# CVPR23/Depth-guided-Texture-Diffusion-for-Image-Semantic-Segmentation

Hardware: NVIDIA B200
Metric: rgbd_images_per_sec_384 (higher is better)
Workload: dtype bf16

## Files before the change

depth-guided-texture-diffusion-for-image-semantic-segmentation_b200/csrc/common.cuh:

```cuda
#pragma once
#include <cuda_bf16.h>
#include <cuda_runtime.h>
#include <stdint.h>
#include <stdio.h>

#include "../../include/dgtd_ops.h"

#if defined(__CUDA_ARCH__) && (__CUDA_ARCH__ < 1000)
#error "libdgtd_ops targets sm_100a only"
#endif

namespace dgtd {

void set_error(const char* fmt, ...);
void count_launch(int n = 1);

#define DGTD_CHECK_ARG(cond, ...)        \
  do {                                   \
    if (!(cond)) {                       \
      ::dgtd::set_error(__VA_ARGS__);    \
      return -1;                         \
    }                                    \
  } while (0)

#define DGTD_LAUNCH_CHECK(name)                                                  \
  do {                                                                           \
    cudaError_t e__ = cudaGetLastError();                                        \
    if (e__ != cudaSuccess) {                                                    \
      ::dgtd::set_error("%s: launch failed: %s", name, cudaGetErrorString(e__)); \
      return -2;                                                                 \
    }                                                                            \
    ::dgtd::count_launch();                                                      \
  } while (0)

static inline int cdiv(int64_t a, int64_t b) { return (int)((a + b - 1) / b); }

__device__ __forceinline__ float warp_sum(float v) {
#pragma unroll
  for (int o = 16; o > 0; o >>= 1) v += __shfl_xor_sync(0xffffffffu, v, o);
  return v;
}

__device__ __forceinline__ float gelu_erf(float x) {
  return 0.5f * x * (1.0f + erff(x * 0.70710678118654752440f));
}

__device__ __forceinline__ float sigmoidf_acc(float x) { return 1.0f / (1.0f + expf(-x)); }

template <int ACT>
__device__ __forceinline__ float apply_act(float x) {
  if (ACT == DGTD_ACT_GELU) return gelu_erf(x);
  if (ACT == DGTD_ACT_RELU) return fmaxf(x, 0.0f);
  return x;
}

__device__ __forceinline__ float to_float(float v) { return v; }
__device__ __forceinline__ float to_float(__nv_bfloat16 v) { return __bfloat162float(v); }

template <typename T>
__device__ __forceinline__ T from_float(float v);
template <>
__device__ __forceinline__ float from_float<float>(float v) { return v; }
template <>
__device__ __forceinline__ __nv_bfloat16 from_float<__nv_bfloat16>(float v) {
  return __float2bfloat16_rn(v);
}

__device__ __forceinline__ void store1(float* p, float v) { *p = v; }
__device__ __forceinline__ void store1(__nv_bfloat16* p, float v) { *p = __float2bfloat16_rn(v); }
__device__ __forceinline__ void store4(float* p, float a, float b, float c, float d) {
  *reinterpret_cast<float4*>(p) = make_float4(a, b, c, d);
}
__device__ __forceinline__ void store4(__nv_bfloat16* p, float a, float b, float c, float d) {
  __nv_bfloat162 lo = __floats2bfloat162_rn(a, b), hi = __floats2bfloat162_rn(c, d);
  uint2 u;
  u.x = *reinterpret_cast<uint32_t*>(&lo);
  u.y = *reinterpret_cast<uint32_t*>(&hi);
  *reinterpret_cast<uint2*>(p) = u;
}
__device__ __forceinline__ float4 load4(const float* p) {
  return *reinterpret_cast<const float4*>(p);
}
__device__ __forceinline__ float4 load4(const __nv_bfloat16* p) {
  uint2 u = *reinterpret_cast<const uint2*>(p);
  __nv_bfloat162 lo = *reinterpret_cast<__nv_bfloat162*>(&u.x);
  __nv_bfloat162 hi = *reinterpret_cast<__nv_bfloat162*>(&u.y);
  float2 a = __bfloat1622float2(lo), b = __bfloat1622float2(hi);
  return make_float4(a.x, a.y, b.x, b.y);
}

__device__ __forceinline__ uint64_t pk2(float a, float b) {
  uint64_t r;
  asm("mov.b64 %0, {%1, %2};" : "=l"(r) : "f"(a), "f"(b));
  return r;
}
__device__ __forceinline__ void up2(uint64_t r, float& a, float& b) {
  asm("mov.b64 {%0, %1}, %2;" : "=f"(a), "=f"(b) : "l"(r));
}
__device__ __forceinline__ uint64_t fma2(uint64_t a, uint64_t b, uint64_t c) {
  uint64_t d;
  asm("fma.rn.f32x2 %0, %1, %2, %3;" : "=l"(d) : "l"(a), "l"(b), "l"(c));
  return d;
}
__device__ __forceinline__ uint64_t mul2(uint64_t a, uint64_t b) {
  uint64_t d;
  asm("mul.rn.f32x2 %0, %1, %2;" : "=l"(d) : "l"(a), "l"(b));
  return d;
}
__device__ __forceinline__ uint64_t add2(uint64_t a, uint64_t b) {
  uint64_t d;
  asm("add.rn.f32x2 %0, %1, %2;" : "=l"(d) : "l"(a), "l"(b));
  return d;
}
__device__ __forceinline__ void bilinear_src(int dst, float scale, int in_size, int& i0, int& i1,
                                             float& l1) {
  float s = (dst + 0.5f) * scale - 0.5f;
  s = s < 0.f ? 0.f : s;
  i0 = (int)s;
  if (i0 > in_size - 1) i0 = in_size - 1;
  i1 = i0 + (i0 < in_size - 1 ? 1 : 0);
  l1 = s - (float)i0;
}

}
```

depth-guided-texture-diffusion-for-image-semantic-segmentation_b200/csrc/convnext_ops.cu:

```cuda
#include "common.cuh"

namespace dgtd {

constexpr int STEM_PX = 16;

constexpr int STEM_TILES_PER_CTA = 12;

__global__ void __launch_bounds__(256)
stem_kernel(const float* __restrict__ image, const float* __restrict__ grid, int G,
            const float* __restrict__ w, const float* __restrict__ bias,
            const float* __restrict__ ln_w, const float* __restrict__ ln_b, float* __restrict__ out,
            int H, int W, int oh, int ow, int Cout, float eps, int total_tiles) {
  extern __shared__ float sm[];
  float* in = sm;
  float* ys = sm + STEM_PX * 48;
  const int tiles_x = (ow + STEM_PX - 1) / STEM_PX;
  const int c = threadIdx.x;
  float wr[48];
#pragma unroll
  for (int k = 0; k < 48; ++k) wr[k] = w[(int64_t)c * 48 + k];
  const float bc = bias[c];
  const int lane = threadIdx.x & 31, wid = threadIdx.x >> 5, nw = blockDim.x >> 5;

  for (int it = 0; it < STEM_TILES_PER_CTA; ++it) {
    int tile = blockIdx.x * STEM_TILES_PER_CTA + it;
    if (tile >= total_tiles) break;
    const int tx = tile % tiles_x;
    tile /= tiles_x;
    const int oy = tile % oh, b = tile / oh;
    const int ox0 = tx * STEM_PX;
    for (int e = threadIdx.x; e < 3 * 4 * 4 * STEM_PX; e += blockDim.x) {
      int ci = e / (16 * STEM_PX), r = e - ci * 16 * STEM_PX;
      int ky = r / (4 * STEM_PX), j = r - ky * 4 * STEM_PX;
      int px = j >> 2, kx = j & 3;
      int iy = oy * 4 + ky, ix = ox0 * 4 + j;
      float v = 0.f;
      if (ox0 + px < ow) {
        v = image[(((int64_t)b * 3 + ci) * H + iy) * W + ix];
        if (grid) {
          int y0, y1, x0, x1;
          float ly, lx;
          bilinear_src(iy, (float)G / H, G, y0, y1, ly);
          bilinear_src(ix, (float)G / W, G, x0, x1, lx);
          const float* g = grid + ((int64_t)b * 3 + ci) * G * G;
          v += (1.f - ly) * ((1.f - lx) * g[y0 * G + x0] + lx * g[y0 * G + x1]) +
               ly * ((1.f - lx) * g[y1 * G + x0] + lx * g[y1 * G + x1]);
        }
      }
      in[px * 48 + ci * 16 + ky * 4 + kx] = v;
    }
    __syncthreads();
#pragma unroll 4
    for (int px = 0; px < STEM_PX; ++px) {
      float acc = bc;
#pragma unroll
      for (int k4 = 0; k4 < 12; ++k4) {
        float4 v = *reinterpret_cast<const float4*>(&in[px * 48 + k4 * 4]);
        acc = fmaf(wr[k4 * 4 + 0], v.x, acc);
        acc = fmaf(wr[k4 * 4 + 1], v.y, acc);
        acc = fmaf(wr[k4 * 4 + 2], v.z, acc);
        acc = fmaf(wr[k4 * 4 + 3], v.w, acc);
      }
      ys[px * Cout + c] = acc;
    }
    __syncthreads();
    for (int px = wid; px < STEM_PX; px += nw) {
      if (ox0 + px >= ow) continue;
      float s = 0.f;
      for (int cc = lane; cc < Cout; cc += 32) s += ys[px * Cout + cc];
      float mean = warp_sum(s) / Cout;
      float q = 0.f;
      for (int cc = lane; cc < Cout; cc += 32) {
        float d = ys[px * Cout + cc] - mean;
        q = fmaf(d, d, q);
      }
      float rstd = 1.0f / sqrtf(warp_sum(q) / Cout + eps);
      float* o = out + (((int64_t)b * oh + oy) * ow + ox0 + px) * Cout;
      for (int cc = lane; cc < Cout; cc += 32)
        o[cc] = (ys[px * Cout + cc] - mean) * rstd * ln_w[cc] + ln_b[cc];
    }
    __syncthreads();
  }
}

template <typename OT, int VPL>
__global__ void __launch_bounds__(256)
ln_patchify_kernel(const float* __restrict__ x, const float* __restrict__ ln_w,
                   const float* __restrict__ ln_b, OT* __restrict__ out, int B, int h, int w, int C,
                   float eps) {
  const int h2 = h >> 1, w2 = w >> 1;
  int64_t pix = (int64_t)blockIdx.x * 8 + (threadIdx.x >> 5);
  int64_t total = (int64_t)B * h2 * 2 * w2 * 2;
  if (pix >= total) return;
  const int lane = threadIdx.x & 31;
  int xx = (int)(pix % (w2 * 2));
  int64_t t = pix / (w2 * 2);
  int yy = (int)(t % (h2 * 2));
  int b = (int)(t / (h2 * 2));
  const float* p = x + (((int64_t)b * h + yy) * w + xx) * C;
  float v[VPL];
  float s = 0.f;
#pragma unroll
  for (int j = 0; j < VPL; ++j) {
    v[j] = p[lane + 32 * j];
    s += v[j];
  }
  float mean = warp_sum(s) / C;
  float q = 0.f;
#pragma unroll
  for (int j = 0; j < VPL; ++j) {
    float d = v[j] - mean;
    q = fmaf(d, d, q);
  }
  float rstd = 1.0f / sqrtf(warp_sum(q) / C + eps);
  OT* o = out + (((int64_t)b * h2 + (yy >> 1)) * w2 + (xx >> 1)) * (4 * (int64_t)C) +
          (int64_t)((yy & 1) * 2 + (xx & 1)) * C;
#pragma unroll
  for (int j = 0; j < VPL; ++j) {
    int cc = lane + 32 * j;
    o[cc] = from_float<OT>((v[j] - mean) * rstd * ln_w[cc] + ln_b[cc]);
  }
}

template <typename OT, int V4, int R>
__global__ void __launch_bounds__(256)
ln_patchify_v4_kernel(const float* __restrict__ x, const float* __restrict__ ln_w, const float* __restrict__ ln_b,
                      OT* __restrict__ out, int B, int h, int w, int C, float eps) {
  const int h2 = h >> 1, w2 = w >> 1;
  const int64_t total = (int64_t)B * h2 * w2 * 4;
  const int64_t pix0 = ((int64_t)blockIdx.x * 8 + (threadIdx.x >> 5)) * R;
  if (pix0 >= total) return;
  const int lane = threadIdx.x & 31;
  float4 v[R][V4];
#pragma unroll
  for (int r = 0; r < R; ++r) {
    const int64_t pix = pix0 + r;
    const int r4 = (int)(pix & 3);
    int64_t t = pix >> 2;
    const int x2 = (int)(t % w2);
    t /= w2;
    const int y2 = (int)(t % h2), b = (int)(t / h2);
    const float* p = x + (((int64_t)b * h + 2 * y2 + (r4 >> 1)) * w + 2 * x2 + (r4 & 1)) * C;
#pragma unroll
    for (int j = 0; j < V4; ++j)
      v[r][j] = pix < total ? __ldg(reinterpret_cast<const float4*>(p + (j * 32 + lane) * 4)) : make_float4(0.f, 0.f, 0.f, 0.f);
  }
  float4 g[V4], be[V4];
#pragma unroll
  for (int j = 0; j < V4; ++j) {
    g[j] = __ldg(reinterpret_cast<const float4*>(ln_w + (j * 32 + lane) * 4));
    be[j] = __ldg(reinterpret_cast<const float4*>(ln_b + (j * 32 + lane) * 4));
  }
  const float inv_c = 1.0f / C;
#pragma unroll
  for (int r = 0; r < R; ++r) {
    float s = 0.f;
#pragma unroll
    for (int j = 0; j < V4; ++j) s += (v[r][j].x + v[r][j].y) + (v[r][j].z + v[r][j].w);
    const float mean = warp_sum(s) * inv_c;
    float q = 0.f;
#pragma unroll
    for (int j = 0; j < V4; ++j) {
      const float a = v[r][j].x - mean, bb = v[r][j].y - mean, c = v[r][j].z - mean, d = v[r][j].w - mean;
      q += (a * a + bb * bb) + (c * c + d * d);
    }
    const float rstd = 1.0f / sqrtf(warp_sum(q) * inv_c + eps);
    if (pix0 + r < total) {
      OT* o = out + (pix0 + r) * C;
#pragma unroll
      for (int j = 0; j < V4; ++j)
        store4(o + (j * 32 + lane) * 4, (v[r][j].x - mean) * rstd * g[j].x + be[j].x, (v[r][j].y - mean) * rstd * g[j].y + be[j].y,
               (v[r][j].z - mean) * rstd * g[j].z + be[j].z, (v[r][j].w - mean) * rstd * g[j].w + be[j].w);
    }
  }
}

template <typename OT, int TH>
__global__ void __launch_bounds__(256, 2)
dwconv7_ln_kernel(const float* __restrict__ x, const float* __restrict__ dw_w,
                  const float* __restrict__ dw_b, const float* __restrict__ ln_w,
                  const float* __restrict__ ln_b, OT* __restrict__ out, int h, int w, int C,
                  float eps) {
  constexpr int TW = 8, NPX = TH * TW;
  extern __shared__ float ys[];
  const int tiles_x = (w + TW - 1) / TW, tiles_y = (h + TH - 1) / TH;
  int bid = blockIdx.x;
  const int tx = bid % tiles_x;
  bid /= tiles_x;
  const int ty = bid % tiles_y, b = bid / tiles_y;
  const int x0 = tx * TW, y0 = ty * TH;
  const float* xb = x + (int64_t)b * h * w * C;

  for (int c = threadIdx.x; c < C; c += blockDim.x) {
    float wr[49];
#pragma unroll
    for (int k = 0; k < 49; ++k) wr[k] = dw_w[(int64_t)c * 49 + k];
    float acc[TH][TW];
    const float bc = dw_b[c];
#pragma unroll
    for (int i = 0; i < TH; ++i)
#pragma unroll
      for (int j = 0; j < TW; ++j) acc[i][j] = bc;
#pragma unroll
    for (int iy = 0; iy < TH + 6; ++iy) {
      const int gy = y0 + iy - 3;
      if (gy < 0 || gy >= h) continue;
      float in[TW + 6];
      const float* row = xb + (int64_t)gy * w * C + c;
#pragma unroll
      for (int j = 0; j < TW + 6; ++j) {
        int gx = x0 + j - 3;
        in[j] = (gx >= 0 && gx < w) ? row[(int64_t)gx * C] : 0.f;
      }
#pragma unroll
      for (int oy = 0; oy < TH; ++oy) {
        const int ky = iy - oy;
        if (ky < 0 || ky >= 7) continue;
#pragma unroll
        for (int ox = 0; ox < TW; ++ox)
#pragma unroll
          for (int kx = 0; kx < 7; ++kx) acc[oy][ox] = fmaf(wr[ky * 7 + kx], in[ox + kx], acc[oy][ox]);
      }
      asm volatile("" ::: "memory");
    }
#pragma unroll
    for (int i = 0; i < TH; ++i)
#pragma unroll
      for (int j = 0; j < TW; ++j) ys[(i * TW + j) * C + c] = acc[i][j];
  }
  __syncthreads();
  const int lane = threadIdx.x & 31, wid = threadIdx.x >> 5, nw = blockDim.x >> 5;
  for (int px = wid; px < NPX; px += nw) {
    const int oy = y0 + px / TW, ox = x0 + px % TW;
    if (oy >= h || ox >= w) continue;
    const float* yp = ys + px * C;
    float s = 0.f;
    for (int c = lane; c < C; c += 32) s += yp[c];
    const float mean = warp_sum(s) / C;
    float q = 0.f;
    for (int c = lane; c < C; c += 32) {
      float d = yp[c] - mean;
      q = fmaf(d, d, q);
    }
    const float rstd = 1.0f / sqrtf(warp_sum(q) / C + eps);
    OT* o = out + (((int64_t)b * h + oy) * w + ox) * C;
    for (int c = lane; c < C; c += 32)
      o[c] = from_float<OT>((yp[c] - mean) * rstd * ln_w[c] + ln_b[c]);
  }
}

__global__ void __launch_bounds__(256)
fusion_sum_kernel(const float* __restrict__ z0, const float* __restrict__ z1, const float* __restrict__ z2,
                  const float* __restrict__ z3, int h0, int w0, int h1, int w1, int h2, int w2, int h3, int w3,
                  const float* __restrict__ bias, float* __restrict__ out_nhwc, float* __restrict__ out_nchw,
                  __nv_bfloat16* __restrict__ out_pad, int C, int Cpad, int quads, int64_t total) {
  const int64_t i = (int64_t)blockIdx.x * blockDim.x + threadIdx.x;
  if (i >= total) return;
  const int cq = (int)(i % quads);
  const int64_t p = i / quads;
  const int c = cq * 4;
  if (c >= C) {
    if (out_pad && c < Cpad) store4(out_pad + p * Cpad + c, 0.f, 0.f, 0.f, 0.f);
    return;
  }
  const int ox = (int)(p % w0);
  const int64_t t = p / w0;
  const int oy = (int)(t % h0), b = (int)(t / h0);
  float4 acc = load4(bias + c);
  {
    const float4 v = load4(z0 + p * C + c);
    acc.x += v.x; acc.y += v.y; acc.z += v.z; acc.w += v.w;
  }
#pragma unroll
  for (int lv = 1; lv < 4; ++lv) {
    const float* src = lv == 1 ? z1 : lv == 2 ? z2 : z3;
    const int hh = lv == 1 ? h1 : lv == 2 ? h2 : h3;
    const int ww = lv == 1 ? w1 : lv == 2 ? w2 : w3;
    int y0, y1, x0, x1;
    float ly, lx;
    bilinear_src(oy, (float)hh / h0, hh, y0, y1, ly);
    bilinear_src(ox, (float)ww / w0, ww, x0, x1, lx);
    const float* sb = src + (int64_t)b * hh * ww * C + c;
    const float4 a = load4(sb + ((int64_t)y0 * ww + x0) * C), bq = load4(sb + ((int64_t)y0 * ww + x1) * C);
    const float4 cc = load4(sb + ((int64_t)y1 * ww + x0) * C), d = load4(sb + ((int64_t)y1 * ww + x1) * C);
    const float w00 = (1.f - ly) * (1.f - lx), w01 = (1.f - ly) * lx, w10 = ly * (1.f - lx), w11 = ly * lx;
    acc.x += w00 * a.x + w01 * bq.x + w10 * cc.x + w11 * d.x;
    acc.y += w00 * a.y + w01 * bq.y + w10 * cc.y + w11 * d.y;
    acc.z += w00 * a.z + w01 * bq.z + w10 * cc.z + w11 * d.z;
    acc.w += w00 * a.w + w01 * bq.w + w10 * cc.w + w11 * d.w;
  }
  if (out_nhwc) store4(out_nhwc + p * C + c, acc.x, acc.y, acc.z, acc.w);
  if (out_pad) store4(out_pad + p * Cpad + c, acc.x, acc.y, acc.z, acc.w);
  if (out_nchw) {
    const int64_t hw = (int64_t)h0 * w0, r = p - (int64_t)b * hw;
    float* o = out_nchw + ((int64_t)b * C + c) * hw + r;
    o[0] = acc.x; o[hw] = acc.y; o[2 * hw] = acc.z; o[3 * hw] = acc.w;
  }
}

template <typename IT, typename OT>
__global__ void resize_nhwc_kernel(const IT* __restrict__ x, OT* __restrict__ out, int h, int w, int C,
                                   int oh, int ow, int64_t total) {
  int64_t i = (int64_t)blockIdx.x * blockDim.x + threadIdx.x;
  if (i >= total) return;
  const int c4 = C >> 2;
  int cq = (int)(i % c4);
  int64_t t = i / c4;
  int ox = (int)(t % ow);
  t /= ow;
  int oy = (int)(t % oh), b = (int)(t / oh);
  int y0, y1, x0, x1;
  float ly, lx;
  bilinear_src(oy, (float)h / oh, h, y0, y1, ly);
  bilinear_src(ox, (float)w / ow, w, x0, x1, lx);
  const IT* xb = x + (int64_t)b * h * w * C + cq * 4;
  float4 a = load4(xb + ((int64_t)y0 * w + x0) * C), bq = load4(xb + ((int64_t)y0 * w + x1) * C);
  float4 cc = load4(xb + ((int64_t)y1 * w + x0) * C), d = load4(xb + ((int64_t)y1 * w + x1) * C);
  float w00 = (1.f - ly) * (1.f - lx), w01 = (1.f - ly) * lx, w10 = ly * (1.f - lx), w11 = ly * lx;
  store4(out + (((int64_t)b * oh + oy) * ow + ox) * C + cq * 4,
         w00 * a.x + w01 * bq.x + w10 * cc.x + w11 * d.x, w00 * a.y + w01 * bq.y + w10 * cc.y + w11 * d.y,
         w00 * a.z + w01 * bq.z + w10 * cc.z + w11 * d.z, w00 * a.w + w01 * bq.w + w10 * cc.w + w11 * d.w);
}

}

namespace dgtd {
int ln_rows_any(const float* y, const float* ln_w, const float* ln_b, void* out, int out_dtype, int64_t rows, int C,
                float eps, cudaStream_t s);
int dwconv7_ln_tma(const float* x, const float* wT, const float* dw_b, const float* ln_w, const float* ln_b,
                   float* ws, void* out, int out_dtype, int B, int h, int w, int C, float eps, cudaStream_t s);
int dwconv7_stats_tma(const float* x, const float* wT, const float* dw_b, __nv_bfloat16* y, float2* stats, int B, int h,
                      int w, int C, float eps, cudaStream_t s);
}
using namespace dgtd;

extern "C" {

int dgtd_stem_fwd(const float* image, const float* grid, int G, const float* w, const float* b,
                  const float* ln_w, const float* ln_b, float* out, int B, int H, int W, int Cout,
                  float eps, dgtd_stream_t stream) {
  DGTD_CHECK_ARG(image && w && b && ln_w && ln_b && out, "stem: null pointer");
  DGTD_CHECK_ARG(B > 0 && H >= 4 && W >= 4 && Cout >= 32 && Cout <= 256 && Cout % 32 == 0,
                 "stem: bad shape B=%d H=%d W=%d Cout=%d", B, H, W, Cout);
  DGTD_CHECK_ARG(!grid || G > 0, "stem: bad grid size");
  const int oh = H / 4, ow = W / 4;
  size_t smem = (size_t)(STEM_PX * 48 + STEM_PX * Cout) * sizeof(float);
  const int total_tiles = cdiv(ow, STEM_PX) * oh * B;
  stem_kernel<<<cdiv(total_tiles, STEM_TILES_PER_CTA), Cout, smem, (cudaStream_t)stream>>>(
      image, grid, G, w, b, ln_w, ln_b, out, H, W, oh, ow, Cout, eps, total_tiles);
  DGTD_LAUNCH_CHECK("stem");
  return 0;
}

}

template <typename OT>
static int ln_patchify_dispatch(const float* x, const float* ln_w, const float* ln_b, OT* out, int B,
                                int h, int w, int C, float eps, cudaStream_t s) {
  int64_t pix = (int64_t)B * (h / 2) * 2 * (w / 2) * 2;
  if (C % 128 == 0 && (reinterpret_cast<uintptr_t>(x) & 15) == 0 && (reinterpret_cast<uintptr_t>(out) & 15) == 0 &&
      (reinterpret_cast<uintptr_t>(ln_w) & 15) == 0 && (reinterpret_cast<uintptr_t>(ln_b) & 15) == 0) {
    switch (C / 128) {
      case 1: ln_patchify_v4_kernel<OT, 1, 4><<<cdiv(pix, 32), 256, 0, s>>>(x, ln_w, ln_b, out, B, h, w, C, eps); return 0;
      case 2: ln_patchify_v4_kernel<OT, 2, 2><<<cdiv(pix, 16), 256, 0, s>>>(x, ln_w, ln_b, out, B, h, w, C, eps); return 0;
      case 4: ln_patchify_v4_kernel<OT, 4, 1><<<cdiv(pix, 8), 256, 0, s>>>(x, ln_w, ln_b, out, B, h, w, C, eps); return 0;
      case 8: ln_patchify_v4_kernel<OT, 8, 1><<<cdiv(pix, 8), 256, 0, s>>>(x, ln_w, ln_b, out, B, h, w, C, eps); return 0;
      default: break;
    }
  }
  int blocks = cdiv(pix, 8);
  switch (C / 32) {
    case 1: ln_patchify_kernel<OT, 1><<<blocks, 256, 0, s>>>(x, ln_w, ln_b, out, B, h, w, C, eps); break;
    case 2: ln_patchify_kernel<OT, 2><<<blocks, 256, 0, s>>>(x, ln_w, ln_b, out, B, h, w, C, eps); break;
    case 4: ln_patchify_kernel<OT, 4><<<blocks, 256, 0, s>>>(x, ln_w, ln_b, out, B, h, w, C, eps); break;
    case 8: ln_patchify_kernel<OT, 8><<<blocks, 256, 0, s>>>(x, ln_w, ln_b, out, B, h, w, C, eps); break;
    case 16: ln_patchify_kernel<OT, 16><<<blocks, 256, 0, s>>>(x, ln_w, ln_b, out, B, h, w, C, eps); break;
    case 32: ln_patchify_kernel<OT, 32><<<blocks, 256, 0, s>>>(x, ln_w, ln_b, out, B, h, w, C, eps); break;
    default:
      set_error("ln_patchify: C=%d must be 32*{1,2,4,8,16,32}", C);
      return -1;
  }
  return 0;
}

extern "C" int dgtd_ln_patchify_fwd(const float* x, const float* ln_w, const float* ln_b, void* out,
                         int out_dtype, int B, int h, int w, int C, float eps,
                         dgtd_stream_t stream) {
  DGTD_CHECK_ARG(x && ln_w && ln_b && out && B > 0 && h >= 2 && w >= 2 && C % 32 == 0,
                 "ln_patchify: bad args");
  int rc = out_dtype == DGTD_BF16
               ? ln_patchify_dispatch(x, ln_w, ln_b, (__nv_bfloat16*)out, B, h, w, C, eps, (cudaStream_t)stream)
               : ln_patchify_dispatch(x, ln_w, ln_b, (float*)out, B, h, w, C, eps, (cudaStream_t)stream);
  if (rc) return rc;
  DGTD_LAUNCH_CHECK("ln_patchify");
  return 0;
}

template <typename OT>
static int dwconv_launch(const float* x, const float* dw_w, const float* dw_b, const float* ln_w,
                         const float* ln_b, OT* out, int B, int h, int w, int C, float eps,
                         cudaStream_t s) {
  constexpr int TH = 4;
  size_t smem = (size_t)TH * 8 * C * sizeof(float);
  if (smem > 48 * 1024) {
    cudaError_t e = cudaFuncSetAttribute(dwconv7_ln_kernel<OT, TH>,
                                         cudaFuncAttributeMaxDynamicSharedMemorySize, (int)smem);
    if (e != cudaSuccess) {
      set_error("dwconv7_ln: cannot opt in to %zu B smem: %s", smem, cudaGetErrorString(e));
      return -2;
    }
  }
  int threads = C < 256 ? C : 256;
  int64_t blocks = (int64_t)B * cdiv(h, TH) * cdiv(w, 8);
  dwconv7_ln_kernel<OT, TH><<<(unsigned)blocks, threads, smem, s>>>(x, dw_w, dw_b, ln_w, ln_b, out, h,
                                                                    w, C, eps);
  return 0;
}

extern "C" {

int dgtd_dwconv7_ln_fwd(const float* x, const float* dw_w, const float* dw_b, const float* ln_w,
                        const float* ln_b, void* out, int out_dtype, int B, int h, int w, int C,
                        float eps, dgtd_stream_t stream) {
  DGTD_CHECK_ARG(x && dw_w && dw_b && ln_w && ln_b && out, "dwconv7_ln: null pointer");
  DGTD_CHECK_ARG(B > 0 && h > 0 && w > 0 && C >= 32 && C % 32 == 0 && C <= 1024,
                 "dwconv7_ln: bad shape B=%d h=%d w=%d C=%d", B, h, w, C);
  int rc = out_dtype == DGTD_BF16
               ? dwconv_launch(x, dw_w, dw_b, ln_w, ln_b, (__nv_bfloat16*)out, B, h, w, C, eps, (cudaStream_t)stream)
               : dwconv_launch(x, dw_w, dw_b, ln_w, ln_b, (float*)out, B, h, w, C, eps, (cudaStream_t)stream);
  if (rc) return rc;
  DGTD_LAUNCH_CHECK("dwconv7_ln");
  return 0;
}

int dgtd_dwconv7_ln_tma_fwd(const float* x, const float* dw_wT, const float* dw_b, const float* ln_w,
                            const float* ln_b, float* ws, void* out, int out_dtype, int B, int h, int w,
                            int C, float eps, dgtd_stream_t stream) {
  DGTD_CHECK_ARG(x && dw_wT && dw_b && ln_w && ln_b && ws && out, "dwconv7_ln_tma: null pointer");
  DGTD_CHECK_ARG(B > 0 && h > 0 && w > 0 && C >= 128 && C % 128 == 0 && C <= 1024,
                 "dwconv7_ln_tma: bad shape B=%d h=%d w=%d C=%d (C must be a multiple of 128)", B, h, w, C);
  int rc = dwconv7_ln_tma(x, dw_wT, dw_b, ln_w, ln_b, ws, out, out_dtype, B, h, w, C, eps, (cudaStream_t)stream);
  if (rc > 0) {
    set_error("dwconv7_ln_tma: shape not supported by the TMA variant");
    return -1;
  }
  if (rc) return rc;
  DGTD_LAUNCH_CHECK("dwconv7_ln_tma.ln");
  return 0;
}

int dgtd_dwconv7_stats_tma_fwd(const float* x, const float* dw_wT, const float* dw_b, void* y, float* stats, int B, int h,
                               int w, int C, float eps, dgtd_stream_t stream) {
  DGTD_CHECK_ARG(x && dw_wT && dw_b && y && stats, "dwconv7_stats_tma: null pointer");
  DGTD_CHECK_ARG(B > 0 && h > 0 && w > 0 && C >= 128 && C % 128 == 0 && C <= 1024,
                 "dwconv7_stats_tma: bad shape B=%d h=%d w=%d C=%d (C must be a multiple of 128)", B, h, w, C);
  DGTD_CHECK_ARG((reinterpret_cast<uintptr_t>(stats) & 7) == 0 && (reinterpret_cast<uintptr_t>(y) & 15) == 0,
                 "dwconv7_stats_tma: y must be 16-byte, stats 8-byte aligned");
  int rc = dwconv7_stats_tma(x, dw_wT, dw_b, (__nv_bfloat16*)y, (float2*)stats, B, h, w, C, eps, (cudaStream_t)stream);
  if (rc > 0) {
    set_error("dwconv7_stats_tma: shape not supported by the TMA variant");
    return -1;
  }
  return rc;
}

int dgtd_ln_rows_fwd(const float* y, const float* ln_w, const float* ln_b, void* out, int out_dtype, int64_t rows,
                     int C, float eps, dgtd_stream_t stream) {
  DGTD_CHECK_ARG(y && ln_w && ln_b && out && rows > 0 && C % 128 == 0 && C <= 1024, "ln_rows: bad args");
  int rc = ln_rows_any(y, ln_w, ln_b, out, out_dtype, rows, C, eps, (cudaStream_t)stream);
  if (rc) return rc;
  DGTD_LAUNCH_CHECK("ln_rows");
  return 0;
}

int dgtd_fusion_sum_fwd(const float* z0, const float* z1, const float* z2, const float* z3, const int* hw,
                        const float* bias, float* out_nhwc, float* out_nchw, void* out_pad, int Cpad, int B, int C,
                        dgtd_stream_t stream) {
  DGTD_CHECK_ARG(z0 && z1 && z2 && z3 && hw && bias, "fusion_sum: null pointer");
  DGTD_CHECK_ARG(C > 0 && C % 4 == 0, "fusion_sum: C must be a multiple of 4");
  DGTD_CHECK_ARG(out_nhwc || out_nchw || out_pad, "fusion_sum: no output requested");
  DGTD_CHECK_ARG(!out_pad || (Cpad >= C && Cpad % 4 == 0), "fusion_sum: Cpad must be a multiple of 4 and >= C");
  const int quads = (out_pad && Cpad > C ? Cpad : C) / 4;
  const int64_t total = (int64_t)B * hw[0] * hw[1] * quads;
  fusion_sum_kernel<<<(unsigned)cdiv(total, (int64_t)256), 256, 0, (cudaStream_t)stream>>>(
      z0, z1, z2, z3, hw[0], hw[1], hw[2], hw[3], hw[4], hw[5], hw[6], hw[7], bias, out_nhwc, out_nchw,
      (__nv_bfloat16*)out_pad, C, Cpad, quads, total);
  DGTD_LAUNCH_CHECK("fusion_sum");
  return 0;
}

int dgtd_resize_nhwc_fwd(const void* x, void* out, int B, int h, int w, int C, int oh, int ow,
                         int dtype_in, int dtype_out, dgtd_stream_t stream) {
  DGTD_CHECK_ARG(x && out && B > 0 && h > 0 && w > 0 && oh > 0 && ow > 0 && C % 4 == 0,
                 "resize_nhwc: bad args (C must be a multiple of 4)");
  int64_t total = (int64_t)B * oh * ow * (C / 4);
  cudaStream_t s = (cudaStream_t)stream;
  int blocks = cdiv(total, 256);
  if (dtype_in == DGTD_F32 && dtype_out == DGTD_F32)
    resize_nhwc_kernel<<<blocks, 256, 0, s>>>((const float*)x, (float*)out, h, w, C, oh, ow, total);
  else if (dtype_in == DGTD_BF16 && dtype_out == DGTD_BF16)
    resize_nhwc_kernel<<<blocks, 256, 0, s>>>((const __nv_bfloat16*)x, (__nv_bfloat16*)out, h, w, C, oh, ow, total);
  else if (dtype_in == DGTD_BF16 && dtype_out == DGTD_F32)
    resize_nhwc_kernel<<<blocks, 256, 0, s>>>((const __nv_bfloat16*)x, (float*)out, h, w, C, oh, ow, total);
  else
    resize_nhwc_kernel<<<blocks, 256, 0, s>>>((const float*)x, (__nv_bfloat16*)out, h, w, C, oh, ow, total);
  DGTD_LAUNCH_CHECK("resize_nhwc");
  return 0;
}

}
```

depth-guided-texture-diffusion-for-image-semantic-segmentation_b200/csrc/dwconv_tma.cu:

```cuda
#include "blackwell.cuh"
#include "common.cuh"

namespace dgtd {

int sm_count();
static inline int sm_count_dw() { return sm_count(); }

template <int SY, int SX, bool ADD, typename OT = float>
__global__ void __launch_bounds__(SY * SX * 32, 2)
dwconv7_tma_kernel(const __grid_constant__ CUtensorMap tmX, const float* __restrict__ wT,
                   const float* __restrict__ bias, const float* __restrict__ add, OT* __restrict__ y, int h,
                   int w, int C, int tiles_x, int tiles_y) {
  constexpr int TH = 4 * SY, TW = 8 * SX, PH = TH + 6, PW = TW + 6, NCH = 4;
  constexpr int TILE_FLOATS = PH * PW * 32;
  constexpr uint32_t TILE_BYTES = TILE_FLOATS * 4;
  extern __shared__ __align__(128) float xs[];
  __shared__ uint64_t bar[2];

  int bid = blockIdx.x;
  const int cgs = C >> 7;
  const int cg = bid % cgs; bid /= cgs;
  const int tx = bid % tiles_x; bid /= tiles_x;
  const int ty = bid % tiles_y;
  const int b = bid / tiles_y;
  const int warp = threadIdx.x >> 5, lane = threadIdx.x & 31;
  const int sy = warp / SX, sx = warp - sy * SX;
  const int x0 = tx * TW, y0 = ty * TH;

  if (threadIdx.x == 0) {
    bw::prefetch_tmap(&tmX);
    bw::mbar_init(&bar[0], 1);
    bw::mbar_init(&bar[1], 1);
    bw::fence_mbar_init();
  }
  __syncthreads();
  if (threadIdx.x == 0) {
    bw::mbar_arrive_expect_tx(&bar[0], TILE_BYTES);
    bw::tma_load_4d(&tmX, &bar[0], xs, cg * 128, x0 - 3, y0 - 3, b);
  }

#pragma unroll 1
  for (int i = 0; i < NCH; ++i) {
    const int c = cg * 128 + i * 32 + lane;
    if (threadIdx.x == 0 && i + 1 < NCH) {
      bw::fence_proxy_async_smem();
      bw::mbar_arrive_expect_tx(&bar[(i + 1) & 1], TILE_BYTES);
      bw::tma_load_4d(&tmX, &bar[(i + 1) & 1], xs + ((i + 1) & 1) * TILE_FLOATS, cg * 128 + (i + 1) * 32, x0 - 3,
                      y0 - 3, b);
    }
    uint64_t w2[49];
#pragma unroll
    for (int k = 0; k < 49; ++k) {
      const float t = __ldg(wT + (int64_t)k * C + c);
      w2[k] = pk2(t, t);
    }
    const float bc = bias ? __ldg(bias + c) : 0.f;
    uint64_t acc[2][8];
#pragma unroll
    for (int q = 0; q < 2; ++q)
#pragma unroll
      for (int j = 0; j < 8; ++j) acc[q][j] = pk2(bc, bc);

    bw::mbar_wait(&bar[i & 1], (i >> 1) & 1);
    const float* base = xs + (i & 1) * TILE_FLOATS + ((4 * sy) * PW + 8 * sx) * 32 + lane;
#pragma unroll
    for (int iy = 0; iy < 9; ++iy) {
      uint64_t pr[14];
#pragma unroll
      for (int j = 0; j < 14; ++j) {
        const volatile float* p0 = base + (iy * PW + j) * 32;
        pr[j] = pk2(p0[0], p0[PW * 32]);
      }
#pragma unroll
      for (int q = 0; q < 2; ++q) {
        const int ky = iy - 2 * q;
        if (ky < 0 || ky >= 7) continue;
#pragma unroll
        for (int kx = 0; kx < 7; ++kx)
#pragma unroll
          for (int j = 0; j < 8; ++j) acc[q][j] = fma2(w2[ky * 7 + kx], pr[j + kx], acc[q][j]);
      }
    }
    if (ADD) {
      float av[4][8];
#pragma unroll
      for (int a = 0; a < 4; ++a)
#pragma unroll
        for (int j = 0; j < 8; ++j) {
          const int oy = y0 + 4 * sy + a, ox = x0 + 8 * sx + j;
          av[a][j] = (oy < h && ox < w) ? __ldg(add + (((int64_t)b * h + oy) * w + ox) * C + c) : 0.f;
        }
#pragma unroll
      for (int q = 0; q < 2; ++q)
#pragma unroll
        for (int j = 0; j < 8; ++j) acc[q][j] = add2(acc[q][j], pk2(av[2 * q][j], av[2 * q + 1][j]));
    }
    {
      const int oy0 = y0 + 4 * sy, ox0 = x0 + 8 * sx;
      OT* yp = y + (((int64_t)b * h + oy0) * w + ox0) * C + c;
      const int rs = w * C;
      if (oy0 + 4 <= h && ox0 + 8 <= w) {
#pragma unroll
        for (int q = 0; q < 2; ++q)
#pragma unroll
          for (int j = 0; j < 8; ++j) {
            float v0, v1;
            up2(acc[q][j], v0, v1);
            store1(yp + (2 * q) * rs + j * C, v0);
            store1(yp + (2 * q + 1) * rs + j * C, v1);
          }
      } else {
#pragma unroll
        for (int q = 0; q < 2; ++q)
#pragma unroll
          for (int j = 0; j < 8; ++j) {
            float v0, v1;
            up2(acc[q][j], v0, v1);
            if (ox0 + j < w) {
              if (oy0 + 2 * q < h) store1(yp + (2 * q) * rs + j * C, v0);
              if (oy0 + 2 * q + 1 < h) store1(yp + (2 * q + 1) * rs + j * C, v1);
            }
          }
      }
    }
    __syncthreads();
  }
}


template <int SY, int SX, bool ADD, typename OT>
__global__ void __launch_bounds__(SY * SX * 32, 2)
dwconv7_tma_persist_kernel(const __grid_constant__ CUtensorMap tmX, const __grid_constant__ CUtensorMap tmW,
                           const float* __restrict__ bias, const float* __restrict__ add, OT* __restrict__ y, int h,
                           int w, int C, int tiles_x, int tiles_y, int num_items) {
  constexpr int TH = 4 * SY, TW = 8 * SX, PH = TH + 6, PW = TW + 6;
  constexpr int TILE_FLOATS = PH * PW * 32;
  constexpr uint32_t TILE_BYTES = TILE_FLOATS * 4, W_BYTES = 49 * 32 * 4;
  extern __shared__ __align__(128) float xs[];
  float* wbuf = xs + 2 * TILE_FLOATS;
  __shared__ uint64_t bar[3];

  const int warp = threadIdx.x >> 5, lane = threadIdx.x & 31;
  const int sy = warp / SX, sx = warp - sy * SX;
  const int nch = C >> 5;
  auto issue_tile = [&](int item, int buf) {
    const int chunk = item % nch;
    int t = item / nch;
    const int tx = t % tiles_x; t /= tiles_x;
    const int ty = t % tiles_y;
    const int b = t / tiles_y;
    bw::mbar_arrive_expect_tx(&bar[buf], TILE_BYTES);
    bw::tma_load_4d(&tmX, &bar[buf], xs + buf * TILE_FLOATS, chunk * 32, tx * TW - 3, ty * TH - 3, b);
  };
  auto issue_weights = [&](int item) {
    bw::mbar_arrive_expect_tx(&bar[2], W_BYTES);
    bw::tma_load_2d(&tmW, &bar[2], wbuf, (item % nch) * 32, 0);
  };
  if (threadIdx.x == 0) {
    bw::prefetch_tmap(&tmX);
    bw::prefetch_tmap(&tmW);
    bw::mbar_init(&bar[0], 1);
    bw::mbar_init(&bar[1], 1);
    bw::mbar_init(&bar[2], 1);
    bw::fence_mbar_init();
  }
  __syncthreads();
  if (threadIdx.x == 0 && (int)blockIdx.x < num_items) {
    issue_tile(blockIdx.x, 0);
    issue_weights(blockIdx.x);
  }
  int it = 0;
#pragma unroll 1
  for (int item = blockIdx.x; item < num_items; item += gridDim.x, ++it) {
    const int next = item + gridDim.x;
    if (threadIdx.x == 0 && next < num_items) {
      bw::fence_proxy_async_smem();
      issue_tile(next, (it + 1) & 1);
    }
    const int chunk = item % nch;
    int t = item / nch;
    const int tx = t % tiles_x; t /= tiles_x;
    const int ty = t % tiles_y;
    const int b = t / tiles_y;
    const int x0 = tx * TW, y0 = ty * TH;
    const int c = chunk * 32 + lane;
    bw::mbar_wait(&bar[2], it & 1);
    uint64_t w2[49];
#pragma unroll
    for (int k = 0; k < 49; ++k) {
      const float tv = wbuf[k * 32 + lane];
      w2[k] = pk2(tv, tv);
    }
    __syncthreads();
    if (threadIdx.x == 0 && next < num_items) {
      bw::fence_proxy_async_smem();
      issue_weights(next);
    }
    const float bc = bias ? __ldg(bias + c) : 0.f;
    uint64_t acc[2][8];
#pragma unroll
    for (int q = 0; q < 2; ++q)
#pragma unroll
      for (int j = 0; j < 8; ++j) acc[q][j] = pk2(bc, bc);

    bw::mbar_wait(&bar[it & 1], (it >> 1) & 1);
    const float* base = xs + (it & 1) * TILE_FLOATS + ((4 * sy) * PW + 8 * sx) * 32 + lane;
#pragma unroll
    for (int iy = 0; iy < 9; ++iy) {
      uint64_t pr[14];
#pragma unroll
      for (int j = 0; j < 14; ++j) {
        const volatile float* p0 = base + (iy * PW + j) * 32;
        pr[j] = pk2(p0[0], p0[PW * 32]);
      }
#pragma unroll
      for (int q = 0; q < 2; ++q) {
        const int ky = iy - 2 * q;
        if (ky < 0 || ky >= 7) continue;
#pragma unroll
        for (int kx = 0; kx < 7; ++kx)
#pragma unroll
          for (int j = 0; j < 8; ++j) acc[q][j] = fma2(w2[ky * 7 + kx], pr[j + kx], acc[q][j]);
      }
    }
    if (ADD) {
      float av[4][8];
#pragma unroll
      for (int a = 0; a < 4; ++a)
#pragma unroll
        for (int j = 0; j < 8; ++j) {
          const int oy = y0 + 4 * sy + a, ox = x0 + 8 * sx + j;
          av[a][j] = (oy < h && ox < w) ? __ldg(add + (((int64_t)b * h + oy) * w + ox) * C + c) : 0.f;
        }
#pragma unroll
      for (int q = 0; q < 2; ++q)
#pragma unroll
        for (int j = 0; j < 8; ++j) acc[q][j] = add2(acc[q][j], pk2(av[2 * q][j], av[2 * q + 1][j]));
    }
    {
      const int oy0 = y0 + 4 * sy, ox0 = x0 + 8 * sx;
      OT* yp = y + (((int64_t)b * h + oy0) * w + ox0) * C + c;
      const int rs = w * C;
      if (oy0 + 4 <= h && ox0 + 8 <= w) {
#pragma unroll
        for (int q = 0; q < 2; ++q)
#pragma unroll
          for (int j = 0; j < 8; ++j) {
            float v0, v1;
            up2(acc[q][j], v0, v1);
            store1(yp + (2 * q) * rs + j * C, v0);
            store1(yp + (2 * q + 1) * rs + j * C, v1);
          }
      } else {
#pragma unroll
        for (int q = 0; q < 2; ++q)
#pragma unroll
          for (int j = 0; j < 8; ++j) {
            float v0, v1;
            up2(acc[q][j], v0, v1);
            if (ox0 + j < w) {
              if (oy0 + 2 * q < h) store1(yp + (2 * q) * rs + j * C, v0);
              if (oy0 + 2 * q + 1 < h) store1(yp + (2 * q + 1) * rs + j * C, v1);
            }
          }
      }
    }
    __syncthreads();
  }
}

template <int SY, int SX>
__global__ void __launch_bounds__(SY * SX * 32, 2)
dwconv7_wgrad_tma_kernel(const __grid_constant__ CUtensorMap tmX, const float* __restrict__ dy,
                         float* __restrict__ part, int h, int w, int C, int tiles_x, int tiles_y, int ntiles) {
  constexpr int TH = 4 * SY, TW = 8 * SX, PH = TH + 6, PW = TW + 6, NW = SY * SX;
  constexpr int TILE_FLOATS = PH * PW * 32;
  constexpr uint32_t TILE_BYTES = TILE_FLOATS * 4;
  static_assert(NW * 50 * 32 <= 2 * TILE_FLOATS, "reduction scratch must fit in the tile buffers");
  extern __shared__ __align__(128) float xs[];
  __shared__ uint64_t bar[2];

  const int chunk = blockIdx.x, P = gridDim.y;
  const int warp = threadIdx.x >> 5, lane = threadIdx.x & 31;
  const int sy = warp / SX, sx = warp - sy * SX;
  const int c = chunk * 32 + lane;

  auto issue = [&](int t, int buf) {
    const int tx = t % tiles_x;
    const int r = t / tiles_x;
    const int ty = r % tiles_y, b = r / tiles_y;
    bw::mbar_arrive_expect_tx(&bar[buf], TILE_BYTES);
    bw::tma_load_4d(&tmX, &bar[buf], xs + buf * TILE_FLOATS, chunk * 32, tx * TW - 3, ty * TH - 3, b);
  };
  if (threadIdx.x == 0) {
    bw::prefetch_tmap(&tmX);
    bw::mbar_init(&bar[0], 1);
    bw::mbar_init(&bar[1], 1);
    bw::fence_mbar_init();
  }
  __syncthreads();
  if (threadIdx.x == 0) issue(blockIdx.y, 0);

  float acc[50];
#pragma unroll
  for (int k = 0; k < 50; ++k) acc[k] = 0.f;

  int it = 0;
#pragma unroll 1
  for (int t = blockIdx.y; t < ntiles; t += P, ++it) {
    if (threadIdx.x == 0 && t + P < ntiles) {
      bw::fence_proxy_async_smem();
      issue(t + P, (it + 1) & 1);
    }
    const int tx = t % tiles_x;
    const int r = t / tiles_x;
    const int ty = r % tiles_y, b = r / tiles_y;
    const int oy0 = ty * TH + 4 * sy, ox0 = tx * TW + 8 * sx;
    float g[4][8];
#pragma unroll
    for (int a = 0; a < 4; ++a)
#pragma unroll
      for (int j = 0; j < 8; ++j) {
        const int oy = oy0 + a, ox = ox0 + j;
        g[a][j] = (oy < h && ox < w) ? __ldg(dy + (((int64_t)b * h + oy) * w + ox) * C + c) : 0.f;
        acc[49] += g[a][j];
      }
    bw::mbar_wait(&bar[it & 1], (it >> 1) & 1);
    const float* base = xs + (it & 1) * TILE_FLOATS + ((4 * sy) * PW + 8 * sx) * 32 + lane;
#pragma unroll
    for (int iy = 0; iy < 10; ++iy) {
      float in[14];
#pragma unroll
      for (int j = 0; j < 14; ++j) in[j] = base[(iy * PW + j) * 32];
#pragma unroll
      for (int a = 0; a < 4; ++a) {
        const int ky = iy - a;
        if (ky < 0 || ky >= 7) continue;
#pragma unroll
        for (int kx = 0; kx < 7; ++kx)
#pragma unroll
          for (int j = 0; j < 8; ++j) acc[ky * 7 + kx] = fmaf(g[a][j], in[j + kx], acc[ky * 7 + kx]);
      }
    }
    __syncthreads();
  }
  float* red = xs;
#pragma unroll
  for (int k = 0; k < 50; ++k) red[(warp * 50 + k) * 32 + lane] = acc[k];
  __syncthreads();
  for (int i = threadIdx.x; i < 50 * 32; i += NW * 32) {
    float v = 0.f;
#pragma unroll
    for (int q = 0; q < NW; ++q) v += red[q * 50 * 32 + i];
    part[((int64_t)blockIdx.y * 50 + (i >> 5)) * C + chunk * 32 + (i & 31)] = v;
  }
}

template <typename OT, int VPL>
__global__ void __launch_bounds__(256)
ln_rows_kernel(const float* __restrict__ y, const float* __restrict__ ln_w, const float* __restrict__ ln_b,
               OT* __restrict__ out, int64_t rows, int C, float eps) {
  const int64_t row = (int64_t)blockIdx.x * 8 + (threadIdx.x >> 5);
  if (row >= rows) return;
  const int lane = threadIdx.x & 31;
  const float* p = y + row * C;
  float4 v[VPL];
  float s = 0.f;
#pragma unroll
  for (int j = 0; j < VPL; ++j) {
    v[j] = *reinterpret_cast<const float4*>(p + (j * 32 + lane) * 4);
    s += (v[j].x + v[j].y) + (v[j].z + v[j].w);
  }
  const float mean = warp_sum(s) / C;
  float q = 0.f;
#pragma unroll
  for (int j = 0; j < VPL; ++j) {
    float a = v[j].x - mean, b = v[j].y - mean, c = v[j].z - mean, d = v[j].w - mean;
    q += (a * a + b * b) + (c * c + d * d);
  }
  const float rstd = 1.0f / sqrtf(warp_sum(q) / C + eps);
  OT* o = out + row * C;
#pragma unroll
  for (int j = 0; j < VPL; ++j) {
    const int c0 = (j * 32 + lane) * 4;
    float4 g = *reinterpret_cast<const float4*>(ln_w + c0), be = *reinterpret_cast<const float4*>(ln_b + c0);
    store4(o + c0, (v[j].x - mean) * rstd * g.x + be.x, (v[j].y - mean) * rstd * g.y + be.y,
           (v[j].z - mean) * rstd * g.z + be.z, (v[j].w - mean) * rstd * g.w + be.w);
  }
}

template <int LPR, int V, int U>
__global__ void __launch_bounds__(256)
row_stats_bf16_kernel(const __nv_bfloat16* __restrict__ y, float2* __restrict__ stats, int64_t rows, int C, float eps) {
  constexpr int RPP = 32 / LPR;
  constexpr int RPW = RPP * U;
  const int lane = threadIdx.x & 31, sub = lane / LPR, l = lane % LPR;
  const int64_t row0 = ((int64_t)blockIdx.x * 8 + (threadIdx.x >> 5)) * RPW + sub;
  uint4 raw[U][V];
#pragma unroll
  for (int u = 0; u < U; ++u) {
    const int64_t row = row0 + u * RPP;
#pragma unroll
    for (int j = 0; j < V; ++j) {
      raw[u][j] = make_uint4(0u, 0u, 0u, 0u);
      if (row < rows) raw[u][j] = __ldg(reinterpret_cast<const uint4*>(y + row * C + (j * LPR + l) * 8));
    }
  }
  const float inv_c = 1.0f / C;
#pragma unroll
  for (int u = 0; u < U; ++u) {
    float f[V][8];
    float s = 0.f;
#pragma unroll
    for (int j = 0; j < V; ++j) {
      const uint32_t w4[4] = {raw[u][j].x, raw[u][j].y, raw[u][j].z, raw[u][j].w};
#pragma unroll
      for (int e = 0; e < 4; ++e) {
        f[j][2 * e] = __uint_as_float(w4[e] << 16);
        f[j][2 * e + 1] = __uint_as_float(w4[e] & 0xffff0000u);
      }
      s += ((f[j][0] + f[j][1]) + (f[j][2] + f[j][3])) + ((f[j][4] + f[j][5]) + (f[j][6] + f[j][7]));
    }
#pragma unroll
    for (int o = LPR / 2; o > 0; o >>= 1) s += __shfl_xor_sync(0xffffffffu, s, o);
    const float mean = s * inv_c;
    float q = 0.f;
#pragma unroll
    for (int j = 0; j < V; ++j) {
#pragma unroll
      for (int e = 0; e < 8; e += 2) {
        const float a = f[j][e] - mean, b = f[j][e + 1] - mean;
        q += a * a + b * b;
      }
    }
#pragma unroll
    for (int o = LPR / 2; o > 0; o >>= 1) q += __shfl_xor_sync(0xffffffffu, q, o);
    const int64_t row = row0 + u * RPP;
    if (l == 0 && row < rows) stats[row] = make_float2(mean, 1.0f / sqrtf(q * inv_c + eps));
  }
}

static int row_stats_grid(int64_t rows, int rows_per_block) { return (int)cdiv(rows, rows_per_block); }

int row_stats_bf16(const __nv_bfloat16* y, float2* stats, int64_t rows, int C, float eps, cudaStream_t s) {
  if (reinterpret_cast<uintptr_t>(y) & 15) {
    set_error("row_stats: the matrix must be 16-byte aligned");
    return -1;
  }
  switch (C / 128) {
    case 1: row_stats_bf16_kernel<16, 1, 4><<<row_stats_grid(rows, 64), 256, 0, s>>>(y, stats, rows, C, eps); break;
    case 2: row_stats_bf16_kernel<32, 1, 4><<<row_stats_grid(rows, 32), 256, 0, s>>>(y, stats, rows, C, eps); break;
    case 4: row_stats_bf16_kernel<32, 2, 2><<<row_stats_grid(rows, 16), 256, 0, s>>>(y, stats, rows, C, eps); break;
    case 8: row_stats_bf16_kernel<32, 4, 1><<<row_stats_grid(rows, 8), 256, 0, s>>>(y, stats, rows, C, eps); break;
    default:
      set_error("row_stats: C=%d must be 128*{1,2,4,8}", C);
      return -1;
  }
  return 0;
}

template <int SY, int SX, bool ADD, typename OT>
static int dw_launch_persist(const CUtensorMap& tm, const float* wT, const float* bias, const float* add, OT* y, int B, int h,
                             int w, int C, cudaStream_t s) {
  constexpr int PH = 4 * SY + 6, PW = 8 * SX + 6;
  constexpr int SMEM = 2 * PH * PW * 128 + 49 * 32 * 4 + 128;
  auto kern = dwconv7_tma_persist_kernel<SY, SX, ADD, OT>;
  static bool configured = false;
  if (!configured) {
    cudaError_t e = cudaFuncSetAttribute(kern, cudaFuncAttributeMaxDynamicSharedMemorySize, SMEM);
    if (e != cudaSuccess) {
      set_error("dwconv7_tma(persistent): cannot opt in to %d B smem: %s", SMEM, cudaGetErrorString(e));
      return -2;
    }
    configured = true;
  }
  CUtensorMap tmW;
  {
    const uint64_t dims[2] = {(uint64_t)C, 49}, strides[1] = {(uint64_t)C * 4};
    const uint32_t box[2] = {32, 49};
    int rc = make_tmap(&tmW, wT, CU_TENSOR_MAP_DATA_TYPE_FLOAT32, 2, dims, strides, box, CU_TENSOR_MAP_SWIZZLE_NONE);
    if (rc) return rc;
  }
  const int tiles_x = cdiv(w, 8 * SX), tiles_y = cdiv(h, 4 * SY);
  const int64_t items = (int64_t)B * tiles_x * tiles_y * (C / 32);
  if (items > 0x7fffffff) {
    set_error("dwconv7_tma(persistent): too many items");
    return -1;
  }
  const int slots = 2 * sm_count_dw();
  const int grid = items < slots ? (int)items : slots;
  kern<<<grid, SY * SX * 32, SMEM, s>>>(tm, tmW, bias, add, y, h, w, C, tiles_x, tiles_y, (int)items);
  return 0;
}

template <int SY, int SX>
static int dw_launch_bf16(const CUtensorMap& tm, const float* wT, const float* bias, __nv_bfloat16* y, int B, int h, int w,
                          int C, cudaStream_t s) {
  if ((reinterpret_cast<uintptr_t>(wT) & 15) == 0)
    return dw_launch_persist<SY, SX, false, __nv_bfloat16>(tm, wT, bias, nullptr, y, B, h, w, C, s);
  constexpr int PH = 4 * SY + 6, PW = 8 * SX + 6;
  constexpr int SMEM = 2 * PH * PW * 128 + 128;
  auto kern = dwconv7_tma_kernel<SY, SX, false, __nv_bfloat16>;
  static bool configured = false;
  if (!configured) {
    cudaError_t e = cudaFuncSetAttribute(kern, cudaFuncAttributeMaxDynamicSharedMemorySize, SMEM);
    if (e != cudaSuccess) {
      set_error("dwconv7_tma(bf16): cannot opt in to %d B smem: %s", SMEM, cudaGetErrorString(e));
      return -2;
    }
    configured = true;
  }
  const int tiles_x = cdiv(w, 8 * SX), tiles_y = cdiv(h, 4 * SY);
  const int64_t blocks = (int64_t)B * tiles_x * tiles_y * (C / 128);
  kern<<<(unsigned)blocks, SY * SX * 32, SMEM, s>>>(tm, wT, bias, nullptr, y, h, w, C, tiles_x, tiles_y);
  return 0;
}

template <int SY, int SX>
static int dw_launch(const CUtensorMap& tm, const float* wT, const float* bias, const float* add, float* y, int B,
                     int h, int w, int C, cudaStream_t s) {
  if ((reinterpret_cast<uintptr_t>(wT) & 15) == 0) {
    if (add) return dw_launch_persist<SY, SX, true, float>(tm, wT, bias, add, y, B, h, w, C, s);
    return dw_launch_persist<SY, SX, false, float>(tm, wT, bias, nullptr, y, B, h, w, C, s);
  }
  constexpr int PH = 4 * SY + 6, PW = 8 * SX + 6;
  constexpr int SMEM = 2 * PH * PW * 128 + 128;
  static bool configured = false;
  if (!configured) {
    cudaError_t e = cudaFuncSetAttribute(dwconv7_tma_kernel<SY, SX, false>, cudaFuncAttributeMaxDynamicSharedMemorySize, SMEM);
    if (e == cudaSuccess)
      e = cudaFuncSetAttribute(dwconv7_tma_kernel<SY, SX, true>, cudaFuncAttributeMaxDynamicSharedMemorySize, SMEM);
    if (e != cudaSuccess) {
      set_error("dwconv7_tma: cannot opt in to %d B smem: %s", SMEM, cudaGetErrorString(e));
      return -2;
    }
    configured = true;
  }
  const int tiles_x = cdiv(w, 8 * SX), tiles_y = cdiv(h, 4 * SY);
  const int64_t blocks = (int64_t)B * tiles_x * tiles_y * (C / 128);
  if (add)
    dwconv7_tma_kernel<SY, SX, true><<<(unsigned)blocks, SY * SX * 32, SMEM, s>>>(tm, wT, bias, add, y, h, w, C, tiles_x, tiles_y);
  else
    dwconv7_tma_kernel<SY, SX, false><<<(unsigned)blocks, SY * SX * 32, SMEM, s>>>(tm, wT, bias, add, y, h, w, C, tiles_x, tiles_y);
  return 0;
}

template <typename OT>
static int ln_rows_launch(const float* y, const float* ln_w, const float* ln_b, OT* out, int64_t rows, int C,
                          float eps, cudaStream_t s) {
  const int blocks = cdiv(rows, 8);
  switch (C / 128) {
    case 1: ln_rows_kernel<OT, 1><<<blocks, 256, 0, s>>>(y, ln_w, ln_b, out, rows, C, eps); break;
    case 2: ln_rows_kernel<OT, 2><<<blocks, 256, 0, s>>>(y, ln_w, ln_b, out, rows, C, eps); break;
    case 4: ln_rows_kernel<OT, 4><<<blocks, 256, 0, s>>>(y, ln_w, ln_b, out, rows, C, eps); break;
    case 8: ln_rows_kernel<OT, 8><<<blocks, 256, 0, s>>>(y, ln_w, ln_b, out, rows, C, eps); break;
    default:
      set_error("dwconv7_ln(tma): C=%d must be 128*{1,2,4,8}", C);
      return -1;
  }
  return 0;
}

int dwconv7_tma(const float* x, const float* wT, const float* dw_b, const float* add, float* y, int B, int h, int w,
                int C, cudaStream_t s) {
  if (C % 128 || C > 1024 || (reinterpret_cast<uintptr_t>(x) & 15)) return 1;
  const int SX = (w % 24 == 0 && w % 16 != 0) ? 3 : 2;
  const int SY = (h % 8 == 0 || h > 12) ? 2 : 3;
  CUtensorMap tm;
  {
    PFN_tmapEncodeTiled enc = get_tmap_encoder();
    if (!enc) return -3;
    cuuint64_t gd[4] = {(cuuint64_t)C, (cuuint64_t)w, (cuuint64_t)h, (cuuint64_t)B};
    cuuint64_t gs[3] = {(cuuint64_t)C * 4, (cuuint64_t)w * C * 4, (cuuint64_t)h * w * C * 4};
    cuuint32_t bx[4] = {32, (cuuint32_t)(8 * SX + 6), (cuuint32_t)(4 * SY + 6), 1};
    cuuint32_t es[4] = {1, 1, 1, 1};
    CUresult r = enc(&tm, CU_TENSOR_MAP_DATA_TYPE_FLOAT32, 4, const_cast<float*>(x), gd, gs, bx, es,
                     CU_TENSOR_MAP_INTERLEAVE_NONE, CU_TENSOR_MAP_SWIZZLE_NONE, CU_TENSOR_MAP_L2_PROMOTION_L2_128B,
                     CU_TENSOR_MAP_FLOAT_OOB_FILL_NONE);
    if (r != CUDA_SUCCESS) {
      set_error("dwconv7(tma): cuTensorMapEncodeTiled failed (%d) for x (%d,%d,%d,%d)", (int)r, B, h, w, C);
      return -3;
    }
  }
  int rc;
  if (SY == 2 && SX == 2) rc = dw_launch<2, 2>(tm, wT, dw_b, add, y, B, h, w, C, s);
  else if (SY == 2 && SX == 3) rc = dw_launch<2, 3>(tm, wT, dw_b, add, y, B, h, w, C, s);
  else if (SY == 3 && SX == 2) rc = dw_launch<3, 2>(tm, wT, dw_b, add, y, B, h, w, C, s);
  else rc = dw_launch<3, 3>(tm, wT, dw_b, add, y, B, h, w, C, s);
  if (rc) return rc;
  cudaError_t e = cudaGetLastError();
  if (e != cudaSuccess) {
    set_error("dwconv7_tma: launch failed: %s", cudaGetErrorString(e));
    return -2;
  }
  count_launch();
  return 0;
}


template <int SY, int SX>
static int dwg_launch(const CUtensorMap& tm, const float* dy, float* part, int P, int B, int h, int w, int C,
                      cudaStream_t s) {
  constexpr int PH = 4 * SY + 6, PW = 8 * SX + 6;
  constexpr int SMEM = 2 * PH * PW * 128 + 128;
  auto kern = dwconv7_wgrad_tma_kernel<SY, SX>;
  static bool configured = false;
  if (!configured) {
    cudaError_t e = cudaFuncSetAttribute(kern, cudaFuncAttributeMaxDynamicSharedMemorySize, SMEM);
    if (e != cudaSuccess) {
      set_error("dwconv7_wgrad_tma: cannot opt in to %d B smem: %s", SMEM, cudaGetErrorString(e));
      return -2;
    }
    configured = true;
  }
  const int tiles_x = cdiv(w, 8 * SX), tiles_y = cdiv(h, 4 * SY);
  kern<<<dim3(C / 32, P), SY * SX * 32, SMEM, s>>>(tm, dy, part, h, w, C, tiles_x, tiles_y, B * tiles_x * tiles_y);
  return 0;
}

static int dw_tile_shape(int h, int w, int* SY, int* SX) {
  *SX = (w % 24 == 0 && w % 16 != 0) ? 3 : 2;
  *SY = (h % 8 == 0 || h > 12) ? 2 : 3;
  return 0;
}

static int dw_make_tmap(CUtensorMap* tm, const float* x, int B, int h, int w, int C, int SY, int SX) {
  PFN_tmapEncodeTiled enc = get_tmap_encoder();
  if (!enc) return -3;
  cuuint64_t gd[4] = {(cuuint64_t)C, (cuuint64_t)w, (cuuint64_t)h, (cuuint64_t)B};
  cuuint64_t gs[3] = {(cuuint64_t)C * 4, (cuuint64_t)w * C * 4, (cuuint64_t)h * w * C * 4};
  cuuint32_t bx[4] = {32, (cuuint32_t)(8 * SX + 6), (cuuint32_t)(4 * SY + 6), 1};
  cuuint32_t es[4] = {1, 1, 1, 1};
  CUresult r = enc(tm, CU_TENSOR_MAP_DATA_TYPE_FLOAT32, 4, const_cast<float*>(x), gd, gs, bx, es,
                   CU_TENSOR_MAP_INTERLEAVE_NONE, CU_TENSOR_MAP_SWIZZLE_NONE, CU_TENSOR_MAP_L2_PROMOTION_L2_128B,
                   CU_TENSOR_MAP_FLOAT_OOB_FILL_NONE);
  if (r != CUDA_SUCCESS) {
    set_error("dwconv7(tma): cuTensorMapEncodeTiled failed (%d) for x (%d,%d,%d,%d)", (int)r, B, h, w, C);
    return -3;
  }
  return 0;
}

int dwconv7_wgrad_tma(const float* x, const float* dy, float* part, int max_parts, int* parts, int B, int h, int w,
                      int C, cudaStream_t s) {
  if (C % 128 || (reinterpret_cast<uintptr_t>(x) & 15) || (int64_t)B * h * w < 2048) return 1;
  int SY, SX;
  dw_tile_shape(h, w, &SY, &SX);
  const int ntiles = B * cdiv(w, 8 * SX) * cdiv(h, 4 * SY);
  int P = cdiv(2 * 148, C / 32);
  if (P > ntiles) P = ntiles;
  if (P > max_parts) P = max_parts;
  if (P < 1) return 1;
  CUtensorMap tm;
  int rc = dw_make_tmap(&tm, x, B, h, w, C, SY, SX);
  if (rc) return rc;
  if (SY == 2 && SX == 2) rc = dwg_launch<2, 2>(tm, dy, part, P, B, h, w, C, s);
  else if (SY == 2 && SX == 3) rc = dwg_launch<2, 3>(tm, dy, part, P, B, h, w, C, s);
  else if (SY == 3 && SX == 2) rc = dwg_launch<3, 2>(tm, dy, part, P, B, h, w, C, s);
  else rc = dwg_launch<3, 3>(tm, dy, part, P, B, h, w, C, s);
  if (rc) return rc;
  cudaError_t e = cudaGetLastError();
  if (e != cudaSuccess) {
    set_error("dwconv7_wgrad_tma: launch failed: %s", cudaGetErrorString(e));
    return -2;
  }
  count_launch();
  *parts = P;
  return 0;
}

int dwconv7_stats_tma(const float* x, const float* wT, const float* dw_b, __nv_bfloat16* y, float2* stats, int B, int h,
                      int w, int C, float eps, cudaStream_t s) {
  if (C % 128 || C > 1024 || (reinterpret_cast<uintptr_t>(x) & 15)) return 1;
  int SY, SX;
  dw_tile_shape(h, w, &SY, &SX);
  CUtensorMap tm;
  int rc = dw_make_tmap(&tm, x, B, h, w, C, SY, SX);
  if (rc) return rc;
  if (SY == 2 && SX == 2) rc = dw_launch_bf16<2, 2>(tm, wT, dw_b, y, B, h, w, C, s);
  else if (SY == 2 && SX == 3) rc = dw_launch_bf16<2, 3>(tm, wT, dw_b, y, B, h, w, C, s);
  else if (SY == 3 && SX == 2) rc = dw_launch_bf16<3, 2>(tm, wT, dw_b, y, B, h, w, C, s);
  else rc = dw_launch_bf16<3, 3>(tm, wT, dw_b, y, B, h, w, C, s);
  if (rc) return rc;
  cudaError_t e = cudaGetLastError();
  if (e != cudaSuccess) {
    set_error("dwconv7_stats_tma: launch failed: %s", cudaGetErrorString(e));
    return -2;
  }
  count_launch();
  rc = row_stats_bf16(y, stats, (int64_t)B * h * w, C, eps, s);
  if (rc) return rc;
  e = cudaGetLastError();
  if (e != cudaSuccess) {
    set_error("row_stats: launch failed: %s", cudaGetErrorString(e));
    return -2;
  }
  count_launch();
  return 0;
}

int dwconv7_ln_tma(const float* x, const float* wT, const float* dw_b, const float* ln_w, const float* ln_b,
                   float* ws, void* out, int out_dtype, int B, int h, int w, int C, float eps, cudaStream_t s) {
  int rc = dwconv7_tma(x, wT, dw_b, nullptr, ws, B, h, w, C, s);
  if (rc) return rc;
  const int64_t rows = (int64_t)B * h * w;
  return out_dtype == DGTD_BF16 ? ln_rows_launch(ws, ln_w, ln_b, (__nv_bfloat16*)out, rows, C, eps, s)
                                : ln_rows_launch(ws, ln_w, ln_b, (float*)out, rows, C, eps, s);
}

int ln_rows_any(const float* y, const float* ln_w, const float* ln_b, void* out, int out_dtype, int64_t rows, int C,
                float eps, cudaStream_t s) {
  return out_dtype == DGTD_BF16 ? ln_rows_launch(y, ln_w, ln_b, (__nv_bfloat16*)out, rows, C, eps, s)
                                : ln_rows_launch(y, ln_w, ln_b, (float*)out, rows, C, eps, s);
}

}
```

depth-guided-texture-diffusion-for-image-semantic-segmentation_b200/csrc/mlp_fused.cu:

```cuda
#include "tc_common.cuh"

namespace dgtd {

namespace mlpf {

constexpr int C = 128, HID = 4 * C, HC = 128, NCH = HID / HC;
constexpr int BLK = 128 * 64 * 2;
constexpr int KB1 = C / 64, KB2 = HC / 64;
constexpr int A_BYTES = KB1 * BLK, H_BYTES = KB2 * BLK;
constexpr int WST = 4;
constexpr int NEPI = 16;
constexpr int STG_BYTES = NEPI * 4096;
constexpr int OFF_A = 0, OFF_H = A_BYTES, OFF_W = OFF_H + 2 * H_BYTES, OFF_STG = OFF_W + WST * BLK, OFF_BAR = OFF_STG + STG_BYTES;
constexpr int NBARS = 2 + 2 * WST + 4 + 4 + 4 + NEPI;
constexpr int SMEM = OFF_BAR + NBARS * 8 + 16;
constexpr int THREADS = 128 + NEPI * 32;
static_assert(SMEM <= 232448, "shared memory budget");

struct Params {
  const float* row_stats;
  const float* col_s;
  const float* cbias;
  const float* b2;
  const float* gamma;
  const float* res;
  float* out;
  int M, tiles;
};

__device__ __forceinline__ uint32_t swz_l(int lane) { return (uint32_t)(lane & 7); }

__global__ void __launch_bounds__(THREADS, 1)
mlp_fused_kernel(const __grid_constant__ CUtensorMap tmY, const __grid_constant__ CUtensorMap tmW1,
                 const __grid_constant__ CUtensorMap tmW2, const __grid_constant__ CUtensorMap tmRes,
                 const __grid_constant__ CUtensorMap tmOut, const Params p) {
  extern __shared__ __align__(1024) uint8_t smem[];
  uint8_t* sA = smem + OFF_A;
  uint8_t* sH = smem + OFF_H;
  uint8_t* sW = smem + OFF_W;
  uint64_t* bars = reinterpret_cast<uint64_t*>(smem + OFF_BAR);
  uint8_t* sStg = smem + OFF_STG;
  uint64_t* a_full = bars;
  uint64_t* a_empty = a_full + 1;
  uint64_t* w_full = a_empty + 1;
  uint64_t* w_empty = w_full + WST;
  uint64_t* c1_full = w_empty + WST;
  uint64_t* c1_empty = c1_full + 2;
  uint64_t* h_full = c1_empty + 2;
  uint64_t* h_empty = h_full + 2;
  uint64_t* c2_full = h_empty + 2;
  uint64_t* c2_empty = c2_full + 2;
  uint64_t* r_full = c2_empty + 2;
  uint32_t* tmem_slot = reinterpret_cast<uint32_t*>(r_full + NEPI);

  const int warp = threadIdx.x >> 5, lane = threadIdx.x & 31;
  if (warp == 0 && lane == 0) {
    bw::prefetch_tmap(&tmY);
    bw::prefetch_tmap(&tmW1);
    bw::prefetch_tmap(&tmW2);
    bw::prefetch_tmap(&tmRes);
    bw::prefetch_tmap(&tmOut);
  }
  if (warp == 1 && lane == 0) {
    bw::mbar_init(a_full, 1);
    bw::mbar_init(a_empty, 1);
    for (int i = 0; i < 2; ++i) {
      bw::mbar_init(&c1_full[i], 1);
      bw::mbar_init(&c1_empty[i], NEPI);
      bw::mbar_init(&h_full[i], NEPI);
      bw::mbar_init(&h_empty[i], 1);
      bw::mbar_init(&c2_full[i], 1);
      bw::mbar_init(&c2_empty[i], NEPI);
    }
    for (int i = 0; i < NEPI; ++i) bw::mbar_init(&r_full[i], 1);
    for (int i = 0; i < WST; ++i) {
      bw::mbar_init(&w_full[i], 1);
      bw::mbar_init(&w_empty[i], 1);
    }
    bw::fence_mbar_init();
  }
  if (warp == 2) bw::tmem_alloc(tmem_slot, 512);
  bw::tc_fence_before();
  __syncthreads();
  bw::tc_fence_after();
  const uint32_t tmem_base = *tmem_slot;

  if (warp == 0) {
    if (lane == 0) {
      int ws = 0;
      uint32_t wph = 0;
      auto load_w = [&](const CUtensorMap* tm, int k0, int r0) {
        bw::mbar_wait(&w_empty[ws], wph ^ 1);
        bw::mbar_arrive_expect_tx(&w_full[ws], BLK);
        bw::tma_load_2d(tm, &w_full[ws], sW + ws * BLK, k0, r0);
        if (++ws == WST) { ws = 0; wph ^= 1; }
      };
      int it = 0;
      for (int tile = blockIdx.x; tile < p.tiles; tile += gridDim.x, ++it) {
        bw::mbar_wait(a_empty, (it & 1) ^ 1);
        bw::mbar_arrive_expect_tx(a_full, A_BYTES);
        for (int kb = 0; kb < KB1; ++kb) bw::tma_load_2d(&tmY, a_full, sA + kb * BLK, kb * 64, tile * 128);
        for (int s = 0; s <= NCH; ++s) {
          if (s < NCH)
            for (int kb = 0; kb < KB1; ++kb) load_w(&tmW1, kb * 64, s * HC);
          if (s >= 1)
            for (int kb = 0; kb < KB2; ++kb) load_w(&tmW2, (s - 1) * HC + kb * 64, 0);
        }
      }
    }
  } else if (warp == 1) {
    if (lane == 0) {
      constexpr uint32_t idesc = bw::umma_idesc_bf16(128, 128);
      int ws = 0;
      uint32_t wph = 0;
      uint32_t q1 = 0, q2 = 0;
      int it = 0;
      for (int tile = blockIdx.x; tile < p.tiles; tile += gridDim.x, ++it) {
        const int ab = it & 1;
        bw::mbar_wait(a_full, it & 1);
        for (int s = 0; s <= NCH; ++s) {
          if (s < NCH) {
            const uint32_t b = q1 & 1;
            bw::mbar_wait(&c1_empty[b], ((q1 >> 1) & 1) ^ 1);
            bw::tc_fence_after();
            const uint32_t d = tmem_base + b * HC;
            for (int kb = 0; kb < KB1; ++kb) {
              bw::mbar_wait(&w_full[ws], wph);
              bw::tc_fence_after();
              const uint64_t da = bw::umma_smem_desc_kmajor(bw::smem_u32(sA + kb * BLK), 128);
              const uint64_t db = bw::umma_smem_desc_kmajor(bw::smem_u32(sW + ws * BLK), 128);
#pragma unroll
              for (int k = 0; k < 4; ++k) bw::umma_bf16(d, da + 2 * k, db + 2 * k, idesc, (kb | k) != 0);
              bw::umma_commit(&w_empty[ws]);
              if (++ws == WST) { ws = 0; wph ^= 1; }
            }
            bw::umma_commit(&c1_full[b]);
            if (s == NCH - 1) bw::umma_commit(a_empty);
            ++q1;
          }
          if (s >= 1) {
            const int c = s - 1;
            const uint32_t b = q2 & 1;
            if (c == 0) {
              bw::mbar_wait(&c2_empty[ab], ((it >> 1) & 1) ^ 1);
              bw::tc_fence_after();
            }
            bw::mbar_wait(&h_full[b], (q2 >> 1) & 1);
            bw::tc_fence_after();
            const uint32_t d = tmem_base + 2 * HC + ab * C;
            for (int kb = 0; kb < KB2; ++kb) {
              bw::mbar_wait(&w_full[ws], wph);
              bw::tc_fence_after();
              const uint64_t da = bw::umma_smem_desc_kmajor(bw::smem_u32(sH + b * H_BYTES + kb * BLK), 128);
              const uint64_t db = bw::umma_smem_desc_kmajor(bw::smem_u32(sW + ws * BLK), 128);
#pragma unroll
              for (int k = 0; k < 4; ++k) bw::umma_bf16(d, da + 2 * k, db + 2 * k, idesc, (c | kb | k) != 0);
              bw::umma_commit(&w_empty[ws]);
              if (++ws == WST) { ws = 0; wph ^= 1; }
            }
            bw::umma_commit(&h_empty[b]);
            if (c == NCH - 1) bw::umma_commit(&c2_full[ab]);
            ++q2;
          }
        }
      }
    }
  } else if (warp >= 4) {
    const int quad = warp & 3, part = (warp - 4) >> 2, ew = warp - 4;
    const int r = quad * 32 + lane;
    const uint32_t lane_addr = (uint32_t)(quad * 32) << 16;
    uint8_t* hrow_p = sH + (part >> 1) * BLK + r * 128;
    const uint32_t swz = (uint32_t)(r & 7);
    uint8_t* stg = sStg + ew * 4096;
    uint8_t* srow_p = stg + lane * 128;
    uint64_t* rbar = &r_full[ew];
    uint32_t q = 0;
    int it = 0;
    for (int tile = blockIdx.x; tile < p.tiles; tile += gridDim.x, ++it) {
      const int ab = it & 1;
      const int row0 = tile * 128 + quad * 32;
      if (lane == 0) {
        bw::tma_store_wait_read<0>();
        bw::mbar_arrive_expect_tx(rbar, 4096);
        bw::tma_load_2d(&tmRes, rbar, stg, part * 32, row0);
      }
      const float2 rs = __ldg(reinterpret_cast<const float2*>(p.row_stats) + row0 + lane);
      const uint64_t nm = pk2(-rs.x, -rs.x), rr = pk2(rs.y, rs.y);
      for (int c = 0; c < NCH; ++c, ++q) {
        const uint32_t b = q & 1;
        bw::mbar_wait(&c1_full[b], (q >> 1) & 1);
        bw::tc_fence_after();
        uint32_t v[32];
        bw::tmem_ld_32x32(tmem_base + lane_addr + b * HC + part * 32, v);
        bw::tmem_ld_wait();
        bw::tc_fence_before();
        __syncwarp();
        if (lane == 0) bw::mbar_arrive(&c1_empty[b]);
        bw::mbar_wait(&h_empty[b], ((q >> 1) & 1) ^ 1);
        const int n0 = c * HC + part * 32;
#pragma unroll
        for (int j = 0; j < 32; j += 8) {
          const float4 s0 = __ldg(reinterpret_cast<const float4*>(p.col_s + n0 + j));
          const float4 s1 = __ldg(reinterpret_cast<const float4*>(p.col_s + n0 + j + 4));
          const float4 b0 = __ldg(reinterpret_cast<const float4*>(p.cbias + n0 + j));
          const float4 b1 = __ldg(reinterpret_cast<const float4*>(p.cbias + n0 + j + 4));
          float f[8];
#pragma unroll
          for (int e = 0; e < 8; ++e) f[e] = __uint_as_float(v[j + e]);
          uint64_t x0 = fma2(nm, pk2(s0.x, s0.y), pk2(f[0], f[1])), x1 = fma2(nm, pk2(s0.z, s0.w), pk2(f[2], f[3]));
          uint64_t x2 = fma2(nm, pk2(s1.x, s1.y), pk2(f[4], f[5])), x3 = fma2(nm, pk2(s1.z, s1.w), pk2(f[6], f[7]));
          up2(fma2(rr, x0, pk2(b0.x, b0.y)), f[0], f[1]);
          up2(fma2(rr, x1, pk2(b0.z, b0.w)), f[2], f[3]);
          up2(fma2(rr, x2, pk2(b1.x, b1.y)), f[4], f[5]);
          up2(fma2(rr, x3, pk2(b1.z, b1.w)), f[6], f[7]);
#pragma unroll
          for (int e = 0; e < 8; e += 2) DGTD_GELU2(f[e], f[e + 1]);
          const __nv_bfloat162 a0 = __floats2bfloat162_rn(f[0], f[1]), a1 = __floats2bfloat162_rn(f[2], f[3]);
          const __nv_bfloat162 a2 = __floats2bfloat162_rn(f[4], f[5]), a3 = __floats2bfloat162_rn(f[6], f[7]);
          const uint32_t ch = (uint32_t)((part & 1) * 4 + (j >> 3));
          *reinterpret_cast<uint4*>(hrow_p + b * H_BYTES + ((ch ^ swz) << 4)) =
              make_uint4(*reinterpret_cast<const uint32_t*>(&a0), *reinterpret_cast<const uint32_t*>(&a1),
                         *reinterpret_cast<const uint32_t*>(&a2), *reinterpret_cast<const uint32_t*>(&a3));
        }
        bw::fence_proxy_async_smem();
        __syncwarp();
        if (lane == 0) bw::mbar_arrive(&h_full[b]);
      }
      bw::mbar_wait(&c2_full[ab], (it >> 1) & 1);
      bw::tc_fence_after();
      uint32_t v[32];
      bw::tmem_ld_32x32(tmem_base + lane_addr + 2 * HC + ab * C + part * 32, v);
      bw::tmem_ld_wait();
      bw::tc_fence_before();
      __syncwarp();
      if (lane == 0) bw::mbar_arrive(&c2_empty[ab]);
      bw::mbar_wait(rbar, it & 1);
#pragma unroll
      for (int j = 0; j < 32; j += 4) {
        float4* sp = reinterpret_cast<float4*>(srow_p + ((((uint32_t)(j >> 2)) ^ swz_l(lane)) << 4));
        float4 x = *sp;
        const float4 bb = __ldg(reinterpret_cast<const float4*>(p.b2 + part * 32 + j));
        float4 g = make_float4(1.f, 1.f, 1.f, 1.f);
        if (p.gamma) g = __ldg(reinterpret_cast<const float4*>(p.gamma + part * 32 + j));
        x.x += g.x * (__uint_as_float(v[j]) + bb.x);
        x.y += g.y * (__uint_as_float(v[j + 1]) + bb.y);
        x.z += g.z * (__uint_as_float(v[j + 2]) + bb.z);
        x.w += g.w * (__uint_as_float(v[j + 3]) + bb.w);
        *sp = x;
      }
      bw::fence_proxy_async_smem();
      __syncwarp();
      if (lane == 0) {
        bw::tma_store_2d(&tmOut, stg, part * 32, row0);
        bw::tma_store_commit();
      }
    }
    if (lane == 0) bw::tma_store_wait_all<0>();
  }

  bw::tc_fence_before();
  __syncthreads();
  if (warp == 2) {
    bw::tc_fence_after();
    bw::tmem_dealloc(tmem_base, 512);
  }
}

}
}

using namespace dgtd;

extern "C" int dgtd_convnext_mlp_fused_fwd(const void* y, const float* row_stats, const void* w1, const float* col_s,
                                           const float* cbias, const void* w2, const float* b2, const float* gamma,
                                           const float* residual, float* out, int64_t M, int C, dgtd_stream_t stream) {
  using namespace mlpf;
  DGTD_CHECK_ARG(y && row_stats && w1 && col_s && cbias && w2 && b2 && residual && out, "convnext_mlp_fused: null pointer");
  DGTD_CHECK_ARG(C == mlpf::C, "convnext_mlp_fused: C = %d is not built (stage 0, C = 128, only)", C);
  DGTD_CHECK_ARG(M > 0 && M % 128 == 0 && M < ((int64_t)1 << 31), "convnext_mlp_fused: M = %lld must be a positive multiple of 128",
                 (long long)M);
  cudaStream_t s = (cudaStream_t)stream;
  CUtensorMap tmY, tmW1, tmW2;
  {
    uint64_t dims[2] = {(uint64_t)C, (uint64_t)M}, str[1] = {(uint64_t)C * 2};
    uint32_t box[2] = {64, 128};
    if (make_tmap(&tmY, y, CU_TENSOR_MAP_DATA_TYPE_BFLOAT16, 2, dims, str, box, CU_TENSOR_MAP_SWIZZLE_128B)) return -3;
  }
  {
    uint64_t dims[2] = {(uint64_t)C, (uint64_t)HID}, str[1] = {(uint64_t)C * 2};
    uint32_t box[2] = {64, 128};
    if (make_tmap(&tmW1, w1, CU_TENSOR_MAP_DATA_TYPE_BFLOAT16, 2, dims, str, box, CU_TENSOR_MAP_SWIZZLE_128B)) return -3;
  }
  {
    uint64_t dims[2] = {(uint64_t)HID, (uint64_t)C}, str[1] = {(uint64_t)HID * 2};
    uint32_t box[2] = {64, 128};
    if (make_tmap(&tmW2, w2, CU_TENSOR_MAP_DATA_TYPE_BFLOAT16, 2, dims, str, box, CU_TENSOR_MAP_SWIZZLE_128B)) return -3;
  }
  CUtensorMap tmRes, tmOut;
  {
    uint64_t dims[2] = {(uint64_t)C, (uint64_t)M}, str[1] = {(uint64_t)C * 4};
    uint32_t box[2] = {32, 32};
    if (make_tmap(&tmRes, residual, CU_TENSOR_MAP_DATA_TYPE_FLOAT32, 2, dims, str, box, CU_TENSOR_MAP_SWIZZLE_128B)) return -3;
    if (make_tmap(&tmOut, out, CU_TENSOR_MAP_DATA_TYPE_FLOAT32, 2, dims, str, box, CU_TENSOR_MAP_SWIZZLE_128B)) return -3;
  }
  static bool configured = false;
  if (!configured) {
    cudaError_t e = cudaFuncSetAttribute(mlp_fused_kernel, cudaFuncAttributeMaxDynamicSharedMemorySize, SMEM);
    if (e != cudaSuccess) {
      set_error("convnext_mlp_fused: cannot opt in to %d B of shared memory: %s", SMEM, cudaGetErrorString(e));
      return -2;
    }
    configured = true;
  }
  Params p;
  p.row_stats = row_stats; p.col_s = col_s; p.cbias = cbias; p.b2 = b2; p.gamma = gamma; p.res = residual; p.out = out;
  p.M = (int)M; p.tiles = (int)(M / 128);
  const int grid = p.tiles < sm_count() ? p.tiles : sm_count();
  mlp_fused_kernel<<<grid, THREADS, SMEM, s>>>(tmY, tmW1, tmW2, tmRes, tmOut, p);
  DGTD_LAUNCH_CHECK("convnext_mlp_fused");
  return 0;
}
```

depth-guided-texture-diffusion-for-image-semantic-segmentation_b200/twig/model/texture_diffuser.py:

```python
from __future__ import annotations

import os

import math
from typing import Dict, List, Optional, Sequence, Tuple

import torch
import torch.nn as nn

from ..ops.capi import ACT_GELU, ACT_NONE, ACT_RELU, BF16, F32
from ..ops.functions import texture_diffusion_func as OP
from ..ops.functions import train_func as TF
from ..ops.functions import decoder_bank as DB

__all__ = [
    "LayerNorm", "ShapePropWeightRegressor", "convnext_Block", "ShapePropEncoder", "MessagePassing",
    "ShapePropDecoder", "prompt_encoder", "prompt_decoder", "DropPath", "init_weights_", "set_precision",
    "build_texture_diffuser", "pvt_token_grids", "texture_prompts", "texture_prompts_train", "PVT_EMBED_DIMS",
    "PVT_DEPTHS",
]

LN_FOLD = os.environ.get("DGTD_LN_FOLD", "1") != "0"

PVT_EMBED_DIMS = (64, 128, 320, 512)
PVT_DEPTHS = (3, 4, 6, 3)


def _mode(module: nn.Module) -> int:
    p = getattr(module, "_dgtd_precision", None)
    if p is None:
        p = "bf16" if torch.is_autocast_enabled() else "fp32"
    return BF16 if p == "bf16" else F32


def set_precision(module: nn.Module, precision: Optional[str]) -> nn.Module:
    assert precision in ("fp32", "bf16", None)
    for m in module.modules():
        m._dgtd_precision = precision
    return module


class _Packed:

    def __init__(self):
        self._store: Dict[str, Tuple[tuple, torch.Tensor]] = {}

    def get(self, key: str, srcs: Sequence[torch.Tensor], fn):
        sig = tuple((t.data_ptr(), t._version, t.device) for t in srcs)
        hit = self._store.get(key)
        if hit is not None and hit[0] == sig:
            return hit[1]
        with torch.no_grad():
            val = fn()
            if hit is not None and _refresh_in_place(hit[1], val):
                val = hit[1]
        self._store[key] = (sig, val)
        return val


def _refresh_in_place(old, new) -> bool:
    if isinstance(old, torch.Tensor) and isinstance(new, torch.Tensor):
        if old.shape != new.shape or old.dtype != new.dtype or old.device != new.device:
            return False
        if old.data_ptr() != new.data_ptr():
            old.copy_(new)
        return True
    if isinstance(old, (tuple, list)) and isinstance(new, (tuple, list)) and len(old) == len(new):
        ok = all(isinstance(a, torch.Tensor) and isinstance(b, torch.Tensor) and a.shape == b.shape and a.dtype == b.dtype
                 and a.device == b.device for a, b in zip(old, new))
        if not ok:
            return False
        for a, b in zip(old, new):
            if a.data_ptr() != b.data_ptr():
                a.copy_(b)
        return True
    return False


def _packed(module: nn.Module) -> _Packed:
    pk = module.__dict__.get("_dgtd_packed")
    if pk is None:
        pk = module.__dict__["_dgtd_packed"] = _Packed()
    return pk


_SCRATCH: Dict[tuple, torch.Tensor] = {}


def scratch_buffer(name: str, device: torch.device, numel: int, dtype: torch.dtype) -> torch.Tensor:
    if torch.cuda.is_current_stream_capturing():
        return torch.empty(numel, device=device, dtype=dtype)
    key = (name, device, torch.cuda.current_stream(device).cuda_stream, dtype)
    buf = _SCRATCH.get(key)
    if buf is None or buf.numel() < numel:
        buf = _SCRATCH[key] = torch.empty(numel, device=device, dtype=dtype)
    return buf


def _scratch(device: torch.device, numel: int) -> torch.Tensor:
    return scratch_buffer("block", device, numel, torch.float32)


def _as(t: torch.Tensor, mode: int) -> torch.Tensor:
    return t.detach().to(torch.bfloat16).contiguous() if mode == BF16 else t.detach().float().contiguous()


def _wants_grad(module: nn.Module, *inputs) -> bool:
    if not torch.is_grad_enabled():
        return False
    return any(p.requires_grad for p in module.parameters()) or any(
        isinstance(t, torch.Tensor) and t.requires_grad for t in inputs)


class DropPath(nn.Module):

    def __init__(self, drop_prob: float = 0.0, scale_by_keep: bool = True):
        super().__init__()
        self.drop_prob = drop_prob
        self.scale_by_keep = scale_by_keep

    def keep_scale(self, batch: int, device, dtype=torch.float32) -> Optional[torch.Tensor]:
        if self.drop_prob == 0.0 or not self.training:
            return None
        keep = 1.0 - self.drop_prob
        mask = torch.empty(batch, device=device, dtype=dtype).bernoulli_(keep)
        if keep > 0.0 and self.scale_by_keep:
            mask.div_(keep)
        return mask

    def forward(self, x):
        ks = self.keep_scale(x.shape[0], x.device, x.dtype)
        return x if ks is None else x * ks.view((-1,) + (1,) * (x.dim() - 1))


class LayerNorm(nn.Module):

    def __init__(self, normalized_shape, eps=1e-6, data_format="channels_last"):
        super().__init__()
        self.weight = nn.Parameter(torch.ones(normalized_shape))
        self.bias = nn.Parameter(torch.zeros(normalized_shape))
        self.eps = eps
        self.data_format = data_format
        if self.data_format not in ["channels_last", "channels_first"]:
            raise NotImplementedError
        self.normalized_shape = (normalized_shape,)

    def forward(self, x):
        if _wants_grad(self, x):
            if self.data_format == "channels_first":
                y = TF.LayerNormRowsFn.apply(TF.LayoutFn.apply(x, True), self.weight, self.bias, self.eps)
                return TF.LayoutFn.apply(y, False)
            return TF.LayerNormRowsFn.apply(x, self.weight, self.bias, self.eps)
        return OP.layer_norm(x.contiguous().float(), self.weight.detach(), self.bias.detach(), self.eps,
                             self.data_format == "channels_first")


class ShapePropWeightRegressor(nn.Module):

    def __init__(self, in_channels, latent_dim):
        super(ShapePropWeightRegressor, self).__init__()
        self.latent_dim = latent_dim
        self.reg = nn.Conv2d(in_channels, self.latent_dim * 49, kernel_size=1)

    def forward(self, x):
        return OP.conv1x1_nchw_autograd(x, self.reg.weight, self.reg.bias, True)


class convnext_Block(nn.Module):

    def __init__(self, dim, drop_path=0., layer_scale_init_value=1e-6):
        super().__init__()
        self.dwconv = nn.Conv2d(dim, dim, kernel_size=7, padding=3, groups=dim)
        self.norm = LayerNorm(dim, eps=1e-6)
        self.pwconv1 = nn.Linear(dim, 4 * dim)
        self.act = nn.GELU()
        self.pwconv2 = nn.Linear(4 * dim, dim)
        self.gamma = nn.Parameter(layer_scale_init_value * torch.ones((dim)),
                                  requires_grad=True) if layer_scale_init_value > 0 else None
        self.drop_path = DropPath(drop_path) if drop_path > 0. else nn.Identity()

    def _forward_nhwc(self, x: torch.Tensor, mode: int) -> torch.Tensor:
        pk = _packed(self)
        B, h, w, C = x.shape
        dw_w = pk.get("dw", [self.dwconv.weight], lambda: self.dwconv.weight.detach().reshape(C, 49).float().contiguous())
        w1 = pk.get(f"w1.{mode}", [self.pwconv1.weight], lambda: _as(self.pwconv1.weight, mode))
        w2 = pk.get(f"w2.{mode}", [self.pwconv2.weight], lambda: _as(self.pwconv2.weight, mode))
        keep = self.drop_path.keep_scale(B, x.device) if isinstance(self.drop_path, DropPath) else None
        gamma = self.gamma.detach() if self.gamma is not None else None
        if mode == BF16 and LN_FOLD and C % 128 == 0 and B * h * w >= 2048:
            dw_wT = pk.get("dwT", [self.dwconv.weight],
                           lambda: self.dwconv.weight.detach().reshape(C, 49).t().float().contiguous())

            def fold():
                w1f = self.pwconv1.weight.detach().float()
                wq = (w1f * self.norm.weight.detach().float()[None, :]).to(torch.bfloat16).contiguous()
                return (wq, wq.float().sum(1).contiguous(),
                        (w1f @ self.norm.bias.detach().float() + self.pwconv1.bias.detach().float()).contiguous())
            wq, col_s, cbias = pk.get("w1.lnfold", [self.pwconv1.weight, self.pwconv1.bias, self.norm.weight, self.norm.bias], fold)
            y, stats = OP.dwconv7_stats_tma(x, dw_wT, self.dwconv.bias.detach(), self.norm.eps)
            if keep is None and C in OP.MLP_FUSED_C and (B * h * w) % 128 == 0:
                OP.convnext_mlp_fused_(y.view(-1, C), stats, wq, col_s, cbias, w2, self.pwconv2.bias.detach(), gamma, x)
                return x
            hid = OP.linear_lnfold(y.view(-1, C), wq, cbias, col_s, stats, act=ACT_GELU)
            OP.linear_residual_(hid, w2, self.pwconv2.bias.detach(), gamma, keep, h * w, x)
            return x
        if C % 128 == 0 and B * h * w >= 2048:
            dw_wT = pk.get("dwT", [self.dwconv.weight],
                           lambda: self.dwconv.weight.detach().reshape(C, 49).t().float().contiguous())
            ws = _scratch(x.device, x.numel())
            a = OP.dwconv7_ln_tma(x, dw_wT, self.dwconv.bias.detach(), self.norm.weight.detach(),
                                  self.norm.bias.detach(), mode, ws, self.norm.eps)
        else:
            a = OP.dwconv7_ln(x, dw_w, self.dwconv.bias.detach(), self.norm.weight.detach(),
                              self.norm.bias.detach(), mode, self.norm.eps)
        hid = OP.linear(a.view(-1, C), w1, self.pwconv1.bias.detach(), act=ACT_GELU)
        OP.linear_residual_(hid, w2, self.pwconv2.bias.detach(), gamma, keep, h * w, x)
        return x

    def _forward_train(self, x: torch.Tensor, mode: int = F32) -> torch.Tensor:
        keep = self.drop_path.keep_scale(x.shape[0], x.device) if isinstance(self.drop_path, DropPath) else None
        M = x.shape[0] * x.shape[1] * x.shape[2]
        fn = TF.ConvNextBlockBf16Fn if (mode == BF16 and TF.tc_rows_ok(M) and x.shape[-1] % 128 == 0) else TF.ConvNextBlockFn
        return fn.apply(x, self.dwconv.weight, self.dwconv.bias, self.norm.weight, self.norm.bias,
                                        self.pwconv1.weight, self.pwconv1.bias, self.pwconv2.weight,
                                        self.pwconv2.bias, self.gamma, keep, self.norm.eps)

    def forward(self, x):
        if _wants_grad(self, x):
            return TF.LayoutFn.apply(self._forward_train(TF.LayoutFn.apply(x, True), _mode(self)), False)
        y = OP.nchw_to_nhwc(x.contiguous().float())
        y = self._forward_nhwc(y, _mode(self))
        return y.permute(0, 3, 1, 2)


class ShapePropEncoder(nn.Module):

    def __init__(self, in_channels, out_dim):
        super(ShapePropEncoder, self).__init__()
        self.downsample_layers = nn.ModuleList()
        dims = [128, 256, 512, 1024]
        stem = nn.Sequential(
            nn.Conv2d(3, dims[0], kernel_size=4, stride=4),
            LayerNorm(dims[0], eps=1e-6, data_format="channels_first")
        )
        self.downsample_layers.append(stem)
        for i in range(3):
            downsample_layer = nn.Sequential(
                LayerNorm(dims[i], eps=1e-6, data_format="channels_first"),
                nn.Conv2d(dims[i], dims[i + 1], kernel_size=2, stride=2),
            )
            self.downsample_layers.append(downsample_layer)

        self.stages = nn.ModuleList()
        drop_path_rate = 0.4
        depths = [3, 3, 27, 3]
        layer_scale_init_value = 1.0
        dp_rates = [x.item() for x in torch.linspace(0, drop_path_rate, sum(depths))]
        cur = 0
        for i in range(4):
            stage = nn.Sequential(
                *[convnext_Block(dim=dims[i], drop_path=dp_rates[cur + j],
                                 layer_scale_init_value=layer_scale_init_value) for j in range(depths[i])]
            )
            self.stages.append(stage)
            cur += depths[i]

        self.convs = nn.ModuleList()
        for i in range(4):
            self.convs.append(nn.Conv2d(dims[i], out_dim, 1))
        self.fusion_conv = nn.Conv2d(out_dim * 4, out_dim, 1)
        self.dims = dims
        self.out_dim = out_dim

    def _pyramid(self, image: torch.Tensor, grid: Optional[torch.Tensor], mode: int) -> List[torch.Tensor]:
        pk = _packed(self)
        st_conv, st_ln = self.downsample_layers[0][0], self.downsample_layers[0][1]
        w0 = pk.get("stem", [st_conv.weight], lambda: st_conv.weight.detach().reshape(self.dims[0], 48).float().contiguous())
        if mode == BF16 and self.dims[0] % 128 == 0 and image.shape[-1] % 4 == 0:
            w0b = pk.get("stem.bf16", [st_conv.weight], lambda: w0.to(torch.bfloat16))
            B, _, H, W = image.shape
            patches = OP.stem_patches(image, grid, BF16)
            if self.dims[0] == 128 and patches.shape[0] >= 256:
                x = OP.linear_ln(patches, w0b, st_conv.bias.detach().float(), st_ln.weight.detach().float(),
                                 st_ln.bias.detach().float(), st_ln.eps).view(B, H // 4, W // 4, self.dims[0])
            else:
                x = OP.linear(patches, w0b, st_conv.bias.detach(), out_dtype=F32)
                x = OP.ln_rows_(x, st_ln.weight.detach(), st_ln.bias.detach(), st_ln.eps).view(B, H // 4, W // 4, self.dims[0])
        else:
            x = OP.stem(image, grid, w0, st_conv.bias.detach(), st_ln.weight.detach(), st_ln.bias.detach(), st_ln.eps)
        outs = []
        for i in range(4):
            if i > 0:
                ln, conv = self.downsample_layers[i][0], self.downsample_layers[i][1]
                B, h, w, C = x.shape
                wd = pk.get(f"ds{i}.{mode}", [conv.weight],
                            lambda conv=conv, C=C: _as(conv.weight.detach().permute(0, 2, 3, 1).reshape(2 * C, 4 * C), mode))
                a = OP.ln_patchify(x, ln.weight.detach(), ln.bias.detach(), mode, ln.eps)
                x = OP.linear(a, wd, conv.bias.detach(), out_dtype=F32).view(B, h // 2, w // 2, 2 * C)
            for blk in self.stages[i]:
                x = blk._forward_nhwc(x, mode)
            outs.append(x)
        return outs

    def _head(self, outs: List[torch.Tensor], want_nchw: bool, pad_to: int = 0, mode: int = F32):
        pk = _packed(self)
        B = outs[0].shape[0]
        levels, hw = [], []
        L = self.out_dim
        fw = self.fusion_conv.weight
        for i, o in enumerate(outs):
            conv = self.convs[i]
            wl = pk.get(f"headf{i}", [conv.weight, fw],
                        lambda conv=conv, i=i: (fw.detach().reshape(L, 4 * L)[:, i * L:(i + 1) * L].float()
                                                @ conv.weight.detach().reshape(L, -1).float()).contiguous())
            bl = pk.get(f"headfb{i}", [conv.bias, fw],
                        lambda conv=conv, i=i: (fw.detach().reshape(L, 4 * L)[:, i * L:(i + 1) * L].float()
                                                @ conv.bias.detach().float()).contiguous())
            a = o.view(-1, o.shape[-1])
            if mode == BF16 and L % 8 == 0 and L <= 64:
                levels.append(OP.linear_tf32(a, wl, bl))
            else:
                levels.append(OP.linear(a, wl, bl, out_dtype=F32))
            hw.append((o.shape[1], o.shape[2]))
        return OP.fusion_sum(levels, hw, self.fusion_conv.bias.detach(), B, want_nhwc=True, want_nchw=want_nchw,
                             pad_to=pad_to)

    def _forward_train(self, image: torch.Tensor, grid: Optional[torch.Tensor], mode: int = F32) -> torch.Tensor:
        st_conv, st_ln = self.downsample_layers[0][0], self.downsample_layers[0][1]
        x = TF.StemFn.apply(image, grid, st_conv.weight, st_conv.bias, st_ln.weight, st_ln.bias, st_ln.eps)
        levels = []
        for i in range(4):
            if i > 0:
                ln, conv = self.downsample_layers[i][0], self.downsample_layers[i][1]
                Mo = x.shape[0] * (x.shape[1] // 2) * (x.shape[2] // 2)
                ds = TF.DownsampleBf16Fn if (mode == BF16 and TF.tc_rows_ok(Mo)) else TF.DownsampleFn
                x = ds.apply(x, ln.weight, ln.bias, conv.weight, conv.bias, ln.eps)
            for blk in self.stages[i]:
                x = blk._forward_train(x, mode)
            levels.append(TF.LinearFn.apply(x, self.convs[i].weight, self.convs[i].bias))
        return TF.FusionFn.apply(levels[0], levels[1], levels[2], levels[3], self.fusion_conv.weight,
                                 self.fusion_conv.bias)

    def forward(self, x):
        if _wants_grad(self, x):
            return TF.LayoutFn.apply(self._forward_train(x, None, _mode(self)), False)
        outs = self._pyramid(x.contiguous().float(), None, _mode(self))
        _, nchw, _ = self._head(outs, want_nchw=True, mode=_mode(self))
        return nchw


class MessagePassing(nn.Module):

    def __init__(self, latent_dim, img_size=384, k=7, max_step=4, sym_norm=False):
        super(MessagePassing, self).__init__()
        if k != 7:
            raise NotImplementedError("MessagePassing kernels are built for k=7 (cod.py:1181)")
        if sym_norm:
            raise NotImplementedError("sym_norm branch is dead code in the reference (cod.py:1194-1198)")
        self.k = k
        self.size = k * k
        self.max_step = max_step
        self.sym_norm = sym_norm
        self.img_size = img_size
        self.conv = nn.Conv2d(latent_dim, 3, 1)

    def forward(self, input, weight):
        n, c, h, w = input.size()
        steps = max(h, w) if self.max_step < 0 else self.max_step
        x = OP.message_passing_core(input, weight, steps, 1e-5)
        x = OP.conv1x1_nchw_autograd(x, self.conv.weight, self.conv.bias, False)
        size = self.img_size if isinstance(self.img_size, (tuple, list)) else (self.img_size, self.img_size)
        return OP.resize_bilinear_nchw_autograd(x, size)


_pack_conv3 = DB.pack_conv3
_fold_conv3_bilinear = DB.fold_conv3_bilinear
_pad_taps_bf16 = DB.pad_taps_bf16
_pad_rows = DB.pad_rows
_fold_params = DB.fold_params


class ShapePropDecoder(nn.Module):

    def __init__(self, out_dim, latent_dim):
        super(ShapePropDecoder, self).__init__()
        dilation = 1
        self.decoder = nn.Sequential(
            nn.Conv2d(latent_dim, latent_dim, kernel_size=3, stride=1, padding=dilation, dilation=dilation),
            nn.ReLU(True),
            nn.Conv2d(latent_dim, latent_dim, kernel_size=3, stride=1, padding=dilation, dilation=dilation),
            nn.ReLU(True),
            nn.Conv2d(latent_dim, out_dim, kernel_size=3, stride=1, padding=dilation, dilation=dilation),
        )

    def _forward_train(self, emb_nhwc: torch.Tensor) -> torch.Tensor:
        d = self.decoder
        y = TF.Conv3x3Fn.apply(emb_nhwc, d[0].weight, d[0].bias, True)
        y = TF.Conv3x3Fn.apply(y, d[2].weight, d[2].bias, True)
        return TF.Conv3x3Fn.apply(y, d[4].weight, d[4].bias, False)

    def forward(self, embedding):
        if _wants_grad(self, embedding):
            return self._forward_train(TF.LayoutFn.apply(embedding, True)).permute(0, 3, 1, 2)
        return _decode_full([self], OP.nchw_to_nhwc(embedding.contiguous().float()))[0]


def _decoder_front(decoders: Sequence[ShapePropDecoder], emb: torch.Tensor) -> torch.Tensor:
    B, h, w, L = emb.shape
    D = len(decoders)
    host = decoders[0]
    pk = _packed(host)
    ws = [d.decoder[0].weight for d in decoders]
    key = "c1." + ".".join(str(id(d)) for d in decoders)
    w1 = pk.get(key + ".w", ws, lambda: torch.cat([_pack_conv3(t) for t in ws], 0).contiguous())
    b1 = pk.get(key + ".b", [d.decoder[0].bias for d in decoders],
                lambda: torch.cat([d.decoder[0].bias.detach().float() for d in decoders]).contiguous())
    h1 = OP.conv_nhwc(emb, w1, b1, L, (h, w), 3, 1, -1, act=ACT_RELU)
    h2 = torch.empty_like(h1)
    for i, d in enumerate(decoders):
        w2 = _packed(d).get("c2", [d.decoder[2].weight], lambda d=d: _pack_conv3(d.decoder[2].weight))
        OP.conv_nhwc(h1[..., i * L:(i + 1) * L], w2, d.decoder[2].bias.detach(), L, (h, w), 3, 1, -1,
                     act=ACT_RELU, out=h2[..., i * L:(i + 1) * L], Cout=L)
    return h2


def _decoder_front_bf16(decoders: Sequence[ShapePropDecoder], emb_pad: torch.Tensor) -> torch.Tensor:
    B, h, w, _ = emb_pad.shape
    D = len(decoders)
    L = decoders[0].decoder[0].in_channels
    pk = _packed(decoders[0])
    key = "bf16." + ".".join(str(id(d)) for d in decoders)
    w1 = pk.get(key + ".w1", [d.decoder[0].weight for d in decoders],
                lambda: torch.cat([_pad_taps_bf16(_pack_conv3(d.decoder[0].weight), L, 32) for d in decoders], 0).contiguous())
    b1 = pk.get(key + ".b1", [d.decoder[0].bias for d in decoders],
                lambda: torch.cat([_pad_rows(d.decoder[0].bias, 32) for d in decoders]).contiguous())
    w2 = pk.get(key + ".w2", [d.decoder[2].weight for d in decoders],
                lambda: torch.cat([_pad_taps_bf16(_pack_conv3(d.decoder[2].weight), L, 32) for d in decoders], 0).contiguous())
    b2 = pk.get(key + ".b2", [d.decoder[2].bias for d in decoders],
                lambda: torch.cat([_pad_rows(d.decoder[2].bias, 32) for d in decoders]).contiguous())
    gs = B * h * w * 32
    h1 = torch.empty(D, B, h, w, 32, device=emb_pad.device, dtype=torch.bfloat16)
    OP.conv_nhwc_grouped(emb_pad, w1, b1, 32, (h, w), 3, 1, -1, ACT_RELU, h1, 32 * D, 32, 1, 0, 32 * D, gs)
    h2 = torch.empty_like(h1)
    OP.conv_nhwc_grouped(h1[0], w2, b2, 32, (h, w), 3, 1, -1, ACT_RELU, h2, 32, 32, D, gs, 32, gs)
    return h2


def _decode_tokens_bf16(decoders: Sequence[ShapePropDecoder], h2: torch.Tensor, index0: int,
                        src_hw: Tuple[int, int], grid: Tuple[int, int]) -> List[torch.Tensor]:
    B = h2.shape[1]
    D = len(decoders)
    E = decoders[0].decoder[4].out_channels
    L = decoders[0].decoder[4].in_channels
    h, w = src_hw
    fold = _fold_params((h, w), grid)
    pk = _packed(decoders[0])
    key = f"bf16.c3.{grid}." + ".".join(str(id(d)) for d in decoders)
    ws = [d.decoder[4].weight for d in decoders]
    if (h, w) == tuple(grid):
        ks, stride, off = 3, 1, -1
        w3 = pk.get(key, ws, lambda: torch.cat([_pad_taps_bf16(_pack_conv3(t), L) for t in ws], 0).contiguous())
    elif fold is not None:
        ks, stride, off = 4, fold[0], fold[1]
        w3 = pk.get(key, ws, lambda: torch.cat([_pad_taps_bf16(_fold_conv3_bilinear(t), L) for t in ws], 0).contiguous())
    else:
        raise NotImplementedError(f"bf16 prompt injection needs an integer power-of-two ratio, got {(h, w)} -> {grid}")
    b3 = pk.get(key + ".b", [d.decoder[4].bias for d in decoders],
                lambda: torch.cat([d.decoder[4].bias.detach().float() for d in decoders]).contiguous())
    out = torch.empty(D, B, grid[0] * grid[1], E, device=h2.device, dtype=torch.bfloat16)
    OP.conv_nhwc_grouped(h2[index0], w3, b3, 32, grid, ks, stride, off, ACT_NONE, out, E, E, D, h2.stride(0), E,
                         B * grid[0] * grid[1] * E)
    return [out[i] for i in range(D)]


def _decode_full(decoders: Sequence[ShapePropDecoder], emb: torch.Tensor) -> List[torch.Tensor]:
    B, h, w, L = emb.shape
    h2 = _decoder_front(decoders, emb)
    outs = []
    for i, d in enumerate(decoders):
        w3 = _packed(d).get("c3", [d.decoder[4].weight], lambda d=d: _pack_conv3(d.decoder[4].weight))
        y = OP.conv_nhwc(h2[..., i * L:(i + 1) * L], w3, d.decoder[4].bias.detach(), L, (h, w), 3, 1, -1)
        outs.append(y.permute(0, 3, 1, 2))
    return outs


def _decode_tokens(decoders: Sequence[ShapePropDecoder], emb: torch.Tensor, grid: Tuple[int, int],
                   h2: Optional[torch.Tensor] = None, index0: int = 0) -> List[torch.Tensor]:
    B, h, w, L = emb.shape
    if h2 is None:
        h2 = _decoder_front(decoders, emb)
        index0 = 0
    outs = []
    fold = _fold_params((h, w), grid)
    for i, d in enumerate(decoders):
        src = h2[..., (index0 + i) * L:(index0 + i + 1) * L]
        conv = d.decoder[4]
        if (h, w) == tuple(grid):
            w3 = _packed(d).get("c3", [conv.weight], lambda conv=conv: _pack_conv3(conv.weight))
            y = OP.conv_nhwc(src, w3, conv.bias.detach(), L, grid, 3, 1, -1)
        elif fold is not None:
            w4 = _packed(d).get("c3fold", [conv.weight], lambda conv=conv: _fold_conv3_bilinear(conv.weight))
            y = OP.conv_nhwc(src, w4, conv.bias.detach(), L, grid, 4, fold[0], fold[1])
        else:
            w3 = _packed(d).get("c3", [conv.weight], lambda conv=conv: _pack_conv3(conv.weight))
            y = OP.resize_nhwc(OP.conv_nhwc(src, w3, conv.bias.detach(), L, (h, w), 3, 1, -1), grid)
        outs.append(y.view(B, grid[0] * grid[1], -1))
    return outs


class prompt_encoder(nn.Module):

    def __init__(self, latent_dim, embed_dim, depth, fusion=False):
        super(prompt_encoder, self).__init__()
        self.embed_dim = embed_dim
        self.depth = depth
        self.propagation_weight_regressor = ShapePropWeightRegressor(3, latent_dim)
        self.encoder1 = nn.Conv2d(1, latent_dim, 1)
        self.encoder2 = ShapePropEncoder(3, 24)
        self.adaptor = nn.Conv2d(6, 3, 1)
        self.message_passing = MessagePassing(latent_dim, img_size=384, sym_norm=False)
        self.freq_nums = 0.3
        self.latent_dim = latent_dim

    def fft(self, x, rate):
        return OP.fft_highpass(x.contiguous().float(), rate)

    def _forward_fused(self, image: torch.Tensor, cues: torch.Tensor, mode: int, want_nchw: bool = True,
                       pad_to: int = 0):
        H = 12
        image = image.contiguous().float()
        cues = cues.contiguous().float()
        x = OP.fft_highpass(image, self.freq_nums, tensor_cores=(mode == BF16))
        reg = self.propagation_weight_regressor.reg
        mp = self.message_passing
        pk = _packed(self)
        reg_w = pk.get("reg", [reg.weight], lambda: reg.weight.detach().reshape(reg.out_channels, 3).float().contiguous())
        enc_w = pk.get("enc1", [self.encoder1.weight], lambda: self.encoder1.weight.detach().reshape(-1).float().contiguous())
        mp_w = pk.get("mpc", [mp.conv.weight], lambda: mp.conv.weight.detach().reshape(3, -1).float().contiguous())
        steps = H if mp.max_step < 0 else mp.max_step
        grid3, _, _ = OP.diffusion_front(x, cues, reg_w, reg.bias.detach(), enc_w, self.encoder1.bias.detach(),
                                         mp_w, mp.conv.bias.detach(), grid=H, steps=steps)
        outs = self.encoder2._pyramid(image, grid3, mode)
        nhwc, nchw, pad = self.encoder2._head(outs, want_nchw=want_nchw, pad_to=pad_to, mode=mode)
        return x, nhwc, nchw, pad

    def _forward_train(self, image: torch.Tensor, cues: torch.Tensor, mode: Optional[int] = None):
        mode = _mode(self) if mode is None else mode
        H = 12
        image = image.contiguous().float()
        x = self.fft(image, self.freq_nums)
        xx = OP.resize_nchw(x, (H, H), bilinear=False)
        weights = self.propagation_weight_regressor(xx)
        c12 = OP.resize_bilinear_nchw_autograd(cues.contiguous().float(), (H, H))
        d12 = OP.conv1x1_nchw_autograd(c12, self.encoder1.weight, self.encoder1.bias, False)
        mp = self.message_passing
        steps = H if mp.max_step < 0 else mp.max_step
        core = OP.message_passing_core(d12, weights, steps, 1e-5)
        grid3 = OP.conv1x1_nchw_autograd(core, mp.conv.weight, mp.conv.bias, False)
        return x, self.encoder2._forward_train(image, grid3, mode)

    def forward(self, image, cues, cross=False):
        if _wants_grad(self, cues):
            x, emb3 = self._forward_train(image, cues)
            return x, TF.LayoutFn.apply(emb3, False)
        x, _, emb3, _ = self._forward_fused(image, cues, _mode(self), want_nchw=True)
        return x, emb3


class prompt_decoder(nn.Module):

    def __init__(self, latent_dim, embed_dim, depth, fusion=False):
        super(prompt_decoder, self).__init__()
        self.depth = depth
        self.decoder = nn.Sequential(*[ShapePropDecoder(embed_dim, 24) for i in range(depth)])

    def forward(self, embedding, cross=False):
        if _wants_grad(self, embedding):
            emb = TF.LayoutFn.apply(embedding, True)
            return [d._forward_train(emb).permute(0, 3, 1, 2) for d in self.decoder]
        emb = OP.nchw_to_nhwc(embedding.contiguous().float())
        return _decode_full(list(self.decoder), emb)


def init_weights_(module: nn.Module) -> None:
    if isinstance(module, nn.Linear):
        nn.init.trunc_normal_(module.weight, std=.02)
        if module.bias is not None:
            nn.init.constant_(module.bias, 0)
    elif isinstance(module, nn.LayerNorm):
        nn.init.constant_(module.bias, 0)
        nn.init.constant_(module.weight, 1.0)
    elif isinstance(module, nn.Conv2d):
        fan_out = module.kernel_size[0] * module.kernel_size[1] * module.out_channels
        fan_out //= module.groups
        module.weight.data.normal_(0, math.sqrt(2.0 / fan_out))
        if module.bias is not None:
            module.bias.data.zero_()


def build_texture_diffuser(seed: Optional[int] = None, embed_dims=PVT_EMBED_DIMS, depths=PVT_DEPTHS,
                           latent_dim: int = 24):
    if seed is not None:
        torch.manual_seed(seed)
    enc = prompt_encoder(latent_dim, list(embed_dims), list(depths), True)
    dec = nn.Sequential(*[prompt_decoder(latent_dim, embed_dims[i], depths[i], True) for i in range(len(depths))])
    enc.apply(init_weights_)
    dec.apply(init_weights_)
    return enc, dec


def pvt_token_grids(img_hw: Sequence[int]) -> List[Tuple[int, int]]:
    h, w = int(img_hw[0]), int(img_hw[1])
    h, w = (h + 6 - 7) // 4 + 1, (w + 6 - 7) // 4 + 1
    out = [(h, w)]
    for _ in range(3):
        h, w = (h + 2 - 3) // 2 + 1, (w + 2 - 3) // 2 + 1
        out.append((h, w))
    return out


def texture_prompts_train(enc: "prompt_encoder", dec: nn.Sequential, image: torch.Tensor, depth: torch.Tensor,
                          precision: Optional[str] = None):
    mode = _mode(enc) if precision is None else (BF16 if precision == "bf16" else F32)
    emb1, emb3 = enc._forward_train(image, depth, mode)
    grids = pvt_token_grids(image.shape[-2:])
    B = image.shape[0]
    if DB.bank_supported(tuple(emb3.shape[1:3]), grids):
        cfg = {"stages": [(len(dec[s].decoder), tuple(grids[s])) for s in range(len(dec))], "mode": mode}
        params = [t for s in range(len(dec)) for d in dec[s].decoder
                  for t in (d.decoder[0].weight, d.decoder[0].bias, d.decoder[2].weight, d.decoder[2].bias,
                            d.decoder[4].weight, d.decoder[4].bias)]
        flat = DB.DecoderBankFn.apply(emb3, cfg, *params)
        tokens, i = [], 0
        for s in range(len(dec)):
            n = len(dec[s].decoder)
            tokens.append(list(flat[i:i + n]))
            i += n
        return emb1, TF.LayoutFn.apply(emb3, False), tokens
    tokens = []
    for s in range(len(dec)):
        row = []
        for d in dec[s].decoder:
            y = d._forward_train(emb3)
            if tuple(y.shape[1:3]) != tuple(grids[s]):
                y = TF.ResizeNHWCFn.apply(y, grids[s])
            row.append(y.reshape(B, grids[s][0] * grids[s][1], -1))
        tokens.append(row)
    return emb1, TF.LayoutFn.apply(emb3, False), tokens


@torch.no_grad()
def texture_prompts(enc: "prompt_encoder", dec: nn.Sequential, image: torch.Tensor, depth: torch.Tensor,
                    precision: Optional[str] = None, want_embedding3: bool = True):
    return _texture_prompts_infer(enc, dec, image, depth, precision, want_embedding3)


def _texture_prompts_infer(enc: "prompt_encoder", dec: nn.Sequential, image: torch.Tensor, depth: torch.Tensor,
                           precision: Optional[str] = None, want_embedding3: bool = True):
    mode = _mode(enc) if precision is None else (BF16 if precision == "bf16" else F32)
    grids = pvt_token_grids(image.shape[-2:])
    all_dec = [d for s in range(len(dec)) for d in dec[s].decoder]
    src_hw = (image.shape[-2] // 4, image.shape[-1] // 4)
    tc_ok = mode == BF16 and all(tuple(g) == src_hw or _fold_params(src_hw, g) is not None for g in grids)
    emb1, nhwc, nchw, pad = enc._forward_fused(image, depth, mode, want_nchw=want_embedding3,
                                               pad_to=32 if tc_ok else 0)
    tokens, idx = [], 0
    if tc_ok:
        h2 = _decoder_front_bf16(all_dec, pad)
        for s in range(len(dec)):
            ds = list(dec[s].decoder)
            tokens.append(_decode_tokens_bf16(ds, h2, idx, src_hw, grids[s]))
            idx += len(ds)
        return emb1, nchw, tokens
    h2 = _decoder_front(all_dec, nhwc)
    for s in range(len(dec)):
        ds = list(dec[s].decoder)
        tokens.append(_decode_tokens(ds, nhwc, grids[s], h2=h2, index0=idx))
        idx += len(ds)
    return emb1, nchw, tokens
```

depth-guided-texture-diffusion-for-image-semantic-segmentation_b200/twig/ops/capi.py:

```python
from __future__ import annotations

import ctypes
import os
from ctypes import c_char_p, c_float, c_int, c_int64, c_void_p
from typing import Optional

import torch

_HERE = os.path.dirname(os.path.abspath(__file__))
LIB_PATH = os.path.join(_HERE, "libdgtd_ops.so")

F32, BF16 = 0, 1
ACT_NONE, ACT_GELU, ACT_RELU = 0, 1, 2

_P, _I, _L, _F = c_void_p, c_int, c_int64, c_float

SIGNATURES = {
    "dgtd_version": [],
    "dgtd_last_error": [],
    "dgtd_launch_count": [],
    "dgtd_surface_normals_fwd": [_P, _P, _I, _I, _I, _P],
    "dgtd_lowpass_projector": [_P, _P, _I, _I, _P],
    "dgtd_fft_highpass_fwd": [_P, _P, _P, _P, _P, _P, _P, _P, _I, _I, _I, _P],
    "dgtd_fft_highpass_tc3_fwd": [_P, _P, _P, _P, _P, _P, _P, _P, _P, _I, _I, _I, _P],
    "dgtd_diffusion_front_fwd": [_P] * 11 + [_I] * 6 + [_P],
    "dgtd_message_passing_fwd": [_P, _P, _P, _P, _I, _I, _I, _I, _I, _I, _F, _P],
    "dgtd_message_passing_tiled_fwd": [_P, _P, _P, _P, _I, _I, _I, _I, _I, _F, _I, _P],
    "dgtd_message_passing_tiled_simt_fwd": [_P, _P, _P, _P, _I, _I, _I, _I, _I, _F, _I, _P],
    "dgtd_message_passing_tc_fwd": [_P, _P, _P, _P, _I, _I, _I, _I, _I, _F, _I, _P],
    "dgtd_pack_regressor": [_P, _P, _P, _I, _P],
    "dgtd_message_passing_regress_fwd": [_P, _P, _P, _P, _P, _I, _I, _I, _I, _I, _F, _I, _I, _P],
    "dgtd_message_passing_bwd": [_P, _P, _P, _P, _P, _I, _I, _I, _I, _I, _I, _F, _P],
    "dgtd_conv1x1_nchw_fwd": [_P, _P, _P, _P, _I, _I, _I, _I, _I, _P],
    "dgtd_conv1x1_nchw_bwd": [_P, _P, _P, _P, _P, _P, _P, _I, _I, _I, _I, _P],
    "dgtd_resize_bilinear_nchw_bwd": [_P, _P, _I, _I, _I, _I, _I, _P],
    "dgtd_resize_nchw_fwd": [_P, _P, _I, _I, _I, _I, _I, _I, _P],
    "dgtd_resize_sigmoid_sized_fwd": [_P, _P, _P, _I, _I, _I, _I, _I, _P],
    "dgtd_layer_norm_fwd": [_P, _P, _P, _P, _L, _I, _L, _F, _P],
    "dgtd_stem_fwd": [_P, _P, _I, _P, _P, _P, _P, _P, _I, _I, _I, _I, _F, _P],
    "dgtd_ln_patchify_fwd": [_P, _P, _P, _P, _I, _I, _I, _I, _I, _F, _P],
    "dgtd_dwconv7_ln_fwd": [_P, _P, _P, _P, _P, _P, _I, _I, _I, _I, _I, _F, _P],
    "dgtd_dwconv7_ln_tma_fwd": [_P, _P, _P, _P, _P, _P, _P, _I, _I, _I, _I, _I, _F, _P],
    "dgtd_linear_fwd": [_P, _P, _P, _P, _I, _I, _I, _I, _I, _I, _I, _P],
    "dgtd_dwconv7_stats_tma_fwd": [_P, _P, _P, _P, _P, _I, _I, _I, _I, _F, _P],
    "dgtd_linear_ln_fwd": [_P, _P, _P, _P, _P, _F, _P, _I, _I, _I, _P],
    "dgtd_linear_tf32_fwd": [_P, _P, _P, _P, _I, _I, _I, _I, _P],
    "dgtd_linear_lnfold_fwd": [_P, _P, _P, _P, _P, _P, _I, _I, _I, _I, _I, _I, _P],
    "dgtd_linear_residual_fwd": [_P, _P, _P, _P, _P, _I, _P, _P, _I, _I, _I, _I, _P],
    "dgtd_convnext_mlp_fused_fwd": [_P, _P, _P, _P, _P, _P, _P, _P, _P, _P, _L, _I, _P],
    "dgtd_fusion_sum_fwd": [_P, _P, _P, _P, _P, _P, _P, _P, _P, _I, _I, _I, _P],
    "dgtd_conv_nhwc_fwd": [_P, _P, _P, _P] + [_I] * 15 + [_P],
    "dgtd_conv_nhwc_grouped_fwd": [_P, _P, _P, _P] + [_I] * 16 + [_L, _I, _L, _P],
    "dgtd_resize_nhwc_fwd": [_P, _P, _I, _I, _I, _I, _I, _I, _I, _I, _P],
    "dgtd_linear_dgrad": [_P, _P, _P, _P, _P, _P, _I, _I, _I, _I, _I, _P],
    "dgtd_linear_wgrad": [_P, _P, _P, _P, _P] + [_I] * 13 + [_P],
    "dgtd_linear_wgrad_ws_floats": [_I, _I, _I],
    "dgtd_colsum": [_P, _P, _I, _P, _P, _I, _I, _P],
    "dgtd_layer_scale_finalize": [_P, _P, _P, _P, _P, _P, _P, _P, _I, _I, _P],
    "dgtd_gelu_fwd": [_P, _P, _L, _P],
    "dgtd_relu_bwd": [_P, _P, _P, _L, _P],
    "dgtd_ln_rows_bwd": [_P, _P, _P, _P, _P, _P, _P, _L, _I, _F, _P],
    "dgtd_ln_rows_bwd_ws_floats": [_L, _I],
    "dgtd_dwconv7_fwd": [_P, _P, _P, _P, _P, _I, _I, _I, _I, _I, _P],
    "dgtd_dwconv7_wgrad": [_P, _P, _P, _P, _P, _I, _I, _I, _I, _P],
    "dgtd_stem_patchify": [_P, _P, _I, _P, _I, _I, _I, _I, _P],
    "dgtd_stem_unpatchify": [_P, _P, _I, _I, _I, _P],
    "dgtd_patchify2": [_P, _P, _I, _I, _I, _I, _P],
    "dgtd_unpatchify2": [_P, _P, _I, _I, _I, _I, _P],
    "dgtd_resize_nhwc_bwd": [_P, _P, _I, _I, _I, _I, _I, _I, _I, _P],
    "dgtd_transpose_op": [_P, _P, _P, _P, _P, _P, _I, _I, _I, _I, _P],
    "dgtd_colsum_bf16": [_P, _P, _P, _I, _I, _P],
    "dgtd_eltwise_colsum_ws_floats": [_I, _I],
    "dgtd_eltwise_colsum": [_P, _P, _P, _P, _I, _P, _P, _I, _I, _I, _P],
    "dgtd_wgrad_tc_ws_floats": [_I, _I, _I],
    "dgtd_wgrad_tc_mn": [_P, _I, _P, _I, _P, _P, _I, _I, _I, _I, _P],
    "dgtd_ln_rows_fwd": [_P, _P, _P, _P, _I, _L, _I, _F, _P],
    "dgtd_ln_tokens_fwd": [_P, _P, _I, _P, _P, _P, _P, _I, _L, _I, _F, _P],
    "dgtd_patchify_tokens_fwd": [_P, _P, _I, _I, _I, _I, _I, _I, _P],
    "dgtd_dwconv3_gelu_fwd": [_P, _P, _P, _P, _I, _I, _I, _I, _I, _P],
    "dgtd_dwconv3_fwd": [_P, _P, _P, _P, _I, _I, _I, _I, _I, _P],
    "dgtd_attention_fwd": [_P, _P, _P, _I, _I, _I, _I, _I, _F, _P],
    "dgtd_attention_bwd_ws_floats": [_I, _I, _I, _I],
    "dgtd_attention_bwd": [_P, _P, _P, _P, _P, _P, _P, _I, _I, _I, _I, _I, _F, _P],
    "dgtd_dwconv3_gelu_bwd_ws_floats": [],
    "dgtd_dwconv3_gelu_bwd": [_P, _P, _P, _P, _P, _P, _P, _P, _I, _I, _I, _I, _I, _P],
    "dgtd_boundary_weight_fwd": [_P, _P, _I, _I, _I, _P],
    "dgtd_structure_loss_ws_floats": [_I, _L],
    "dgtd_structure_loss_fwd": [_P, _P, _P, _P, _P, _P, _I, _L, _P],
    "dgtd_structure_loss_bwd": [_P, _P, _P, _P, _P, _P, _I, _L, _P],
    "dgtd_col2im_nhwc": [_P, _I, _I, _I, _P, _I, _P, _I, _I, _I, _I, _I, _I, _I, _I, _I, _I, _I, _P],
    "dgtd_im2col_nhwc": [_P, _I, _P, _I, _I, _I, _I, _I, _I, _I, _I, _I, _P],
    "dgtd_group_sum": [_P, _I, _P, _L, _I, _I, _I, _P],
    "dgtd_cast_fwd": [_P, _P, _L, _I, _I, _P],
    "dgtd_nhwc_to_nchw_fwd": [_P, _P, _I, _I, _I, _I, _I, _I, _P],
    "dgtd_nchw_to_nhwc_fwd": [_P, _P, _I, _I, _I, _I, _I, _I, _P],
    "dgtd_conv_nhwc_affine_fwd": [_P, _P, _P, _P, _P, _P, _I, _P] + [_I] * 12 + [_P],
    "dgtd_channel_sums_chunks": [_I],
    "dgtd_channel_sums_fwd": [_P, _I, _P, _I, _I, _I, _P],
    "dgtd_channel_gate_fwd": [_P, _I, _I, _P, _P, _P, _I, _I, _I, _I, _P],
    "dgtd_gated_sum_fwd": [_P, _I, _P, _P, _P, _I, _P, _P, _P, _I, _I, _I, _I, _P],
    "dgtd_resize_nhwc_ld_fwd": [_P, _I, _P, _I] + [_I] * 7 + [_P],
    "dgtd_copy_channels_fwd": [_P, _I, _P, _I, _L, _I, _P],
    "dgtd_head1_fwd": [_P, _I, _P, _P, _P, _L, _I, _I, _P],
    "dgtd_sigmoid_fwd": [_P, _P, _L, _P],
    "dgtd_cast_pad_act_fwd": [_P, _I, _P, _P, _L, _I, _I, _P],
    "dgtd_conv3x3_tc_fwd": [_P, _P, _P, _P, _I, _I, _I, _I, _I, _I, _P],
    "dgtd_im2col_act_fwd": [_P, _I, _P, _P] + [_I] * 9 + [_P],
    "dgtd_col_stats_ws_bytes": [_L, _I],
    "dgtd_bn_train_fwd": [_P, _I, _P, _P, _P, _P, _F, _F, _P, _I, _P, _P, _P, _L, _I, _P],
    "dgtd_bn_apply_fwd": [_P, _I, _P, _P, _P, _P, _P, _I, _L, _I, _P],
    "dgtd_bn_train_bwd": [_P, _I, _P, _I, _P, _P, _P, _P, _I, _P, _P, _P, _I, _L, _I, _P],
    "dgtd_prelu_fwd": [_P, _P, _P, _L, _P],
    "dgtd_prelu_bwd_ws_bytes": [_L],
    "dgtd_prelu_bwd": [_P, _P, _P, _P, _P, _P, _L, _P],
    "dgtd_channel_dot_fwd": [_P, _I, _P, _I, _P, _I, _I, _I, _P],
    "dgtd_gate_bwd_ws_floats": [_I, _I, _I, _I],
    "dgtd_gate_bwd": [_P, _I, _I, _P, _I, _P, _P, _P, _P, _P, _P, _P, _P, _P, _P, _I, _I, _I, _I, _I, _P],
    "dgtd_gated_bwd": [_P, _I, _P, _P, _P, _P, _I, _I, _I, _I, _P],
    "dgtd_head1_bwd": [_P, _P, _I, _P, _P, _I, _P, _P, _P, _L, _I, _P],
    "dgtd_resize_nhwc_ld_bwd": [_P, _I, _P, _I] + [_I] * 7 + [_P],
    "dgtd_ssim_loss_ws_floats": [_L],
    "dgtd_ssim_loss_fwd": [_P, _P, _P, _P, _I, _I, _I, _P],
    "dgtd_adamw_slice_bytes": [],
    "dgtd_adamw_step": [_P, _P, _P, _P, _P, _I, _F, _F, _F, _I, _F, _F, _P],
    "dgtd_sod_metrics_ws_bytes": [_I, _I, _I],
    "dgtd_sod_metrics_fwd": [_P, _P, _P, _P, _P, _I, _I, _I, _P],
    "dgtd_sod_wfm_ws_bytes": [_I, _I, _I],
    "dgtd_sod_wfm_fwd": [_P, _P, _P, _P, _I, _I, _I, _P],
    "dgtd_sod_metrics_sized_fwd": [_P, _P, _P, _P, _P, _P, _I, _I, _I, _P],
    "dgtd_sod_wfm_sized_fwd": [_P, _P, _P, _P, _P, _I, _I, _I, _P],
}
_RESTYPES = {"dgtd_last_error": c_char_p, "dgtd_launch_count": c_int64, "dgtd_sod_metrics_ws_bytes": c_int64,
             "dgtd_sod_wfm_ws_bytes": c_int64,
             "dgtd_col_stats_ws_bytes": c_int64, "dgtd_attention_bwd_ws_floats": c_int64, "dgtd_dwconv3_gelu_bwd_ws_floats": c_int64, "dgtd_gate_bwd_ws_floats": c_int64, "dgtd_prelu_bwd_ws_bytes": c_int64}

_lib: Optional[ctypes.CDLL] = None


def load() -> ctypes.CDLL:
    global _lib
    if _lib is not None:
        return _lib
    if not os.path.exists(LIB_PATH):
        raise RuntimeError(
            f"{LIB_PATH} is missing: build it with `python -m dgtd_b200.twig.ops.build` "
            "(there is no CPU or PyTorch fallback for the texture-diffusion kernels)")
    lib = ctypes.CDLL(LIB_PATH)
    for name, argtypes in SIGNATURES.items():
        fn = getattr(lib, name)
        fn.argtypes = argtypes
        fn.restype = _RESTYPES.get(name, c_int)
    if lib.dgtd_version() != 100:
        raise RuntimeError(f"libdgtd_ops.so version {lib.dgtd_version()} != 100 (stale build?)")
    _lib = lib
    return lib


def last_error() -> str:
    msg = load().dgtd_last_error()
    return msg.decode() if msg else ""


def launch_count() -> int:
    return int(load().dgtd_launch_count())


def ptr(t: Optional[torch.Tensor]) -> Optional[int]:
    if t is None:
        return None
    return t.data_ptr()


def stream() -> int:
    return torch.cuda.current_stream().cuda_stream


def dtype_code(dt: torch.dtype) -> int:
    if dt == torch.float32:
        return F32
    if dt == torch.bfloat16:
        return BF16
    raise TypeError(f"dgtd ops support float32 / bfloat16 only, got {dt}")


_PROF = {"on": False, "events": []}


def enable_profile(on: bool = True) -> None:
    _PROF["on"] = bool(on)
    _PROF["events"] = []


def profile_summary() -> dict:
    torch.cuda.synchronize()
    out = {}
    for name, a, b in _PROF["events"]:
        e = out.setdefault(name, [0, 0.0])
        e[0] += 1
        e[1] += a.elapsed_time(b)
    return out


def call(name: str, *args) -> None:
    lib = load()
    if _PROF["on"]:
        a, b = torch.cuda.Event(enable_timing=True), torch.cuda.Event(enable_timing=True)
        a.record()
        rc = getattr(lib, name)(*args)
        b.record()
        _PROF["events"].append((name, a, b))
    else:
        rc = getattr(lib, name)(*args)
    if rc != 0:
        raise RuntimeError(f"{name} failed ({rc}): {last_error()}")


def check_cuda(*tensors: Optional[torch.Tensor]) -> None:
    for t in tensors:
        if t is None:
            continue
        if not t.is_cuda:
            raise RuntimeError("dgtd ops run on CUDA tensors only (no CPU fallback); got a "
                               f"{t.device} tensor")
        if not t.is_contiguous():
            raise RuntimeError("dgtd ops need contiguous tensors")
```

depth-guided-texture-diffusion-for-image-semantic-segmentation_b200/twig/ops/functions/texture_diffusion_func.py:

```python
from __future__ import annotations

from typing import List, Optional, Sequence, Tuple

import torch
from torch.autograd import Function
from torch.autograd.function import once_differentiable

from .. import capi
from ..capi import ACT_GELU, ACT_NONE, ACT_RELU, BF16, F32, call, check_cuda, ptr, stream

__all__ = [
    "surface_normals", "HighpassPlan", "fft_highpass", "diffusion_front", "MessagePassingFunction",
    "message_passing_core", "message_passing_tiled", "conv1x1_nchw_autograd", "resize_bilinear_nchw_autograd", "conv1x1_nchw", "resize_nchw", "layer_norm",
    "stem", "stem_patches", "ln_rows_", "fusion_sum", "ln_patchify", "dwconv7_ln", "dwconv7_ln_tma", "linear", "linear_ln", "linear_tf32", "linear_residual_", "conv_nhwc", "conv_nhwc_grouped",
    "resize_nhwc", "cast", "nhwc_to_nchw", "nchw_to_nhwc", "enable_gemm_profile", "collect_gemm_profile",
]


_PROFILE = {"on": False, "events": []}


def enable_gemm_profile(on: bool = True):
    _PROFILE["on"] = bool(on)
    _PROFILE["events"] = []
    return _PROFILE


def collect_gemm_profile(min_n: int = 0, min_k: int = 0):
    torch.cuda.synchronize()
    ev = [e for e in _PROFILE["events"] if e[3] is None or (e[3][1] >= min_n and e[3][2] >= min_k)]
    flops = sum(e[0] for e in ev)
    ms = sum(e[1].elapsed_time(e[2]) for e in ev)
    return flops, ms, len(ev)


class _timed:
    def __init__(self, flops: float, active: bool, shape=None):
        self.flops, self.active, self.shape = flops, active and _PROFILE["on"], shape

    def __enter__(self):
        if self.active:
            self.a = torch.cuda.Event(enable_timing=True)
            self.b = torch.cuda.Event(enable_timing=True)
            self.a.record()

    def __exit__(self, *exc):
        if self.active:
            self.b.record()
            _PROFILE["events"].append((self.flops, self.a, self.b, self.shape))


def _tdtype(code: int) -> torch.dtype:
    return torch.float32 if code == F32 else torch.bfloat16


def surface_normals(depth: torch.Tensor) -> torch.Tensor:
    check_cuda(depth)
    B, _, H, W = depth.shape
    out = torch.empty(B, 3, H, W, device=depth.device, dtype=torch.float32)
    call("dgtd_surface_normals_fwd", ptr(depth), ptr(out), B, H, W, stream())
    return out


class HighpassPlan:

    _cache = {}

    def __init__(self, H: int, W: int, rate: float, device: torch.device):
        line = int((W * H * rate) ** 0.5 // 2)
        self.H, self.W, self.line = H, W, line
        self.Ph = torch.empty(H, H, device=device, dtype=torch.float32)
        self.sc_h = torch.empty(2 * H, device=device, dtype=torch.float32)
        call("dgtd_lowpass_projector", ptr(self.Ph), ptr(self.sc_h), H, line, stream())
        if W == H:
            self.Pw, self.sc_w = self.Ph, self.sc_h
        else:
            self.Pw = torch.empty(W, W, device=device, dtype=torch.float32)
            self.sc_w = torch.empty(2 * W, device=device, dtype=torch.float32)
            call("dgtd_lowpass_projector", ptr(self.Pw), ptr(self.sc_w), W, line, stream())

    @classmethod
    def get(cls, H: int, W: int, rate: float, device: torch.device) -> "HighpassPlan":
        key = (H, W, float(rate), device.index)
        plan = cls._cache.get(key)
        if plan is None:
            plan = cls._cache[key] = cls(H, W, rate, device)
        return plan


def _split_bf16(t: torch.Tensor):
    hi = t.to(torch.bfloat16)
    return hi.contiguous(), (t - hi.float()).to(torch.bfloat16).contiguous()


def fft_highpass(x: torch.Tensor, rate: float = 0.3, tensor_cores: bool = False) -> torch.Tensor:
    check_cuda(x)
    assert x.dtype == torch.float32 and x.dim() == 4
    B, C, H, W = x.shape
    plan = HighpassPlan.get(H, W, rate, x.device)
    if tensor_cores and H % 8 == 0 and W % 8 == 0:
        if not hasattr(plan, "tc3"):
            def cat(t):
                hi, lo = _split_bf16(t)
                return torch.cat([hi, hi, lo], 1).contiguous()
            ph = cat(plan.Ph)
            plan.tc3 = (ph, ph if plan.Pw is plan.Ph else cat(plan.Pw))
        ph_cat, pw_cat = plan.tc3
        n = x.numel()
        ws_a = torch.empty(3 * n, device=x.device, dtype=torch.bfloat16)
        ws_f = torch.empty(n, device=x.device, dtype=torch.float32)
        coef = torch.empty(B * C * 4, device=x.device, dtype=torch.float32)
        out = torch.empty_like(x)
        call("dgtd_fft_highpass_tc3_fwd", ptr(x), ptr(ph_cat), ptr(pw_cat), ptr(plan.sc_h), ptr(plan.sc_w), ptr(ws_a),
             ptr(ws_f), ptr(coef), ptr(out), B * C, H, W, stream())
        return out
    tmp = torch.empty_like(x)
    coef = torch.empty(B * C * 4, device=x.device, dtype=torch.float32)
    out = torch.empty_like(x)
    call("dgtd_fft_highpass_fwd", ptr(x), ptr(plan.Ph), ptr(plan.Pw), ptr(plan.sc_h), ptr(plan.sc_w),
         ptr(tmp), ptr(coef), ptr(out), B * C, H, W, stream())
    return out


def diffusion_front(emb1: torch.Tensor, depth: torch.Tensor, reg_w, reg_b, enc_w, enc_b, conv_w, conv_b,
                    grid: int = 12, steps: int = 4, save_wn: bool = False):
    check_cuda(emb1, depth, reg_w, reg_b, enc_w, enc_b, conv_w, conv_b)
    B, _, H, W = emb1.shape
    C = enc_w.shape[0]
    out = torch.empty(B, 3, grid, grid, device=emb1.device, dtype=torch.float32)
    states = torch.empty(B, steps + 1, C, grid, grid, device=emb1.device, dtype=torch.float32)
    wn = torch.empty(B, C, 49, grid * grid, device=emb1.device, dtype=torch.float32) if save_wn else None
    call("dgtd_diffusion_front_fwd", ptr(emb1), ptr(depth), ptr(reg_w), ptr(reg_b), ptr(enc_w), ptr(enc_b),
         ptr(conv_w), ptr(conv_b), ptr(out), ptr(states), ptr(wn), B, H, W, grid, C, steps, stream())
    return out, states, wn


class MessagePassingFunction(Function):

    @staticmethod
    def forward(ctx, x: torch.Tensor, weight: torch.Tensor, steps: int, eps: float):
        x = x.contiguous().float()
        weight = weight.contiguous().float()
        check_cuda(x, weight)
        n, c, h, w = x.shape
        wc = weight.shape[1] // 49
        out = torch.empty_like(x)
        need_grad = x.requires_grad or weight.requires_grad
        states = torch.empty(n, steps + 1, c, h, w, device=x.device, dtype=torch.float32) if need_grad else None
        call("dgtd_message_passing_fwd", ptr(x), ptr(weight), ptr(out), ptr(states), n, c, h, w, wc, steps,
             float(eps), stream())
        if need_grad:
            ctx.save_for_backward(weight, states)
        ctx.cfg = (n, c, h, w, wc, steps, float(eps))
        return out

    @staticmethod
    @once_differentiable
    def backward(ctx, grad_out):
        weight, states = ctx.saved_tensors
        n, c, h, w, wc, steps, eps = ctx.cfg
        grad_out = grad_out.contiguous().float()
        gx = torch.empty(n, c, h, w, device=grad_out.device, dtype=torch.float32)
        gw = torch.empty_like(weight)
        call("dgtd_message_passing_bwd", ptr(grad_out), ptr(weight), ptr(states), ptr(gx), ptr(gw), n, c, h,
             w, wc, steps, eps, stream())
        return gx, gw, None, None


def message_passing_core(x: torch.Tensor, weight: torch.Tensor, steps: int = 4, eps: float = 1e-5):
    return MessagePassingFunction.apply(x, weight, steps, eps)


class Conv1x1NCHWFunction(Function):

    @staticmethod
    def forward(ctx, x, weight, bias, sigmoid: bool):
        x = x.contiguous().float()
        w2 = weight.reshape(weight.shape[0], -1).contiguous().float()
        out = conv1x1_nchw(x, w2, None if bias is None else bias.contiguous().float(), sigmoid)
        ctx.sigmoid = bool(sigmoid)
        ctx.wshape = tuple(weight.shape)
        ctx.has_bias = bias is not None
        ctx.save_for_backward(x, w2, out if sigmoid else None)
        return out

    @staticmethod
    @once_differentiable
    def backward(ctx, g):
        x, w2, y = ctx.saved_tensors
        g = g.contiguous().float()
        B, Cin = x.shape[0], x.shape[1]
        HW = x.numel() // (B * Cin)
        Cout = w2.shape[0]
        gx = torch.empty_like(x) if ctx.needs_input_grad[0] else None
        gw = torch.empty_like(w2) if (ctx.needs_input_grad[1] or ctx.needs_input_grad[2]) else None
        gb = torch.empty(Cout, device=x.device, dtype=torch.float32) if gw is not None else None
        call("dgtd_conv1x1_nchw_bwd", ptr(g), ptr(y), ptr(x), ptr(w2), ptr(gx), ptr(gw), ptr(gb), B, Cin, Cout, HW,
             stream())
        return (gx, gw.reshape(ctx.wshape) if gw is not None and ctx.needs_input_grad[1] else None,
                gb if ctx.has_bias and ctx.needs_input_grad[2] else None, None)


class ResizeBilinearNCHWFunction(Function):

    @staticmethod
    def forward(ctx, x, size):
        x = x.contiguous().float()
        ctx.in_hw = (x.shape[2], x.shape[3])
        ctx.out_hw = (int(size[0]), int(size[1]))
        return resize_nchw(x, ctx.out_hw, bilinear=True)

    @staticmethod
    @once_differentiable
    def backward(ctx, g):
        g = g.contiguous().float()
        B, C = g.shape[0], g.shape[1]
        gx = torch.empty(B, C, ctx.in_hw[0], ctx.in_hw[1], device=g.device, dtype=torch.float32)
        call("dgtd_resize_bilinear_nchw_bwd", ptr(g), ptr(gx), B * C, ctx.in_hw[0], ctx.in_hw[1], ctx.out_hw[0],
             ctx.out_hw[1], stream())
        return gx, None


def conv1x1_nchw_autograd(x, weight, bias, sigmoid: bool = False):
    return Conv1x1NCHWFunction.apply(x, weight, bias, sigmoid)


def resize_bilinear_nchw_autograd(x, size):
    return ResizeBilinearNCHWFunction.apply(x, size)


def message_passing_tiled(x: torch.Tensor, weight: torch.Tensor, steps: int, eps: float = 1e-5, impl: str = "auto"):
    check_cuda(x, weight)
    n, h, w, c = x.shape
    out = torch.empty_like(x)
    tmp = torch.empty_like(x) if steps > 1 else None
    if impl == "tc":
        call("dgtd_message_passing_tc_fwd", ptr(x), ptr(weight), ptr(out), ptr(tmp), n, h, w, c, steps,
             float(eps), capi.dtype_code(x.dtype), stream())
        return out
    assert impl in ("auto", "simt")
    call("dgtd_message_passing_tiled_fwd" if impl == "auto" else "dgtd_message_passing_tiled_simt_fwd", ptr(x),
         ptr(weight), ptr(out), ptr(tmp), n, h, w, c, steps, float(eps), capi.dtype_code(x.dtype), stream())
    return out


def message_passing_regress(x: torch.Tensor, guide: torch.Tensor, reg_w: torch.Tensor, reg_b: torch.Tensor,
                            steps: int, eps: float = 1e-5, fast_sigmoid: bool = False) -> torch.Tensor:
    check_cuda(x, guide, reg_w, reg_b)
    n, h, w, c = x.shape
    assert guide.shape == (n, 3, h, w) and reg_w.numel() == c * 49 * 3 and reg_b.numel() == c * 49
    packed = torch.empty(c * 49, 4, device=x.device, dtype=torch.float32)
    call("dgtd_pack_regressor", ptr(reg_w.detach().reshape(c * 49, 3).float().contiguous()),
         ptr(reg_b.detach().float().contiguous()), ptr(packed), c, stream())
    out = torch.empty_like(x)
    tmp = torch.empty_like(x) if steps > 1 else None
    call("dgtd_message_passing_regress_fwd", ptr(x), ptr(guide.contiguous().float()), ptr(packed), ptr(out), ptr(tmp),
         n, h, w, c, steps, float(eps), capi.dtype_code(x.dtype), int(fast_sigmoid), stream())
    return out


def conv1x1_nchw(x: torch.Tensor, w: torch.Tensor, b: Optional[torch.Tensor], sigmoid: bool = False):
    check_cuda(x, w, b)
    B, Cin = x.shape[0], x.shape[1]
    HW = x.numel() // (B * Cin)
    Cout = w.shape[0]
    out = torch.empty((B, Cout) + tuple(x.shape[2:]), device=x.device, dtype=torch.float32)
    call("dgtd_conv1x1_nchw_fwd", ptr(x), ptr(w), ptr(b), ptr(out), B, Cin, Cout, HW, int(sigmoid), stream())
    return out


def resize_nchw(x: torch.Tensor, size: Sequence[int], bilinear: bool = True) -> torch.Tensor:
    check_cuda(x)
    B, C, h, w = x.shape
    oh, ow = int(size[0]), int(size[1])
    out = torch.empty(B, C, oh, ow, device=x.device, dtype=torch.float32)
    call("dgtd_resize_nchw_fwd", ptr(x), ptr(out), B * C, h, w, oh, ow, int(bilinear), stream())
    return out


def layer_norm(x: torch.Tensor, w: torch.Tensor, b: torch.Tensor, eps: float, channels_first: bool):
    check_cuda(x, w, b)
    out = torch.empty_like(x)
    if channels_first:
        outer, C = x.shape[0], x.shape[1]
        inner = x.numel() // (outer * C)
    else:
        C = x.shape[-1]
        outer, inner = x.numel() // C, 1
    call("dgtd_layer_norm_fwd", ptr(x), ptr(w), ptr(b), ptr(out), outer, C, inner, float(eps), stream())
    return out


def stem(image: torch.Tensor, grid: Optional[torch.Tensor], w, b, ln_w, ln_b, eps: float = 1e-6):
    check_cuda(image, grid, w, b, ln_w, ln_b)
    B, _, H, W = image.shape
    Cout = w.shape[0]
    out = torch.empty(B, H // 4, W // 4, Cout, device=image.device, dtype=torch.float32)
    G = grid.shape[-1] if grid is not None else 0
    call("dgtd_stem_fwd", ptr(image), ptr(grid), G, ptr(w), ptr(b), ptr(ln_w), ptr(ln_b), ptr(out), B, H, W,
         Cout, float(eps), stream())
    return out


def ln_patchify(x: torch.Tensor, ln_w, ln_b, out_dtype: int, eps: float = 1e-6) -> torch.Tensor:
    check_cuda(x, ln_w, ln_b)
    B, h, w, C = x.shape
    out = torch.empty(B * (h // 2) * (w // 2), 4 * C, device=x.device, dtype=_tdtype(out_dtype))
    call("dgtd_ln_patchify_fwd", ptr(x), ptr(ln_w), ptr(ln_b), ptr(out), out_dtype, B, h, w, C, float(eps),
         stream())
    return out


def dwconv7_ln(x: torch.Tensor, dw_w, dw_b, ln_w, ln_b, out_dtype: int, eps: float = 1e-6) -> torch.Tensor:
    check_cuda(x, dw_w, dw_b, ln_w, ln_b)
    B, h, w, C = x.shape
    out = torch.empty(B, h, w, C, device=x.device, dtype=_tdtype(out_dtype))
    call("dgtd_dwconv7_ln_fwd", ptr(x), ptr(dw_w), ptr(dw_b), ptr(ln_w), ptr(ln_b), ptr(out), out_dtype, B, h,
         w, C, float(eps), stream())
    return out


def dwconv7_ln_tma(x: torch.Tensor, dw_wT, dw_b, ln_w, ln_b, out_dtype: int, ws: torch.Tensor,
                   eps: float = 1e-6) -> torch.Tensor:
    check_cuda(x, dw_wT, dw_b, ln_w, ln_b, ws)
    B, h, w, C = x.shape
    assert ws.numel() >= x.numel() and ws.dtype == torch.float32
    out = torch.empty(B, h, w, C, device=x.device, dtype=_tdtype(out_dtype))
    call("dgtd_dwconv7_ln_tma_fwd", ptr(x), ptr(dw_wT), ptr(dw_b), ptr(ln_w), ptr(ln_b), ptr(ws), ptr(out),
         out_dtype, B, h, w, C, float(eps), stream())
    return out


def dwconv7_stats_tma(x: torch.Tensor, dw_wT, dw_b, eps: float = 1e-6):
    check_cuda(x, dw_wT, dw_b)
    B, h, w, C = x.shape
    y = torch.empty(B, h, w, C, device=x.device, dtype=torch.bfloat16)
    stats = torch.empty(B * h * w, 2, device=x.device, dtype=torch.float32)
    call("dgtd_dwconv7_stats_tma_fwd", ptr(x), ptr(dw_wT), ptr(dw_b), ptr(y), ptr(stats), B, h, w, C, float(eps), stream())
    return y, stats


def linear_lnfold(a: torch.Tensor, w: torch.Tensor, bias: torch.Tensor, col_s: torch.Tensor, row_stats: torch.Tensor,
                  act: int = ACT_NONE, out_dtype: int = BF16) -> torch.Tensor:
    check_cuda(a, w, bias, col_s, row_stats)
    K = a.shape[-1]
    M = a.numel() // K
    N = w.shape[0]
    assert w.shape[1] == K and a.dtype == torch.bfloat16 and w.dtype == torch.bfloat16 and row_stats.shape == (M, 2)
    out = torch.empty(tuple(a.shape[:-1]) + (N,), device=a.device, dtype=_tdtype(out_dtype))
    with _timed(2.0 * M * N * K, True, (M, N, K)):
        call("dgtd_linear_lnfold_fwd", ptr(a), ptr(w), ptr(bias), ptr(col_s), ptr(row_stats), ptr(out), M, N, K, N,
             out_dtype, act, stream())
    return out


def linear(a: torch.Tensor, w: torch.Tensor, bias: Optional[torch.Tensor], act: int = ACT_NONE,
           out_dtype: Optional[int] = None, out: Optional[torch.Tensor] = None) -> torch.Tensor:
    check_cuda(a, w, bias)
    K = a.shape[-1]
    M = a.numel() // K
    N = w.shape[0]
    assert w.shape[1] == K and a.dtype == w.dtype
    din = capi.dtype_code(a.dtype)
    dout = din if out_dtype is None else out_dtype
    if out is None:
        out = torch.empty(tuple(a.shape[:-1]) + (N,), device=a.device, dtype=_tdtype(dout))
    ldo = out.shape[-1]
    with _timed(2.0 * M * N * K, din == BF16, (M, N, K)):
        call("dgtd_linear_fwd", ptr(a), ptr(w), ptr(bias), ptr(out), M, N, K, ldo, din, dout, act, stream())
    return out


def linear_ln(a: torch.Tensor, w: torch.Tensor, bias, ln_w: torch.Tensor, ln_b: torch.Tensor, eps: float) -> torch.Tensor:
    check_cuda(a, w, bias, ln_w, ln_b)
    K = a.shape[-1]
    M = a.numel() // K
    N = w.shape[0]
    assert w.shape[1] == K and a.dtype == torch.bfloat16 and w.dtype == torch.bfloat16 and a.is_contiguous()
    out = torch.empty(tuple(a.shape[:-1]) + (N,), device=a.device, dtype=torch.float32)
    call("dgtd_linear_ln_fwd", ptr(a), ptr(w), ptr(bias), ptr(ln_w), ptr(ln_b), float(eps), ptr(out), M, N, K, stream())
    return out


def linear_tf32(a: torch.Tensor, w: torch.Tensor, bias: Optional[torch.Tensor]) -> torch.Tensor:
    check_cuda(a, w, bias)
    K = a.shape[-1]
    M = a.numel() // K
    N = w.shape[0]
    assert w.shape[1] == K and a.dtype == torch.float32 and w.dtype == torch.float32 and a.is_contiguous()
    out = torch.empty(tuple(a.shape[:-1]) + (N,), device=a.device, dtype=torch.float32)
    call("dgtd_linear_tf32_fwd", ptr(a), ptr(w), ptr(bias), ptr(out), M, N, K, N, stream())
    return out


def linear_residual_(a: torch.Tensor, w: torch.Tensor, bias, gamma, keep: Optional[torch.Tensor],
                     rows_per_sample: int, residual: torch.Tensor, out: Optional[torch.Tensor] = None):
    check_cuda(a, w, bias, gamma, keep, residual)
    K = a.shape[-1]
    M = a.numel() // K
    N = w.shape[0]
    assert residual.dtype == torch.float32 and residual.numel() == M * N
    out = residual if out is None else out
    with _timed(2.0 * M * N * K, a.dtype == torch.bfloat16, (M, N, K)):
        call("dgtd_linear_residual_fwd", ptr(a), ptr(w), ptr(bias), ptr(gamma), ptr(keep), rows_per_sample,
             ptr(residual), ptr(out), M, N, K, capi.dtype_code(a.dtype), stream())
    return out


MLP_FUSED_C = (128,)


def convnext_mlp_fused_(y: torch.Tensor, row_stats: torch.Tensor, w1: torch.Tensor, col_s: torch.Tensor,
                        cbias: torch.Tensor, w2: torch.Tensor, b2: torch.Tensor, gamma: Optional[torch.Tensor],
                        residual: torch.Tensor, out: Optional[torch.Tensor] = None) -> torch.Tensor:
    check_cuda(y, row_stats, w1, col_s, cbias, w2, b2, gamma, residual)
    C = y.shape[-1]
    M = y.numel() // C
    assert y.dtype == torch.bfloat16 and w1.dtype == torch.bfloat16 and w2.dtype == torch.bfloat16
    assert w1.shape == (4 * C, C) and w2.shape == (C, 4 * C) and row_stats.shape == (M, 2)
    assert residual.dtype == torch.float32 and residual.numel() == M * C
    out = residual if out is None else out
    with _timed(4.0 * M * C * 4 * C, True, (M, 4 * C, C)):
        call("dgtd_convnext_mlp_fused_fwd", ptr(y), ptr(row_stats), ptr(w1), ptr(col_s), ptr(cbias), ptr(w2), ptr(b2),
             ptr(gamma), ptr(residual), ptr(out), M, C, stream())
    return out


def fusion_sum(levels: List[torch.Tensor], hw: List[Tuple[int, int]], bias, B: int, want_nhwc=True,
               want_nchw=False, pad_to: int = 0):
    check_cuda(*levels, bias)
    C = levels[0].shape[-1]
    dev = levels[0].device
    h0, w0 = hw[0]
    nhwc = torch.empty(B, h0, w0, C, device=dev, dtype=torch.float32) if want_nhwc else None
    nchw = torch.empty(B, C, h0, w0, device=dev, dtype=torch.float32) if want_nchw else None
    pad = torch.empty(B, h0, w0, pad_to, device=dev, dtype=torch.bfloat16) if pad_to else None
    hw_arr = (capi.c_int * 8)(*[v for pair in hw for v in pair])
    call("dgtd_fusion_sum_fwd", ptr(levels[0]), ptr(levels[1]), ptr(levels[2]), ptr(levels[3]), hw_arr,
         ptr(bias), ptr(nhwc), ptr(nchw), ptr(pad), pad_to, B, C, stream())
    return nhwc, nchw, pad


def stem_patches(image: torch.Tensor, grid: Optional[torch.Tensor], out_dtype: int) -> torch.Tensor:
    check_cuda(image, grid)
    B, _, H, W = image.shape
    out = torch.empty(B * (H // 4) * (W // 4), 48, device=image.device, dtype=_tdtype(out_dtype))
    call("dgtd_stem_patchify", ptr(image), ptr(grid), grid.shape[-1] if grid is not None else 0, ptr(out), out_dtype,
         B, H, W, stream())
    return out


def ln_rows_(y: torch.Tensor, ln_w, ln_b, eps: float = 1e-6) -> torch.Tensor:
    check_cuda(y, ln_w, ln_b)
    C = y.shape[-1]
    call("dgtd_ln_rows_fwd", ptr(y), ptr(ln_w), ptr(ln_b), ptr(y), F32, y.numel() // C, C, float(eps), stream())
    return y


def conv_nhwc(x: torch.Tensor, w: torch.Tensor, bias, Cin: int, out_hw: Tuple[int, int], ks: int,
              stride: int, off: int, act: int = ACT_NONE, out: Optional[torch.Tensor] = None,
              out_dtype: Optional[int] = None, Cout: Optional[int] = None) -> torch.Tensor:
    B, h, wd = x.shape[0], x.shape[1], x.shape[2]
    ldx = x.stride(2)
    assert x.stride(3) == 1 and x.stride(1) == wd * ldx and x.stride(0) == h * wd * ldx
    Cout = w.shape[0] if Cout is None else Cout
    oh, ow = out_hw
    din = capi.dtype_code(x.dtype)
    dout = din if out_dtype is None else out_dtype
    if out is None:
        out = torch.empty(B, oh, ow, Cout, device=x.device, dtype=_tdtype(dout))
    ldo = out.stride(2)
    call("dgtd_conv_nhwc_fwd", x.data_ptr(), ptr(w), ptr(bias), out.data_ptr(), B, h, wd, Cin, ldx, oh, ow,
         Cout, ldo, ks, stride, off, act, din, dout, stream())
    return out


def conv_nhwc_grouped(x: torch.Tensor, w: torch.Tensor, bias, Cin: int, out_hw: Tuple[int, int], ks: int,
                      stride: int, off: int, act: int, out: torch.Tensor, Cout: int, ldo: int, groups: int,
                      x_group_stride: int, w_group_rows: int, out_group_stride: int) -> torch.Tensor:
    B, h, wd = x.shape[0], x.shape[1], x.shape[2]
    ldx = x.stride(2)
    assert x.stride(3) == 1 and x.stride(1) == wd * ldx and x.stride(0) == h * wd * ldx
    oh, ow = out_hw
    call("dgtd_conv_nhwc_grouped_fwd", x.data_ptr(), ptr(w), ptr(bias), out.data_ptr(), B, h, wd, Cin, ldx,
         oh, ow, Cout, ldo, ks, stride, off, act, capi.dtype_code(x.dtype), capi.dtype_code(out.dtype), groups,
         x_group_stride, w_group_rows, out_group_stride, stream())
    return out


def resize_nhwc(x: torch.Tensor, size: Tuple[int, int], out_dtype: Optional[int] = None) -> torch.Tensor:
    check_cuda(x)
    B, h, w, C = x.shape
    din = capi.dtype_code(x.dtype)
    dout = din if out_dtype is None else out_dtype
    out = torch.empty(B, size[0], size[1], C, device=x.device, dtype=_tdtype(dout))
    call("dgtd_resize_nhwc_fwd", ptr(x), ptr(out), B, h, w, C, size[0], size[1], din, dout, stream())
    return out


def cast(x: torch.Tensor, dtype: torch.dtype) -> torch.Tensor:
    check_cuda(x)
    out = torch.empty(x.shape, device=x.device, dtype=dtype)
    call("dgtd_cast_fwd", ptr(x), ptr(out), x.numel(), capi.dtype_code(x.dtype), capi.dtype_code(dtype),
         stream())
    return out


def nhwc_to_nchw(x: torch.Tensor, C: Optional[int] = None) -> torch.Tensor:
    check_cuda(x)
    B, h, w, ld = x.shape
    C = ld if C is None else C
    out = torch.empty(B, C, h, w, device=x.device, dtype=torch.float32)
    call("dgtd_nhwc_to_nchw_fwd", ptr(x), ptr(out), B, h, w, C, ld, capi.dtype_code(x.dtype), stream())
    return out


def nchw_to_nhwc(x: torch.Tensor, dtype: torch.dtype = torch.float32, ld: Optional[int] = None):
    check_cuda(x)
    B, C, h, w = x.shape
    ld = C if ld is None else ld
    out = torch.empty(B, h, w, ld, device=x.device, dtype=dtype)
    call("dgtd_nchw_to_nhwc_fwd", ptr(x), ptr(out), B, h, w, C, ld, capi.dtype_code(dtype), stream())
    return out
```

include/dgtd_ops.h:

```cpp
#ifndef DGTD_OPS_H_
#define DGTD_OPS_H_

#include <stddef.h>
#include <stdint.h>

#ifdef __cplusplus
extern "C" {
#endif

#define DGTD_VERSION 100
#define DGTD_F32 0
#define DGTD_BF16 1

#define DGTD_ACT_NONE 0
#define DGTD_ACT_GELU 1
#define DGTD_ACT_RELU 2

typedef void* dgtd_stream_t;

int dgtd_version(void);
const char* dgtd_last_error(void);
int64_t dgtd_launch_count(void);

int dgtd_surface_normals_fwd(const float* depth, float* normals, int B, int H, int W,
                             dgtd_stream_t stream);

int dgtd_lowpass_projector(float* P, float* sc, int n, int line, dgtd_stream_t stream);
int dgtd_fft_highpass_fwd(const float* x, const float* Ph, const float* Pw, const float* sc_h,
                          const float* sc_w, float* tmp, float* coef, float* out, int planes,
                          int H, int W, dgtd_stream_t stream);
int dgtd_fft_highpass_tc3_fwd(const float* x, const void* Ph_cat, const void* Pw_cat, const float* sc_h, const float* sc_w,
                              void* ws_a, float* ws_f32, float* coef, float* out, int planes, int H, int W,
                              dgtd_stream_t stream);

int dgtd_diffusion_front_fwd(const float* emb1, const float* depth, const float* reg_w,
                             const float* reg_b, const float* enc_w, const float* enc_b,
                             const float* conv_w, const float* conv_b, float* out_grid,
                             float* save_states, float* save_wn, int B, int H, int W, int G, int C,
                             int T, dgtd_stream_t stream);

int dgtd_message_passing_fwd(const float* x, const float* weight, float* out, float* save_states,
                             int n, int c, int h, int w, int wc, int T, float eps,
                             dgtd_stream_t stream);
int dgtd_message_passing_tiled_fwd(const void* x, const float* weight, void* out, void* tmp,
                                   int n, int h, int w, int c, int T, float eps, int dtype,
                                   dgtd_stream_t stream);
int dgtd_message_passing_tiled_simt_fwd(const void* x, const float* weight, void* out, void* tmp,
                                        int n, int h, int w, int c, int T, float eps, int dtype,
                                        dgtd_stream_t stream);
int dgtd_message_passing_tc_fwd(const void* x, const float* weight, void* out, void* tmp,
                                int n, int h, int w, int c, int T, float eps, int dtype,
                                dgtd_stream_t stream);
int dgtd_pack_regressor(const float* wr, const float* br, float* packed, int c, dgtd_stream_t stream);
int dgtd_message_passing_regress_fwd(const void* x, const float* guide, const float* packed, void* out, void* tmp,
                                     int n, int h, int w, int c, int T, float eps, int dtype, int fast_sigmoid,
                                     dgtd_stream_t stream);
int dgtd_message_passing_bwd(const float* grad_out, const float* weight, const float* states,
                             float* grad_x, float* grad_weight, int n, int c, int h, int w, int wc,
                             int T, float eps, dgtd_stream_t stream);

int dgtd_conv1x1_nchw_fwd(const float* x, const float* w, const float* b, float* out, int B,
                          int Cin, int Cout, int HW, int sigmoid, dgtd_stream_t stream);
int dgtd_conv1x1_nchw_bwd(const float* grad_out, const float* y_out, const float* x, const float* w,
                          float* grad_x, float* grad_w, float* grad_b, int B, int Cin, int Cout, int HW,
                          dgtd_stream_t stream);
int dgtd_resize_bilinear_nchw_bwd(const float* grad_out, float* grad_x, int planes, int h, int w, int oh,
                                  int ow, dgtd_stream_t stream);
int dgtd_resize_nchw_fwd(const float* x, float* out, int planes, int h, int w, int oh, int ow,
                         int bilinear, dgtd_stream_t stream);
int dgtd_resize_sigmoid_sized_fwd(const float* x, float* out, const int32_t* sizes, int B, int h, int w, int Hmax,
                                  int Wmax, dgtd_stream_t stream);
int dgtd_layer_norm_fwd(const float* x, const float* w, const float* b, float* out, int64_t outer,
                        int C, int64_t inner, float eps, dgtd_stream_t stream);

int dgtd_stem_fwd(const float* image, const float* grid, int G, const float* w, const float* b,
                  const float* ln_w, const float* ln_b, float* out, int B, int H, int W, int Cout,
                  float eps, dgtd_stream_t stream);
int dgtd_ln_patchify_fwd(const float* x, const float* ln_w, const float* ln_b, void* out,
                         int out_dtype, int B, int h, int w, int C, float eps,
                         dgtd_stream_t stream);

int dgtd_dwconv7_ln_fwd(const float* x, const float* dw_w, const float* dw_b, const float* ln_w,
                        const float* ln_b, void* out, int out_dtype, int B, int h, int w, int C,
                        float eps, dgtd_stream_t stream);
int dgtd_dwconv7_ln_tma_fwd(const float* x, const float* dw_wT, const float* dw_b, const float* ln_w,
                            const float* ln_b, float* ws, void* out, int out_dtype, int B, int h, int w,
                            int C, float eps, dgtd_stream_t stream);
int dgtd_dwconv7_stats_tma_fwd(const float* x, const float* dw_wT, const float* dw_b, void* y, float* stats, int B,
                               int h, int w, int C, float eps, dgtd_stream_t stream);
int dgtd_linear_ln_fwd(const void* a, const void* w, const float* bias, const float* ln_w, const float* ln_b, float eps,
                       float* out, int M, int N, int K, dgtd_stream_t stream);
int dgtd_linear_tf32_fwd(const float* a, const float* w, const float* bias, float* out, int M, int N, int K, int ldo,
                         dgtd_stream_t stream);
int dgtd_linear_lnfold_fwd(const void* a, const void* w, const float* bias, const float* col_s, const float* row_stats,
                           void* out, int M, int N, int K, int ldo, int dtype_out, int act, dgtd_stream_t stream);
int dgtd_convnext_mlp_fused_fwd(const void* y, const float* row_stats, const void* w1, const float* col_s,
                                const float* cbias, const void* w2, const float* b2, const float* gamma,
                                const float* residual, float* out, int64_t M, int C, dgtd_stream_t stream);
int dgtd_linear_fwd(const void* a, const void* w, const float* bias, void* out, int M, int N,
                    int K, int ldo, int dtype_in, int dtype_out, int act, dgtd_stream_t stream);
int dgtd_linear_residual_fwd(const void* a, const void* w, const float* bias, const float* gamma,
                             const float* keep, int rows_per_sample, const float* residual,
                             float* out, int M, int N, int K, int dtype_in, dgtd_stream_t stream);

int dgtd_fusion_sum_fwd(const float* z0, const float* z1, const float* z2, const float* z3, const int* hw,
                        const float* bias, float* out_nhwc, float* out_nchw, void* out_pad, int Cpad, int B, int C,
                        dgtd_stream_t stream);

int dgtd_conv_nhwc_fwd(const void* x, const void* w, const float* bias, void* out, int B, int h,
                       int wd, int Cin, int ldx, int oh, int ow, int Cout, int ldo, int ks,
                       int stride, int off, int act, int dtype_in, int dtype_out,
                       dgtd_stream_t stream);
int dgtd_conv_nhwc_grouped_fwd(const void* x, const void* w, const float* bias, void* out, int B,
                               int h, int wd, int Cin, int ldx, int oh, int ow, int Cout, int ldo,
                               int ks, int stride, int off, int act, int dtype_in, int dtype_out,
                               int groups, int64_t x_group_stride, int w_group_rows,
                               int64_t out_group_stride, dgtd_stream_t stream);
int dgtd_resize_nhwc_fwd(const void* x, void* out, int B, int h, int w, int C, int oh, int ow,
                         int dtype_in, int dtype_out, dgtd_stream_t stream);

int dgtd_linear_dgrad(const float* g, const float* w, float* dx, const float* pre, const float* keep,
                      const float* gamma, int rows_per_sample, int M, int N, int K, int accumulate,
                      dgtd_stream_t stream);
int dgtd_linear_wgrad(const float* g, const float* a, float* dw, float* ws, const float* keep, int rows_per_sample,
                      int M, int N, int K, int ks, int h, int wd, int Cin, int ldx, int oh, int ow, int stride,
                      int off, dgtd_stream_t stream);
int dgtd_linear_wgrad_ws_floats(int M, int N, int K);
int dgtd_colsum(const float* x, const float* keep, int rows_per_sample, float* ws, float* out, int M, int N,
                dgtd_stream_t stream);
int dgtd_layer_scale_finalize(const float* G, const float* s, const float* W2, const float* b2, const float* gamma,
                              float* dW2, float* db2, float* dgamma, int N, int K, dgtd_stream_t stream);
int dgtd_gelu_fwd(const float* x, float* out, int64_t n, dgtd_stream_t stream);
int dgtd_relu_bwd(const float* g, const float* out, float* dx, int64_t n, dgtd_stream_t stream);
int dgtd_ln_rows_bwd(const float* g, const float* y, const float* w, float* dy, float* ws, float* dw, float* db,
                     int64_t rows, int C, float eps, dgtd_stream_t stream);
int dgtd_ln_rows_bwd_ws_floats(int64_t rows, int C);
int dgtd_dwconv7_fwd(const float* x, const float* wT, const float* bias, const float* add, float* y, int B, int h,
                     int w, int C, int flip, dgtd_stream_t stream);
int dgtd_dwconv7_wgrad(const float* x, const float* dy, float* ws, float* dwT, float* db, int B, int h, int w, int C,
                       dgtd_stream_t stream);
int dgtd_stem_patchify(const float* image, const float* grid, int G, void* patches, int out_dtype, int B, int H,
                       int W, dgtd_stream_t stream);
int dgtd_stem_unpatchify(const float* dpatches, float* dimg, int B, int H, int W, dgtd_stream_t stream);
int dgtd_patchify2(const float* x, float* out, int B, int h, int w, int C, dgtd_stream_t stream);
int dgtd_unpatchify2(const float* dp, float* dx, int B, int h, int w, int C, dgtd_stream_t stream);
int dgtd_resize_nhwc_bwd(const float* g, float* dx, int B, int h, int w, int C, int oh, int ow, int accumulate,
                         dgtd_stream_t stream);

int dgtd_transpose_op(const void* src, const void* aux, void* dst, void* dstT, const float* keep, const float* gamma,
                      int rows_per_sample, int M, int N, int mode, dgtd_stream_t stream);
int dgtd_colsum_bf16(const void* x, float* ws, float* out, int M, int N, dgtd_stream_t stream);
int dgtd_eltwise_colsum_ws_floats(int M, int N);
int dgtd_eltwise_colsum(const void* src, const void* aux, void* dst, const float* keep, int rows_per_sample, float* ws,
                        float* colsum, int M, int N, int mode, dgtd_stream_t stream);
int dgtd_wgrad_tc_ws_floats(int Mo, int No, int Kr);
int dgtd_wgrad_tc_mn(const void* a, int lda, const void* b, int ldb, float* out, float* ws, int Mo, int No, int Kr,
                     int transpose_out, dgtd_stream_t stream);
int dgtd_col2im_nhwc(const void* dcol, int dcol_dtype, int ldc, int Ct, const void* mask, int ldm, void* out,
                     int out_dtype, int ldo, int B, int h, int w, int C, int ks, int stride, int off, int oh, int ow,
                     dgtd_stream_t stream);
int dgtd_im2col_nhwc(const void* x, int ldx, void* col, int B, int h, int w, int C, int ks, int stride, int off, int oh,
                     int ow, dgtd_stream_t stream);
int dgtd_group_sum(const void* x, int dtype, float* out, int64_t M, int groups, int group_stride, int C,
                   dgtd_stream_t stream);
int dgtd_ln_rows_fwd(const float* y, const float* ln_w, const float* ln_b, void* out, int out_dtype, int64_t rows,
                     int C, float eps, dgtd_stream_t stream);

int dgtd_cast_fwd(const void* src, void* dst, int64_t n, int dtype_src, int dtype_dst,
                  dgtd_stream_t stream);
int dgtd_nhwc_to_nchw_fwd(const void* x, float* out, int B, int h, int w, int C, int ldx,
                          int dtype_in, dgtd_stream_t stream);
int dgtd_nchw_to_nhwc_fwd(const float* x, void* out, int B, int h, int w, int C, int ldo,
                          int dtype_out, dgtd_stream_t stream);

int dgtd_ln_tokens_fwd(const float* x, const void* add, int add_dtype, float* sum_out, const float* ln_w,
                       const float* ln_b, void* out, int out_dtype, int64_t rows, int C, float eps,
                       dgtd_stream_t stream);
int dgtd_patchify_tokens_fwd(const void* x, void* out, int dtype, int B, int h, int w, int C, int sr,
                             dgtd_stream_t stream);
int dgtd_dwconv3_gelu_fwd(const void* x, const float* wT, const float* bias, void* out, int dtype, int B, int h, int w,
                          int C, dgtd_stream_t stream);
int dgtd_dwconv3_fwd(const void* x, const float* wT, const float* bias, void* out, int dtype, int B, int h, int w, int C,
                     dgtd_stream_t stream);
int dgtd_attention_fwd(const void* q, const void* kv, void* out, int dtype, int B, int N, int Nk, int heads,
                       float scale, dgtd_stream_t stream);
int64_t dgtd_attention_bwd_ws_floats(int B, int N, int Nk, int heads);
int dgtd_attention_bwd(const void* q, const void* kv, const void* out, const float* dout, float* dq, float* dkv, float* ws,
                       int dtype, int B, int N, int Nk, int heads, float scale, dgtd_stream_t stream);
int64_t dgtd_dwconv3_gelu_bwd_ws_floats(void);
int dgtd_dwconv3_gelu_bwd(const void* x, const float* wT, const float* bias, const float* g, float* du, float* dwT,
                          float* dbias, float* ws, int dtype, int B, int h, int w, int C, dgtd_stream_t stream);

int dgtd_boundary_weight_fwd(const float* gt, float* weit, int planes, int H, int W, dgtd_stream_t stream);
int dgtd_structure_loss_ws_floats(int planes, int64_t HW);
int dgtd_structure_loss_fwd(const float* preds, const float* gt, const float* weit, float* ws, float* sums, float* loss,
                            int planes, int64_t HW, dgtd_stream_t stream);
int dgtd_structure_loss_bwd(const float* preds, const float* gt, const float* weit, const float* sums,
                            const float* grad_out, float* dpreds, int planes, int64_t HW, dgtd_stream_t stream);

int dgtd_ssim_loss_ws_floats(int64_t n);
int dgtd_ssim_loss_fwd(const float* emb1, const float* image, float* ws, float* out, int planes, int H, int W,
                       dgtd_stream_t stream);

int dgtd_conv_nhwc_affine_fwd(const float* x, const float* w, const float* scale, const float* shift,
                              const float* prelu, const float* residual, int ldr, float* out, int B, int h, int wd,
                              int Cin, int ldx, int oh, int ow, int Cout, int ldo, int ks, int stride, int off,
                              dgtd_stream_t stream);
int dgtd_channel_sums_chunks(int hw);
int dgtd_channel_sums_fwd(const float* x, int ldx, float* partial, int B, int hw, int C, dgtd_stream_t stream);
int dgtd_channel_gate_fwd(const float* partial, int nchunks, int hw, const float* w1, const float* w2, float* gate,
                          int B, int C, int Cr, int Co, dgtd_stream_t stream);
int dgtd_gated_sum_fwd(const float* a, int lda, const float* ga, const float* sa, const float* b, int ldb,
                       const float* gb, const float* sb, float* out, int ldo, int B, int hw, int C,
                       dgtd_stream_t stream);
int dgtd_resize_nhwc_ld_fwd(const float* x, int ldx, float* out, int ldo, int B, int h, int w, int C, int oh, int ow,
                            int align_corners, dgtd_stream_t stream);
int dgtd_copy_channels_fwd(const float* x, int ldx, float* out, int ldo, int64_t rows, int C, dgtd_stream_t stream);
int dgtd_head1_fwd(const float* x, int ldx, const float* w, const float* bias, float* out, int64_t rows, int C,
                   int accumulate, dgtd_stream_t stream);
int dgtd_im2col_act_fwd(const float* x, int ldx, void* col, const float* prelu, int B, int h, int w, int C, int ks,
                        int stride, int off, int oh, int ow, dgtd_stream_t stream);
int dgtd_cast_pad_act_fwd(const float* x, int ldx, void* out, const float* prelu, int64_t rows, int C, int Cp,
                          dgtd_stream_t stream);
int dgtd_conv3x3_tc_fwd(const void* x, const void* w, const float* bias, float* out, int B, int h, int wd, int Cp,
                        int Cout, int ldo, dgtd_stream_t stream);
int dgtd_sigmoid_fwd(const float* x, float* out, int64_t n, dgtd_stream_t stream);

int64_t dgtd_col_stats_ws_bytes(int64_t M, int C);
int dgtd_bn_train_fwd(const float* y, int ldy, const float* gamma, const float* beta, float* run_mean, float* run_var,
                      float momentum, float eps, float* out, int ldo, float* mean, float* rstd, void* ws, int64_t M,
                      int C, dgtd_stream_t stream);
int dgtd_bn_apply_fwd(const float* y, int ldy, const float* mean, const float* rstd, const float* gamma,
                      const float* beta, float* out, int ldo, int64_t M, int C, dgtd_stream_t stream);
int dgtd_bn_train_bwd(const float* dy, int lddy, const float* y, int ldy, const float* mean, const float* rstd,
                      const float* gamma, float* dx, int lddx, float* dgamma, float* dbeta, void* ws, int batch_stats,
                      int64_t M, int C, dgtd_stream_t stream);
int dgtd_prelu_fwd(const float* u, const float* slope, float* v, int64_t n, dgtd_stream_t stream);
int64_t dgtd_prelu_bwd_ws_bytes(int64_t n);
int dgtd_prelu_bwd(const float* u, const float* g, const float* slope, float* du, float* dslope, void* ws, int64_t n,
                   dgtd_stream_t stream);
int dgtd_channel_dot_fwd(const float* a, int lda, const float* b, int ldb, float* partial, int B, int hw, int C,
                         dgtd_stream_t stream);
int64_t dgtd_gate_bwd_ws_floats(int B, int C, int Cr, int Cs);
int dgtd_gate_bwd(const float* part, int nch, int hw, const float* dpart, int nchd, const float* w1, const float* w2,
                  const float* v1, const float* v2, float* dmean, float* dw1, float* dw2, float* dv1, float* dv2,
                  float* ws, int accumulate, int B, int C, int Cr, int Cs, dgtd_stream_t stream);
int dgtd_gated_bwd(const float* g, int ldg, const float* gate, const float* scal, const float* dmean, float* out, int ldo,
                   int B, int hw, int C, dgtd_stream_t stream);
int dgtd_head1_bwd(const float* g, const float* x, int ldx, const float* w, float* dx, int lddx, float* dw, float* db,
                   void* ws, int64_t rows, int C, dgtd_stream_t stream);
int dgtd_resize_nhwc_ld_bwd(const float* g, int ldg, float* dx, int lddx, int B, int h, int w, int C, int oh, int ow,
                            int align_corners, dgtd_stream_t stream);

int64_t dgtd_sod_metrics_ws_bytes(int B, int H, int W);
int dgtd_sod_metrics_fwd(const float* pred, const float* gt, void* ws, double* out, double* curves, int B, int H,
                         int W, dgtd_stream_t stream);
int64_t dgtd_sod_wfm_ws_bytes(int B, int H, int W);
int dgtd_sod_wfm_fwd(const float* pred, const float* gt, void* ws, double* out, int B, int H, int W,
                     dgtd_stream_t stream);
int dgtd_sod_metrics_sized_fwd(const float* pred, const float* gt, const int32_t* sizes, void* ws, double* out,
                               double* curves, int B, int Hmax, int Wmax, dgtd_stream_t stream);
int dgtd_sod_wfm_sized_fwd(const float* pred, const float* gt, const int32_t* sizes, void* ws, double* out, int B,
                           int Hmax, int Wmax, dgtd_stream_t stream);

int dgtd_adamw_slice_bytes(void);
int dgtd_adamw_step(float* p, const float* g, float* m, float* v, const void* table, int nslices, float beta1, float beta2,
                    float eps, int step, float grad_scale, float lr_scale, dgtd_stream_t stream);

#ifdef __cplusplus
}
#endif
#endif
```

Baseline: 5374.

## Fuse LayerNorm row statistics into ConvNeXt MLP kernel and prefetch next tile

Measured after the change: 5195 (median of 6 runs). 3.3% lower.

```diff
diff --git a/depth-guided-texture-diffusion-for-image-semantic-segmentation_b200/csrc/common.cuh b/depth-guided-texture-diffusion-for-image-semantic-segmentation_b200/csrc/common.cuh
--- a/depth-guided-texture-diffusion-for-image-semantic-segmentation_b200/csrc/common.cuh
+++ b/depth-guided-texture-diffusion-for-image-semantic-segmentation_b200/csrc/common.cuh
@@ -39,6 +39,37 @@
 #pragma unroll
   for (int o = 16; o > 0; o >>= 1) v += __shfl_xor_sync(0xffffffffu, v, o);
   return v;
+}
+
+template <int LPR, int V>
+__device__ __forceinline__ float2 row_moments_bf16(const uint4 (&raw)[V], float inv_c, float eps) {
+  float f[V][8];
+  float s = 0.f;
+#pragma unroll
+  for (int j = 0; j < V; ++j) {
+    const uint32_t w4[4] = {raw[j].x, raw[j].y, raw[j].z, raw[j].w};
+#pragma unroll
+    for (int e = 0; e < 4; ++e) {
+      f[j][2 * e] = __uint_as_float(w4[e] << 16);
+      f[j][2 * e + 1] = __uint_as_float(w4[e] & 0xffff0000u);
+    }
+    s += ((f[j][0] + f[j][1]) + (f[j][2] + f[j][3])) + ((f[j][4] + f[j][5]) + (f[j][6] + f[j][7]));
+  }
+#pragma unroll
+  for (int o = LPR / 2; o > 0; o >>= 1) s += __shfl_xor_sync(0xffffffffu, s, o);
+  const float mean = s * inv_c;
+  float q = 0.f;
+#pragma unroll
+  for (int j = 0; j < V; ++j) {
+#pragma unroll
+    for (int e = 0; e < 8; e += 2) {
+      const float a = f[j][e] - mean, b = f[j][e + 1] - mean;
+      q += a * a + b * b;
+    }
+  }
+#pragma unroll
+  for (int o = LPR / 2; o > 0; o >>= 1) q += __shfl_xor_sync(0xffffffffu, q, o);
+  return make_float2(mean, 1.0f / sqrtf(q * inv_c + eps));
 }
 
 __device__ __forceinline__ float gelu_erf(float x) {
diff --git a/depth-guided-texture-diffusion-for-image-semantic-segmentation_b200/csrc/convnext_ops.cu b/depth-guided-texture-diffusion-for-image-semantic-segmentation_b200/csrc/convnext_ops.cu
--- a/depth-guided-texture-diffusion-for-image-semantic-segmentation_b200/csrc/convnext_ops.cu
+++ b/depth-guided-texture-diffusion-for-image-semantic-segmentation_b200/csrc/convnext_ops.cu
@@ -331,6 +331,8 @@
                    float* ws, void* out, int out_dtype, int B, int h, int w, int C, float eps, cudaStream_t s);
 int dwconv7_stats_tma(const float* x, const float* wT, const float* dw_b, __nv_bfloat16* y, float2* stats, int B, int h,
                       int w, int C, float eps, cudaStream_t s);
+int dwconv7_bf16_tma(const float* x, const float* wT, const float* dw_b, __nv_bfloat16* y, int B, int h, int w, int C,
+                     cudaStream_t s);
 }
 using namespace dgtd;
 
@@ -459,6 +461,20 @@
   int rc = dwconv7_stats_tma(x, dw_wT, dw_b, (__nv_bfloat16*)y, (float2*)stats, B, h, w, C, eps, (cudaStream_t)stream);
   if (rc > 0) {
     set_error("dwconv7_stats_tma: shape not supported by the TMA variant");
+    return -1;
+  }
+  return rc;
+}
+
+int dgtd_dwconv7_bf16_tma_fwd(const float* x, const float* dw_wT, const float* dw_b, void* y, int B, int h, int w, int C,
+                              dgtd_stream_t stream) {
+  DGTD_CHECK_ARG(x && dw_wT && dw_b && y, "dwconv7_bf16_tma: null pointer");
+  DGTD_CHECK_ARG(B > 0 && h > 0 && w > 0 && C >= 128 && C % 128 == 0 && C <= 1024,
+                 "dwconv7_bf16_tma: bad shape B=%d h=%d w=%d C=%d (C must be a multiple of 128)", B, h, w, C);
+  DGTD_CHECK_ARG((reinterpret_cast<uintptr_t>(y) & 15) == 0, "dwconv7_bf16_tma: y must be 16-byte aligned");
+  int rc = dwconv7_bf16_tma(x, dw_wT, dw_b, (__nv_bfloat16*)y, B, h, w, C, (cudaStream_t)stream);
+  if (rc > 0) {
+    set_error("dwconv7_bf16_tma: shape not supported by the TMA variant");
     return -1;
   }
   return rc;
diff --git a/depth-guided-texture-diffusion-for-image-semantic-segmentation_b200/csrc/dwconv_tma.cu b/depth-guided-texture-diffusion-for-image-semantic-segmentation_b200/csrc/dwconv_tma.cu
--- a/depth-guided-texture-diffusion-for-image-semantic-segmentation_b200/csrc/dwconv_tma.cu
+++ b/depth-guided-texture-diffusion-for-image-semantic-segmentation_b200/csrc/dwconv_tma.cu
@@ -409,34 +409,9 @@
   const float inv_c = 1.0f / C;
 #pragma unroll
   for (int u = 0; u < U; ++u) {
-    float f[V][8];
-    float s = 0.f;
-#pragma unroll
-    for (int j = 0; j < V; ++j) {
-      const uint32_t w4[4] = {raw[u][j].x, raw[u][j].y, raw[u][j].z, raw[u][j].w};
-#pragma unroll
-      for (int e = 0; e < 4; ++e) {
-        f[j][2 * e] = __uint_as_float(w4[e] << 16);
-        f[j][2 * e + 1] = __uint_as_float(w4[e] & 0xffff0000u);
-      }
-      s += ((f[j][0] + f[j][1]) + (f[j][2] + f[j][3])) + ((f[j][4] + f[j][5]) + (f[j][6] + f[j][7]));
-    }
-#pragma unroll
-    for (int o = LPR / 2; o > 0; o >>= 1) s += __shfl_xor_sync(0xffffffffu, s, o);
-    const float mean = s * inv_c;
-    float q = 0.f;
-#pragma unroll
-    for (int j = 0; j < V; ++j) {
-#pragma unroll
-      for (int e = 0; e < 8; e += 2) {
-        const float a = f[j][e] - mean, b = f[j][e + 1] - mean;
-        q += a * a + b * b;
-      }
-    }
-#pragma unroll
-    for (int o = LPR / 2; o > 0; o >>= 1) q += __shfl_xor_sync(0xffffffffu, q, o);
+    const float2 ms = row_moments_bf16<LPR, V>(raw[u], inv_c, eps);
     const int64_t row = row0 + u * RPP;
-    if (l == 0 && row < rows) stats[row] = make_float2(mean, 1.0f / sqrtf(q * inv_c + eps));
+    if (l == 0 && row < rows) stats[row] = ms;
   }
 }
 
@@ -669,8 +644,8 @@
   return 0;
 }
 
-int dwconv7_stats_tma(const float* x, const float* wT, const float* dw_b, __nv_bfloat16* y, float2* stats, int B, int h,
-                      int w, int C, float eps, cudaStream_t s) {
+int dwconv7_bf16_tma(const float* x, const float* wT, const float* dw_b, __nv_bfloat16* y, int B, int h, int w, int C,
+                     cudaStream_t s) {
   if (C % 128 || C > 1024 || (reinterpret_cast<uintptr_t>(x) & 15)) return 1;
   int SY, SX;
   dw_tile_shape(h, w, &SY, &SX);
@@ -684,13 +659,20 @@
   if (rc) return rc;
   cudaError_t e = cudaGetLastError();
   if (e != cudaSuccess) {
-    set_error("dwconv7_stats_tma: launch failed: %s", cudaGetErrorString(e));
+    set_error("dwconv7_bf16_tma: launch failed: %s", cudaGetErrorString(e));
     return -2;
   }
   count_launch();
+  return 0;
+}
+
+int dwconv7_stats_tma(const float* x, const float* wT, const float* dw_b, __nv_bfloat16* y, float2* stats, int B, int h,
+                      int w, int C, float eps, cudaStream_t s) {
+  int rc = dwconv7_bf16_tma(x, wT, dw_b, y, B, h, w, C, s);
+  if (rc) return rc;
   rc = row_stats_bf16(y, stats, (int64_t)B * h * w, C, eps, s);
   if (rc) return rc;
-  e = cudaGetLastError();
+  cudaError_t e = cudaGetLastError();
   if (e != cudaSuccess) {
     set_error("row_stats: launch failed: %s", cudaGetErrorString(e));
     return -2;
diff --git a/depth-guided-texture-diffusion-for-image-semantic-segmentation_b200/csrc/mlp_fused.cu b/depth-guided-texture-diffusion-for-image-semantic-segmentation_b200/csrc/mlp_fused.cu
--- a/depth-guided-texture-diffusion-for-image-semantic-segmentation_b200/csrc/mlp_fused.cu
+++ b/depth-guided-texture-diffusion-for-image-semantic-segmentation_b200/csrc/mlp_fused.cu
@@ -11,8 +11,10 @@
 constexpr int WST = 4;
 constexpr int NEPI = 16;
 constexpr int STG_BYTES = NEPI * 4096;
-constexpr int OFF_A = 0, OFF_H = A_BYTES, OFF_W = OFF_H + 2 * H_BYTES, OFF_STG = OFF_W + WST * BLK, OFF_BAR = OFF_STG + STG_BYTES;
-constexpr int NBARS = 2 + 2 * WST + 4 + 4 + 4 + NEPI;
+constexpr int OFF_A = 0, OFF_H = A_BYTES, OFF_W = OFF_H + 2 * H_BYTES, OFF_STG = OFF_W + WST * BLK;
+constexpr int OFF_ST = OFF_STG + STG_BYTES, OFF_BAR = OFF_ST + 2 * 128 * 8;
+constexpr int NSTAT = 64;
+constexpr int NBARS = 2 + 2 * WST + 4 + 4 + 4 + 4 + NEPI;
 constexpr int SMEM = OFF_BAR + NBARS * 8 + 16;
 constexpr int THREADS = 128 + NEPI * 32;
 static_assert(SMEM <= 232448, "shared memory budget");
@@ -25,11 +27,13 @@
   const float* gamma;
   const float* res;
   float* out;
+  float eps;
   int M, tiles;
 };
 
 __device__ __forceinline__ uint32_t swz_l(int lane) { return (uint32_t)(lane & 7); }
 
+template <bool LN>
 __global__ void __launch_bounds__(THREADS, 1)
 mlp_fused_kernel(const __grid_constant__ CUtensorMap tmY, const __grid_constant__ CUtensorMap tmW1,
                  const __grid_constant__ CUtensorMap tmW2, const __grid_constant__ CUtensorMap tmRes,
@@ -40,6 +44,7 @@
   uint8_t* sW = smem + OFF_W;
   uint64_t* bars = reinterpret_cast<uint64_t*>(smem + OFF_BAR);
   uint8_t* sStg = smem + OFF_STG;
+  float2* sStats = reinterpret_cast<float2*>(smem + OFF_ST);
   uint64_t* a_full = bars;
   uint64_t* a_empty = a_full + 1;
   uint64_t* w_full = a_empty + 1;
@@ -50,7 +55,9 @@
   uint64_t* h_empty = h_full + 2;
   uint64_t* c2_full = h_empty + 2;
   uint64_t* c2_empty = c2_full + 2;
-  uint64_t* r_full = c2_empty + 2;
+  uint64_t* st_full = c2_empty + 2;
+  uint64_t* st_empty = st_full + 2;
+  uint64_t* r_full = st_empty + 2;
   uint32_t* tmem_slot = reinterpret_cast<uint32_t*>(r_full + NEPI);
 
   const int warp = threadIdx.x >> 5, lane = threadIdx.x & 31;
@@ -63,7 +70,7 @@
   }
   if (warp == 1 && lane == 0) {
     bw::mbar_init(a_full, 1);
-    bw::mbar_init(a_empty, 1);
+    bw::mbar_init(a_empty, LN ? 1 + NSTAT : 1);
     for (int i = 0; i < 2; ++i) {
       bw::mbar_init(&c1_full[i], 1);
       bw::mbar_init(&c1_empty[i], NEPI);
@@ -71,6 +78,8 @@
       bw::mbar_init(&h_empty[i], 1);
       bw::mbar_init(&c2_full[i], 1);
       bw::mbar_init(&c2_empty[i], NEPI);
+      bw::mbar_init(&st_full[i], NSTAT);
+      bw::mbar_init(&st_empty[i], NEPI);
     }
     for (int i = 0; i < NEPI; ++i) bw::mbar_init(&r_full[i], 1);
     for (int i = 0; i < WST; ++i) {
@@ -95,16 +104,28 @@
         bw::tma_load_2d(tm, &w_full[ws], sW + ws * BLK, k0, r0);
         if (++ws == WST) { ws = 0; wph ^= 1; }
       };
+      auto load_y = [&](int j, int tile) {
+        bw::mbar_wait(a_empty, (j & 1) ^ 1);
+        bw::mbar_arrive_expect_tx(a_full, A_BYTES);
+        for (int kb = 0; kb < KB1; ++kb) bw::tma_load_2d(&tmY, a_full, sA + kb * BLK, kb * 64, tile * 128);
+      };
+      auto load_w1 = [&](int s) {
+        for (int kb = 0; kb < KB1; ++kb) load_w(&tmW1, kb * 64, s * HC);
+      };
       int it = 0;
       for (int tile = blockIdx.x; tile < p.tiles; tile += gridDim.x, ++it) {
-        bw::mbar_wait(a_empty, (it & 1) ^ 1);
-        bw::mbar_arrive_expect_tx(a_full, A_BYTES);
-        for (int kb = 0; kb < KB1; ++kb) bw::tma_load_2d(&tmY, a_full, sA + kb * BLK, kb * 64, tile * 128);
-        for (int s = 0; s <= NCH; ++s) {
-          if (s < NCH)
-            for (int kb = 0; kb < KB1; ++kb) load_w(&tmW1, kb * 64, s * HC);
-          if (s >= 1)
-            for (int kb = 0; kb < KB2; ++kb) load_w(&tmW2, (s - 1) * HC + kb * 64, 0);
+        if (it == 0) {
+          load_y(0, tile);
+          load_w1(0);
+        }
+        for (int s = 1; s <= NCH; ++s) {
+          if (s < NCH) {
+            load_w1(s);
+          } else if (tile + gridDim.x < p.tiles) {
+            load_y(it + 1, tile + gridDim.x);
+            load_w1(0);
+          }
+          for (int kb = 0; kb < KB2; ++kb) load_w(&tmW2, (s - 1) * HC + kb * 64, 0);
         }
       }
     }
@@ -114,55 +135,85 @@
       int ws = 0;
       uint32_t wph = 0;
       uint32_t q1 = 0, q2 = 0;
+      auto gemm1 = [&](int s) {
+        const uint32_t b = q1 & 1;
+        bw::mbar_wait(&c1_empty[b], ((q1 >> 1) & 1) ^ 1);
+        bw::tc_fence_after();
+        const uint32_t d = tmem_base + b * HC;
+        for (int kb = 0; kb < KB1; ++kb) {
+          bw::mbar_wait(&w_full[ws], wph);
+          bw::tc_fence_after();
+          const uint64_t da = bw::umma_smem_desc_kmajor(bw::smem_u32(sA + kb * BLK), 128);
+          const uint64_t db = bw::umma_smem_desc_kmajor(bw::smem_u32(sW + ws * BLK), 128);
+#pragma unroll
+          for (int k = 0; k < 4; ++k) bw::umma_bf16(d, da + 2 * k, db + 2 * k, idesc, (kb | k) != 0);
+          bw::umma_commit(&w_empty[ws]);
+          if (++ws == WST) { ws = 0; wph ^= 1; }
+        }
+        bw::umma_commit(&c1_full[b]);
+        if (s == NCH - 1) bw::umma_commit(a_empty);
+        ++q1;
+      };
+      auto gemm2 = [&](int c, int it) {
+        const int ab = it & 1;
+        const uint32_t b = q2 & 1;
+        if (c == 0) {
+          bw::mbar_wait(&c2_empty[ab], ((it >> 1) & 1) ^ 1);
+          bw::tc_fence_after();
+        }
+        bw::mbar_wait(&h_full[b], (q2 >> 1) & 1);
+        bw::tc_fence_after();
+        const uint32_t d = tmem_base + 2 * HC + ab * C;
+        for (int kb = 0; kb < KB2; ++kb) {
+          bw::mbar_wait(&w_full[ws], wph);
+          bw::tc_fence_after();
+          const uint64_t da = bw::umma_smem_desc_kmajor(bw::smem_u32(sH + b * H_BYTES + kb * BLK), 128);
+          const uint64_t db = bw::umma_smem_desc_kmajor(bw::smem_u32(sW + ws * BLK), 128);
+#pragma unroll
+          for (int k = 0; k < 4; ++k) bw::umma_bf16(d, da + 2 * k, db + 2 * k, idesc, (c | kb | k) != 0);
+          bw::umma_commit(&w_empty[ws]);
+          if (++ws == WST) { ws = 0; wph ^= 1; }
+        }
+        bw::umma_commit(&h_empty[b]);
+        if (c == NCH - 1) bw::umma_commit(&c2_full[ab]);
+        ++q2;
+      };
       int it = 0;
       for (int tile = blockIdx.x; tile < p.tiles; tile += gridDim.x, ++it) {
-        const int ab = it & 1;
-        bw::mbar_wait(a_full, it & 1);
-        for (int s = 0; s <= NCH; ++s) {
+        if (it == 0) {
+          bw::mbar_wait(a_full, 0);
+          gemm1(0);
+        }
+        for (int s = 1; s <= NCH; ++s) {
           if (s < NCH) {
-            const uint32_t b = q1 & 1;
-            bw::mbar_wait(&c1_empty[b], ((q1 >> 1) & 1) ^ 1);
-            bw::tc_fence_after();
-            const uint32_t d = tmem_base + b * HC;
-            for (int kb = 0; kb < KB1; ++kb) {
-              bw::mbar_wait(&w_full[ws], wph);
-              bw::tc_fence_after();
-              const uint64_t da = bw::umma_smem_desc_kmajor(bw::smem_u32(sA + kb * BLK), 128);
-              const uint64_t db = bw::umma_smem_desc_kmajor(bw::smem_u32(sW + ws * BLK), 128);
-#pragma unroll
-              for (int k = 0; k < 4; ++k) bw::umma_bf16(d, da + 2 * k, db + 2 * k, idesc, (kb | k) != 0);
-              bw::umma_commit(&w_empty[ws]);
-              if (++ws == WST) { ws = 0; wph ^= 1; }
-            }
-            bw::umma_commit(&c1_full[b]);
-            if (s == NCH - 1) bw::umma_commit(a_empty);
-            ++q1;
+            gemm1(s);
+          } else if (tile + gridDim.x < p.tiles) {
+            bw::mbar_wait(a_full, (it + 1) & 1);
+            gemm1(0);
           }
-          if (s >= 1) {
-            const int c = s - 1;
-            const uint32_t b = q2 & 1;
-            if (c == 0) {
-              bw::mbar_wait(&c2_empty[ab], ((it >> 1) & 1) ^ 1);
-              bw::tc_fence_after();
-            }
-            bw::mbar_wait(&h_full[b], (q2 >> 1) & 1);
-            bw::tc_fence_after();
-            const uint32_t d = tmem_base + 2 * HC + ab * C;
-            for (int kb = 0; kb < KB2; ++kb) {
-              bw::mbar_wait(&w_full[ws], wph);
-              bw::tc_fence_after();
-              const uint64_t da = bw::umma_smem_desc_kmajor(bw::smem_u32(sH + b * H_BYTES + kb * BLK), 128);
-              const uint64_t db = bw::umma_smem_desc_kmajor(bw::smem_u32(sW + ws * BLK), 128);
-#pragma unroll
-              for (int k = 0; k < 4; ++k) bw::umma_bf16(d, da + 2 * k, db + 2 * k, idesc, (c | kb | k) != 0);
-              bw::umma_commit(&w_empty[ws]);
-              if (++ws == WST) { ws = 0; wph ^= 1; }
-            }
-            bw::umma_commit(&h_empty[b]);
-            if (c == NCH - 1) bw::umma_commit(&c2_full[ab]);
-            ++q2;
-          }
-        }
+          gemm2(s - 1, it);
+        }
+      }
+    }
+  } else if (warp == 2 || warp == 3) {
+    if constexpr (LN) {
+      const int sub = lane >> 4, l = lane & 15;
+      const float inv_c = 1.0f / C;
+      const uint8_t* wp = sA + (l >> 3) * BLK;
+      int it = 0;
+      for (int tile = blockIdx.x; tile < p.tiles; tile += gridDim.x, ++it) {
+        const int sb = it & 1;
+        bw::mbar_wait_relaxed(&st_empty[sb], ((it >> 1) & 1) ^ 1, 64);
+        bw::mbar_wait_relaxed(a_full, it & 1, 64);
+        float2* st = sStats + sb * 128;
+#pragma unroll 4
+        for (int r = (warp - 2) * 2 + sub; r < 128; r += 4) {
+          const uint4 raw[1] = {*reinterpret_cast<const uint4*>(wp + r * 128 + (((l ^ r) & 7) << 4))};
+          const float2 ms = row_moments_bf16<16, 1>(raw, inv_c, p.eps);
+          if (l == 0) st[r] = ms;
+        }
+        bw::mbar_arrive(&st_full[sb]);
+        bw::mbar_arrive(a_empty);
       }
     }
   } else if (warp >= 4) {
@@ -174,19 +225,58 @@
     uint8_t* stg = sStg + ew * 4096;
     uint8_t* srow_p = stg + lane * 128;
     uint64_t* rbar = &r_full[ew];
+    auto epilogue2 = [&](int jt, int tile) {
+      const int ab = jt & 1;
+      bw::mbar_wait(&c2_full[ab], (jt >> 1) & 1);
+      bw::tc_fence_after();
+      uint32_t v[32];
+      bw::tmem_ld_32x32(tmem_base + lane_addr + 2 * HC + ab * C + part * 32, v);
+      bw::tmem_ld_wait();
+      bw::tc_fence_before();
+      __syncwarp();
+      if (lane == 0) bw::mbar_arrive(&c2_empty[ab]);
+      bw::mbar_wait(rbar, jt & 1);
+#pragma unroll
+      for (int j = 0; j < 32; j += 4) {
+        float4* sp = reinterpret_cast<float4*>(srow_p + ((((uint32_t)(j >> 2)) ^ swz_l(lane)) << 4));
+        float4 x = *sp;
+        const float4 bb = __ldg(reinterpret_cast<const float4*>(p.b2 + part * 32 + j));
+        float4 g = make_float4(1.f, 1.f, 1.f, 1.f);
+        if (p.gamma) g = __ldg(reinterpret_cast<const float4*>(p.gamma + part * 32 + j));
+        x.x += g.x * (__uint_as_float(v[j]) + bb.x);
+        x.y += g.y * (__uint_as_float(v[j + 1]) + bb.y);
+        x.z += g.z * (__uint_as_float(v[j + 2]) + bb.z);
+        x.w += g.w * (__uint_as_float(v[j + 3]) + bb.w);
+        *sp = x;
+      }
+      bw::fence_proxy_async_smem();
+      __syncwarp();
+      if (lane == 0) {
+        bw::tma_store_2d(&tmOut, stg, part * 32, tile * 128 + quad * 32);
+        bw::tma_store_commit();
+      }
+    };
     uint32_t q = 0;
-    int it = 0;
-    for (int tile = blockIdx.x; tile < p.tiles; tile += gridDim.x, ++it) {
+    int it = 0, tile = blockIdx.x;
+    for (; tile < p.tiles; tile += gridDim.x, ++it) {
       const int ab = it & 1;
       const int row0 = tile * 128 + quad * 32;
-      if (lane == 0) {
-        bw::tma_store_wait_read<0>();
-        bw::mbar_arrive_expect_tx(rbar, 4096);
-        bw::tma_load_2d(&tmRes, rbar, stg, part * 32, row0);
-      }
-      const float2 rs = __ldg(reinterpret_cast<const float2*>(p.row_stats) + row0 + lane);
+      float2 rs;
+      if constexpr (LN) {
+        bw::mbar_wait(&st_full[ab], (it >> 1) & 1);
+        rs = sStats[ab * 128 + quad * 32 + lane];
+        __syncwarp();
+        if (lane == 0) bw::mbar_arrive(&st_empty[ab]);
+      } else {
+        rs = __ldg(reinterpret_cast<const float2*>(p.row_stats) + row0 + lane);
+      }
       const uint64_t nm = pk2(-rs.x, -rs.x), rr = pk2(rs.y, rs.y);
       for (int c = 0; c < NCH; ++c, ++q) {
+        if (c == 2 && lane == 0) {
+          bw::tma_store_wait_read<0>();
+          bw::mbar_arrive_expect_tx(rbar, 4096);
+          bw::tma_load_2d(&tmRes, rbar, stg, part * 32, row0);
+        }
         const uint32_t b = q & 1;
         bw::mbar_wait(&c1_full[b], (q >> 1) & 1);
         bw::tc_fence_after();
@@ -225,36 +315,10 @@
         bw::fence_proxy_async_smem();
         __syncwarp();
         if (lane == 0) bw::mbar_arrive(&h_full[b]);
-      }
-      bw::mbar_wait(&c2_full[ab], (it >> 1) & 1);
-      bw::tc_fence_after();
-      uint32_t v[32];
-      bw::tmem_ld_32x32(tmem_base + lane_addr + 2 * HC + ab * C + part * 32, v);
-      bw::tmem_ld_wait();
-      bw::tc_fence_before();
-      __syncwarp();
-      if (lane == 0) bw::mbar_arrive(&c2_empty[ab]);
-      bw::mbar_wait(rbar, it & 1);
-#pragma unroll
-      for (int j = 0; j < 32; j += 4) {
-        float4* sp = reinterpret_cast<float4*>(srow_p + ((((uint32_t)(j >> 2)) ^ swz_l(lane)) << 4));
-        float4 x = *sp;
-        const float4 bb = __ldg(reinterpret_cast<const float4*>(p.b2 + part * 32 + j));
-        float4 g = make_float4(1.f, 1.f, 1.f, 1.f);
-        if (p.gamma) g = __ldg(reinterpret_cast<const float4*>(p.gamma + part * 32 + j));
-        x.x += g.x * (__uint_as_float(v[j]) + bb.x);
-        x.y += g.y * (__uint_as_float(v[j + 1]) + bb.y);
-        x.z += g.z * (__uint_as_float(v[j + 2]) + bb.z);
-        x.w += g.w * (__uint_as_float(v[j + 3]) + bb.w);
-        *sp = x;
-      }
-      bw::fence_proxy_async_smem();
-      __syncwarp();
-      if (lane == 0) {
-        bw::tma_store_2d(&tmOut, stg, part * 32, row0);
-        bw::tma_store_commit();
-      }
-    }
+        if (c == 0 && it > 0) epilogue2(it - 1, tile - gridDim.x);
+      }
+    }
+    if (it > 0) epilogue2(it - 1, tile - gridDim.x);
     if (lane == 0) bw::tma_store_wait_all<0>();
   }
 
@@ -271,15 +335,16 @@
 
 using namespace dgtd;
 
-extern "C" int dgtd_convnext_mlp_fused_fwd(const void* y, const float* row_stats, const void* w1, const float* col_s,
-                                           const float* cbias, const void* w2, const float* b2, const float* gamma,
-                                           const float* residual, float* out, int64_t M, int C, dgtd_stream_t stream) {
+namespace {
+template <bool LN>
+int mlp_fused_launch(const char* name, const void* y, const float* row_stats, const void* w1, const float* col_s,
+                     const float* cbias, const void* w2, const float* b2, const float* gamma, const float* residual,
+                     float* out, int64_t M, int C, float eps, cudaStream_t s) {
   using namespace mlpf;
-  DGTD_CHECK_ARG(y && row_stats && w1 && col_s && cbias && w2 && b2 && residual && out, "convnext_mlp_fused: null pointer");
-  DGTD_CHECK_ARG(C == mlpf::C, "convnext_mlp_fused: C = %d is not built (stage 0, C = 128, only)", C);
-  DGTD_CHECK_ARG(M > 0 && M % 128 == 0 && M < ((int64_t)1 << 31), "convnext_mlp_fused: M = %lld must be a positive multiple of 128",
+  DGTD_CHECK_ARG(y && (LN || row_stats) && w1 && col_s && cbias && w2 && b2 && residual && out, "%s: null pointer", name);
+  DGTD_CHECK_ARG(C == mlpf::C, "%s: C = %d is not built (stage 0, C = 128, only)", name, C);
+  DGTD_CHECK_ARG(M > 0 && M % 128 == 0 && M < ((int64_t)1 << 31), "%s: M = %lld must be a positive multiple of 128", name,
                  (long long)M);
-  cudaStream_t s = (cudaStream_t)stream;
   CUtensorMap tmY, tmW1, tmW2;
   {
     uint64_t dims[2] = {(uint64_t)C, (uint64_t)M}, str[1] = {(uint64_t)C * 2};
@@ -305,18 +370,33 @@
   }
   static bool configured = false;
   if (!configured) {
-    cudaError_t e = cudaFuncSetAttribute(mlp_fused_kernel, cudaFuncAttributeMaxDynamicSharedMemorySize, SMEM);
+    cudaError_t e = cudaFuncSetAttribute(mlp_fused_kernel<LN>, cudaFuncAttributeMaxDynamicSharedMemorySize, SMEM);
     if (e != cudaSuccess) {
-      set_error("convnext_mlp_fused: cannot opt in to %d B of shared memory: %s", SMEM, cudaGetErrorString(e));
+      set_error("%s: cannot opt in to %d B of shared memory: %s", name, SMEM, cudaGetErrorString(e));
       return -2;
     }
     configured = true;
   }
   Params p;
   p.row_stats = row_stats; p.col_s = col_s; p.cbias = cbias; p.b2 = b2; p.gamma = gamma; p.res = residual; p.out = out;
-  p.M = (int)M; p.tiles = (int)(M / 128);
+  p.eps = eps; p.M = (int)M; p.tiles = (int)(M / 128);
   const int grid = p.tiles < sm_count() ? p.tiles : sm_count();
-  mlp_fused_kernel<<<grid, THREADS, SMEM, s>>>(tmY, tmW1, tmW2, tmRes, tmOut, p);
-  DGTD_LAUNCH_CHECK("convnext_mlp_fused");
+  mlp_fused_kernel<LN><<<grid, THREADS, SMEM, s>>>(tmY, tmW1, tmW2, tmRes, tmOut, p);
+  DGTD_LAUNCH_CHECK(name);
   return 0;
 }
+}
+
+extern "C" int dgtd_convnext_mlp_fused_fwd(const void* y, const float* row_stats, const void* w1, const float* col_s,
+                                           const float* cbias, const void* w2, const float* b2, const float* gamma,
+                                           const float* residual, float* out, int64_t M, int C, dgtd_stream_t stream) {
+  return mlp_fused_launch<false>("convnext_mlp_fused", y, row_stats, w1, col_s, cbias, w2, b2, gamma, residual, out, M, C,
+                                 0.f, (cudaStream_t)stream);
+}
+
+extern "C" int dgtd_convnext_mlp_fused_ln_fwd(const void* y, const void* w1, const float* col_s, const float* cbias,
+                                              const void* w2, const float* b2, const float* gamma, const float* residual,
+                                              float* out, int64_t M, int C, float eps, dgtd_stream_t stream) {
+  return mlp_fused_launch<true>("convnext_mlp_fused_ln", y, nullptr, w1, col_s, cbias, w2, b2, gamma, residual, out, M, C,
+                                eps, (cudaStream_t)stream);
+}
diff --git a/depth-guided-texture-diffusion-for-image-semantic-segmentation_b200/twig/model/texture_diffuser.py b/depth-guided-texture-diffusion-for-image-semantic-segmentation_b200/twig/model/texture_diffuser.py
--- a/depth-guided-texture-diffusion-for-image-semantic-segmentation_b200/twig/model/texture_diffuser.py
+++ b/depth-guided-texture-diffusion-for-image-semantic-segmentation_b200/twig/model/texture_diffuser.py
@@ -197,10 +197,12 @@
                 return (wq, wq.float().sum(1).contiguous(),
                         (w1f @ self.norm.bias.detach().float() + self.pwconv1.bias.detach().float()).contiguous())
             wq, col_s, cbias = pk.get("w1.lnfold", [self.pwconv1.weight, self.pwconv1.bias, self.norm.weight, self.norm.bias], fold)
+            if keep is None and C in OP.MLP_FUSED_C and (B * h * w) % 128 == 0:
+                y = OP.dwconv7_bf16_tma(x, dw_wT, self.dwconv.bias.detach())
+                OP.convnext_mlp_fused_ln_(y.view(-1, C), wq, col_s, cbias, w2, self.pwconv2.bias.detach(), gamma, x,
+                                          self.norm.eps)
+                return x
             y, stats = OP.dwconv7_stats_tma(x, dw_wT, self.dwconv.bias.detach(), self.norm.eps)
-            if keep is None and C in OP.MLP_FUSED_C and (B * h * w) % 128 == 0:
-                OP.convnext_mlp_fused_(y.view(-1, C), stats, wq, col_s, cbias, w2, self.pwconv2.bias.detach(), gamma, x)
-                return x
             hid = OP.linear_lnfold(y.view(-1, C), wq, cbias, col_s, stats, act=ACT_GELU)
             OP.linear_residual_(hid, w2, self.pwconv2.bias.detach(), gamma, keep, h * w, x)
             return x
diff --git a/depth-guided-texture-diffusion-for-image-semantic-segmentation_b200/twig/ops/capi.py b/depth-guided-texture-diffusion-for-image-semantic-segmentation_b200/twig/ops/capi.py
--- a/depth-guided-texture-diffusion-for-image-semantic-segmentation_b200/twig/ops/capi.py
+++ b/depth-guided-texture-diffusion-for-image-semantic-segmentation_b200/twig/ops/capi.py
@@ -43,11 +43,13 @@
     "dgtd_dwconv7_ln_tma_fwd": [_P, _P, _P, _P, _P, _P, _P, _I, _I, _I, _I, _I, _F, _P],
     "dgtd_linear_fwd": [_P, _P, _P, _P, _I, _I, _I, _I, _I, _I, _I, _P],
     "dgtd_dwconv7_stats_tma_fwd": [_P, _P, _P, _P, _P, _I, _I, _I, _I, _F, _P],
+    "dgtd_dwconv7_bf16_tma_fwd": [_P, _P, _P, _P, _I, _I, _I, _I, _P],
     "dgtd_linear_ln_fwd": [_P, _P, _P, _P, _P, _F, _P, _I, _I, _I, _P],
     "dgtd_linear_tf32_fwd": [_P, _P, _P, _P, _I, _I, _I, _I, _P],
     "dgtd_linear_lnfold_fwd": [_P, _P, _P, _P, _P, _P, _I, _I, _I, _I, _I, _I, _P],
     "dgtd_linear_residual_fwd": [_P, _P, _P, _P, _P, _I, _P, _P, _I, _I, _I, _I, _P],
     "dgtd_convnext_mlp_fused_fwd": [_P, _P, _P, _P, _P, _P, _P, _P, _P, _P, _L, _I, _P],
+    "dgtd_convnext_mlp_fused_ln_fwd": [_P, _P, _P, _P, _P, _P, _P, _P, _P, _L, _I, _F, _P],
     "dgtd_fusion_sum_fwd": [_P, _P, _P, _P, _P, _P, _P, _P, _P, _I, _I, _I, _P],
     "dgtd_conv_nhwc_fwd": [_P, _P, _P, _P] + [_I] * 15 + [_P],
     "dgtd_conv_nhwc_grouped_fwd": [_P, _P, _P, _P] + [_I] * 16 + [_L, _I, _L, _P],
diff --git a/depth-guided-texture-diffusion-for-image-semantic-segmentation_b200/twig/ops/functions/texture_diffusion_func.py b/depth-guided-texture-diffusion-for-image-semantic-segmentation_b200/twig/ops/functions/texture_diffusion_func.py
--- a/depth-guided-texture-diffusion-for-image-semantic-segmentation_b200/twig/ops/functions/texture_diffusion_func.py
+++ b/depth-guided-texture-diffusion-for-image-semantic-segmentation_b200/twig/ops/functions/texture_diffusion_func.py
@@ -340,6 +340,14 @@
     return y, stats
 
 
+def dwconv7_bf16_tma(x: torch.Tensor, dw_wT, dw_b) -> torch.Tensor:
+    check_cuda(x, dw_wT, dw_b)
+    B, h, w, C = x.shape
+    y = torch.empty(B, h, w, C, device=x.device, dtype=torch.bfloat16)
+    call("dgtd_dwconv7_bf16_tma_fwd", ptr(x), ptr(dw_wT), ptr(dw_b), ptr(y), B, h, w, C, stream())
+    return y
+
+
 def linear_lnfold(a: torch.Tensor, w: torch.Tensor, bias: torch.Tensor, col_s: torch.Tensor, row_stats: torch.Tensor,
                   act: int = ACT_NONE, out_dtype: int = BF16) -> torch.Tensor:
     check_cuda(a, w, bias, col_s, row_stats)
@@ -423,6 +431,22 @@
     with _timed(4.0 * M * C * 4 * C, True, (M, 4 * C, C)):
         call("dgtd_convnext_mlp_fused_fwd", ptr(y), ptr(row_stats), ptr(w1), ptr(col_s), ptr(cbias), ptr(w2), ptr(b2),
              ptr(gamma), ptr(residual), ptr(out), M, C, stream())
+    return out
+
+
+def convnext_mlp_fused_ln_(y: torch.Tensor, w1: torch.Tensor, col_s: torch.Tensor, cbias: torch.Tensor, w2: torch.Tensor,
+                           b2: torch.Tensor, gamma: Optional[torch.Tensor], residual: torch.Tensor, eps: float = 1e-6,
+                           out: Optional[torch.Tensor] = None) -> torch.Tensor:
+    check_cuda(y, w1, col_s, cbias, w2, b2, gamma, residual)
+    C = y.shape[-1]
+    M = y.numel() // C
+    assert y.dtype == torch.bfloat16 and w1.dtype == torch.bfloat16 and w2.dtype == torch.bfloat16
+    assert w1.shape == (4 * C, C) and w2.shape == (C, 4 * C)
+    assert residual.dtype == torch.float32 and residual.numel() == M * C
+    out = residual if out is None else out
+    with _timed(4.0 * M * C * 4 * C, True, (M, 4 * C, C)):
+        call("dgtd_convnext_mlp_fused_ln_fwd", ptr(y), ptr(w1), ptr(col_s), ptr(cbias), ptr(w2), ptr(b2), ptr(gamma),
+             ptr(residual), ptr(out), M, C, float(eps), stream())
     return out
 
 
diff --git a/include/dgtd_ops.h b/include/dgtd_ops.h
--- a/include/dgtd_ops.h
+++ b/include/dgtd_ops.h
@@ -88,6 +88,8 @@
                             int C, float eps, dgtd_stream_t stream);
 int dgtd_dwconv7_stats_tma_fwd(const float* x, const float* dw_wT, const float* dw_b, void* y, float* stats, int B,
                                int h, int w, int C, float eps, dgtd_stream_t stream);
+int dgtd_dwconv7_bf16_tma_fwd(const float* x, const float* dw_wT, const float* dw_b, void* y, int B, int h, int w, int C,
+                              dgtd_stream_t stream);
 int dgtd_linear_ln_fwd(const void* a, const void* w, const float* bias, const float* ln_w, const float* ln_b, float eps,
                        float* out, int M, int N, int K, dgtd_stream_t stream);
 int dgtd_linear_tf32_fwd(const float* a, const float* w, const float* bias, float* out, int M, int N, int K, int ldo,
@@ -97,6 +99,9 @@
 int dgtd_convnext_mlp_fused_fwd(const void* y, const float* row_stats, const void* w1, const float* col_s,
                                 const float* cbias, const void* w2, const float* b2, const float* gamma,
                                 const float* residual, float* out, int64_t M, int C, dgtd_stream_t stream);
+int dgtd_convnext_mlp_fused_ln_fwd(const void* y, const void* w1, const float* col_s, const float* cbias, const void* w2,
+                                   const float* b2, const float* gamma, const float* residual, float* out, int64_t M,
+                                   int C, float eps, dgtd_stream_t stream);
 int dgtd_linear_fwd(const void* a, const void* w, const float* bias, void* out, int M, int N,
                     int K, int ldo, int dtype_in, int dtype_out, int act, dgtd_stream_t stream);
 int dgtd_linear_residual_fwd(const void* a, const void* w, const float* bias, const float* gamma,
```
